# ShigemichiMatsuzaki/MSPL

Hardware: AMD Instinct MI355X
Metric: images/sec pseudo-label gen, ESPDNet-UE s=2.0 480x360(->288x480) bs=16 (higher is better)
Workload: dtype f32; 1 GPU; BASELINE configs[1]: ESPDNet-UE s=2.0 C=13 single-source pseudo-label gen (forward + pred+0.5aux argmax + KL uncertainty + histogram), bs=16/GPU, 16x3x288x480 fp32, hipGraph replay, 3 launches in flight per GPU, 2 consecutive batches of 16 per launch; per_gpu_batch=16, batches_in_flight=3, batches_per_launch=2, classes=13

## Files before the change

include/mspl_hip.h:

```cpp
#ifndef MSPL_HIP_H
#define MSPL_HIP_H

#include <stddef.h>
#include <stdint.h>

#ifdef __cplusplus
extern "C" {
#endif

typedef enum {
    MSPL_OK = 0,
    MSPL_ERR_BAD_SHAPE = -1,
    MSPL_ERR_UNSUPPORTED = -2,
    MSPL_ERR_NULL_POINTER = -3,
    MSPL_ERR_HIP = -4
} mspl_status;

typedef struct {
    const float* scale;
    const float* shift;
    const float* alpha;
    const float* pre_add;
    const float* residual;
    const float* reinf_r;
    const float* reinf_w;
    const float* gate;
    int32_t out_ctot;
    int32_t out_coff;
    float* raw_out;
    uint32_t struct_size;
    uint32_t flags;
} mspl_epilogue_t;

#define MSPL_LAUNCH_THROUGHPUT 1u
#define MSPL_LAUNCH_K2_STREAM_OFF 2u
#define MSPL_LAUNCH_K2_STREAM_FORCE 4u

const char* mspl_version(void);
#define MSPL_ABI_VERSION 5
int mspl_abi_version(void);
size_t mspl_last_error(char* buf, size_t cap);

int mspl_eesp_dw_hff_fwd(const float* x, const float* w, const int32_t dil[4], int32_t stride,
                         int32_t N, int32_t n, int32_t H, int32_t W,
                         const mspl_epilogue_t* ep, float* out, void* stream);

int mspl_conv1x1_fwd(const float* x, const float* w, int32_t N, int32_t Cin, int32_t Cout,
                     int32_t groups, int32_t HW, const mspl_epilogue_t* ep, float* out, void* stream);

int mspl_conv3x3_fwd(const float* x, const float* w, int32_t N, int32_t Cin, int32_t Cout,
                     int32_t groups, int32_t H, int32_t W, int32_t stride, int32_t shuffle_groups,
                     const mspl_epilogue_t* ep, float* out, void* stream);

int mspl_eesp_proj_dw_hff_fits(int32_t N, int32_t Cin, int32_t n, int32_t groups, int32_t H, int32_t W, const int32_t dil[4],
                               uint32_t launch_flags);
int mspl_eesp_proj_dw_hff_fwd(const float* x, const float* wp, const float* pscale, const float* pshift, const float* palpha,
                              const float* w, const int32_t dil[4], int32_t N, int32_t Cin, int32_t n, int32_t groups,
                              int32_t H, int32_t W, const mspl_epilogue_t* ep, float* out, void* stream);

int mspl_eesp_dw_exp_fits(int32_t N, int32_t n, int32_t H, int32_t W, const int32_t dil[4], uint32_t launch_flags);
int64_t mspl_eesp_dw_exp_pack_floats(int32_t n);
int mspl_eesp_dw_exp_pack(const float* w4, const float* bscale, const float* bshift, const float* balpha, const float* wexp,
                          int32_t n, int32_t H, int32_t W, const int32_t dil[4], float* packed, void* stream);
int mspl_eesp_dw_exp_fwd(const float* r, const float* packed, const int32_t dil[4], int32_t N, int32_t n, int32_t H, int32_t W,
                         const mspl_epilogue_t* ep, float* out, void* stream);
int64_t mspl_eesp_dw_exp_next_pack_floats(int32_t n);
int mspl_eesp_dw_exp_next_pack(const float* w1, int32_t n, float* next_packed, void* stream);
int mspl_eesp_dw_exp_next_fwd(const float* r, const float* packed, const int32_t dil[4], int32_t N, int32_t n, int32_t H, int32_t W,
                              const mspl_epilogue_t* ep, float* out, const float* next_packed, const float* nscale,
                              const float* nshift, const float* nalpha, float* rnext, void* stream);

int mspl_avgpool3x3s2_fwd(const float* x, int32_t N, int32_t C, int32_t H, int32_t W,
                          const mspl_epilogue_t* ep, float* out, void* stream);

int mspl_bilinear_fwd(const float* x, int32_t N, int32_t C, int32_t Hi, int32_t Wi, int32_t Ho,
                      int32_t Wo, int32_t align_corners, const mspl_epilogue_t* ep, float* out, void* stream);

int mspl_decoder_merge_fwd(const float* enc, const float* bu, const float* w3, const float* e_scale, const float* e_shift,
                           const float* e_alpha, const float* gate, const float* b_scale, const float* b_shift,
                           const float* b_alpha, const float* wp, const float* p_scale, const float* p_shift,
                           const float* p_alpha, int32_t N, int32_t Cin, int32_t Cout, int32_t P, int32_t H, int32_t W,
                           float* out, void* stream);

int mspl_adaptive_avgpool_fwd(const float* x, int32_t N, int32_t C, int32_t Hi, int32_t Wi,
                              int32_t Ho, int32_t Wo, const mspl_epilogue_t* ep, float* out,
                              void* stream);

int mspl_pointwise_fwd(const float* x, int32_t N, int32_t C, int32_t HW, const mspl_epilogue_t* ep,
                       float* out, void* stream);

int mspl_gap_gate_fwd(const float* x, const float* w, int32_t N, int32_t Cin, int32_t Cout,
                      int32_t HW, float* mean_ws, float* gate, void* stream);

int mspl_fusion_gate_fwd(const float* z, const float* rgb, const float* depth, int64_t count, float* out, void* stream);
int mspl_fusion_gate_bwd(const float* z, const float* rgb, const float* depth, const float* gy, int64_t count,
                         float* gz, float* grgb, float* gdepth, void* stream);

int mspl_avgpool3x3s2_psum_blocks(int32_t H, int32_t W);
int mspl_avgpool3x3s2_psum_fwd(const float* x, int32_t N, int32_t C, int32_t H, int32_t W, const mspl_epilogue_t* ep, float* out,
                               float* psum, void* stream);
int mspl_gate_from_sums_fwd(const float* psum, const float* w, int32_t N, int32_t Cin, int32_t Cout, int32_t nblk, int32_t HW,
                            float* gate, void* stream);

int mspl_down_head_fits(int32_t N, int32_t nin, int32_t n, int32_t groups, int32_t H, int32_t W, uint32_t launch_flags);
int mspl_down_head_psum_blocks(int32_t H, int32_t W);
int mspl_down_head_fwd(const float* x, const float* wp, const float* pscale, const float* pshift, const float* palpha, int32_t N,
                       int32_t nin, int32_t n, int32_t groups, int32_t H, int32_t W, const mspl_epilogue_t* ep, float* r, float* out,
                       float* psum, void* stream);

int64_t mspl_pyr_down_prep_lds_bytes(int32_t N, int32_t P, int32_t h, int32_t w, int32_t nb, const int32_t* hs,
                                     const int32_t* ws);
int mspl_pyr_down_prep_fwd(const float* x, int32_t N, int32_t P, int32_t h, int32_t w, int32_t nb, const int32_t* hs,
                           const int32_t* ws, const float* const* stage_w, float* const* out, void* stream);
int mspl_pyr_down_prep_train_fwd(const float* x, int32_t N, int32_t P, int32_t h, int32_t w, int32_t nb, const int32_t* hs,
                                 const int32_t* ws, const float* const* stage_w, float* const* out, float* const* pooled,
                                 void* stream);
int mspl_pyr_down_mid_bwd(const float* const* g_e, const float* const* pooled, const float* const* stage_w, int32_t N, int32_t P,
                          int32_t h, int32_t w, int32_t nb, const int32_t* hs, const int32_t* ws, float* const* gw,
                          float* const* gx, void* stream);

int mspl_pyrpool_fused_fwd(const float* x, int32_t N, int32_t P, int32_t h, int32_t w, int32_t nb,
                           const int32_t* hs, const int32_t* ws, const float* const* stage_w,
                           const float* const* down_e, const float* br_scale, const float* br_shift,
                           const float* br_alpha, const float* merge_w, const mspl_epilogue_t* ep,
                           float* out, void* stream);

int mspl_pyrpool_fused_train_fwd(const float* x, int32_t N, int32_t P, int32_t h, int32_t w, int32_t nb,
                                 const int32_t* hs, const int32_t* ws, const float* const* stage_w,
                                 const float* const* down_e, const float* br_scale, const float* br_shift,
                                 const float* br_alpha, const float* merge_w, const mspl_epilogue_t* ep,
                                 float* out, float* zcat, void* stream);
int mspl_pyrpool_fused_train_fits(int32_t N, int32_t P, int32_t h, int32_t w, int32_t nb, const int32_t* hs, const int32_t* ws);
int mspl_pyrpool_merge_bwd(const float* gy, const float* mraw, const float* zcat, int32_t N, int32_t P, int32_t h,
                           int32_t w, int32_t nb, const float* br_scale, const float* br_shift, const float* br_alpha,
                           const float* br_mean, const float* br_inv, const float* merge_w, const float* m_scale,
                           const float* m_shift, const float* m_alpha, const float* m_mean, const float* m_inv,
                           float* gt, float* g_br_scale, float* g_br_shift, float* g_br_alpha, float* g_merge_w,
                           float* g_m_scale, float* g_m_shift, float* g_m_alpha, void* stream);
int mspl_pyrpool_branch_bwd_fits(int32_t N, int32_t P, int32_t h, int32_t w, int32_t nb, const int32_t* hs, const int32_t* ws);
int mspl_pyrpool_branch_bwd(const float* x, int32_t N, int32_t P, int32_t h, int32_t w, int32_t nb, const int32_t* hs,
                            const int32_t* ws, const float* const* stage_w, const float* const* gt, float* const* gw,
                            const float* add0, const float* add1, float* gx, void* stream);
typedef enum {
    MSPL_PYR_BRANCH_BWD_UNSUPPORTED = 0,
    MSPL_PYR_BRANCH_BWD_STREAM3 = 1,
    MSPL_PYR_BRANCH_BWD_STREAM = 2,
    MSPL_PYR_BRANCH_BWD_TILE = 3
} mspl_pyr_branch_bwd_form_t;
int mspl_pyrpool_branch_bwd_plan(int32_t N, int32_t P, int32_t h, int32_t w, int32_t nb, const int32_t* hs, const int32_t* ws,
                                 int32_t aligned8, int32_t* form, int32_t* ncb, int32_t* nseg, int32_t* seg, int32_t* taps,
                                 int32_t* tiles_x, int32_t* tiles_y);

int mspl_label_epilogue_fwd(const float* main, const float* aux, int32_t N, int32_t C,
                            int32_t Hm, int32_t Wm, int32_t Ha, int32_t Wa, int32_t H, int32_t W,
                            const uint8_t* lut, uint8_t* labels, float* prob, float* kld,
                            float* main_up, float* aux_up, void* stream);

int64_t mspl_label_epilogue_hist_workspace_bytes(int32_t N, int32_t H, int32_t W);
int mspl_label_epilogue_hist_fits(int32_t N, int32_t C, int32_t Hm, int32_t Wm, int32_t Ha, int32_t Wa, int32_t H, int32_t W);
int mspl_label_epilogue_hist_fwd(const float* main, const float* aux, int32_t N, int32_t C,
                                 int32_t Hm, int32_t Wm, int32_t Ha, int32_t Wa, int32_t H, int32_t W,
                                 const uint8_t* lut, uint8_t* labels, float* kld, unsigned long long* hist,
                                 int32_t num_classes, void* workspace, int64_t workspace_bytes, void* stream);

int mspl_label_epilogue_planes_fits(int32_t N, int32_t P, int32_t C, int32_t Hm, int32_t Wm, int32_t Ha, int32_t Wa,
                                    int32_t H, int32_t W);
int mspl_label_epilogue_planes_fwd(const float* main_planes, const float* main_w, const float* main_b,
                                   const float* aux_planes, const float* aux_w, const float* aux_b, int32_t N, int32_t P,
                                   int32_t C, int32_t Hm, int32_t Wm, int32_t Ha, int32_t Wa, int32_t H, int32_t W,
                                   const uint8_t* lut, uint8_t* labels, float* kld, unsigned long long* hist,
                                   int32_t num_classes, void* workspace, int64_t workspace_bytes, void* stream);

int mspl_merge_labels_fwd(const uint8_t* const* src, int32_t S, int64_t npix, int32_t num_classes,
                          int32_t thresh, int32_t fill, uint8_t* out, unsigned long long* hist,
                          void* stream);


int mspl_conv_bwd_data(const float* gy, const float* w, int32_t N, int32_t Cin, int32_t Cout, int32_t groups,
                       int32_t H, int32_t W, int32_t K, int32_t stride, int32_t dilation, int32_t accumulate,
                       float* gx, void* stream);

int mspl_conv_bwd_weight(const float* gy, const float* x, int32_t N, int32_t Cin, int32_t Cout, int32_t groups,
                         int32_t H, int32_t W, int32_t K, int32_t stride, int32_t dilation, int32_t accumulate,
                         float* gw, void* stream);

typedef enum {
    MSPL_WGRAD_1X1_MFMA = 1,
    MSPL_WGRAD_1X1_LDS = 2,
    MSPL_WGRAD_STEM_S2_STRIP = 3,
    MSPL_WGRAD_STEM_COB4 = 4,
    MSPL_WGRAD_STRIP = 5,
    MSPL_WGRAD_G3X3 = 6,
    MSPL_WGRAD_GENERIC = 7
} mspl_wgrad_form_t;
int mspl_conv_bwd_weight_plan(int32_t N, int32_t Cin, int32_t Cout, int32_t groups, int32_t H, int32_t W, int32_t K, int32_t stride,
                              int32_t dilation, int32_t aligned16, int32_t* form, int32_t* parts, int32_t* ngroups);
int mspl_conv1x1_wgrad_batch(const float* const* gy, const float* const* x, float* const* gw, const float* const* rowscale,
                             const int32_t* N, const int32_t* Cin, const int32_t* Cout, const int32_t* groups, const int32_t* HW, int32_t nprob,
                             void* stream);

int mspl_down_tail_fwd(const float* a, const float* b, const float* reinf, const float* alpha, int32_t N, int32_t nin, int32_t C,
                       int32_t HW, float* y, void* stream);
int mspl_down_tail_bwd(const float* a, const float* b, const float* reinf, const float* gy, const float* alpha, int32_t N, int32_t nin,
                       int32_t C, int32_t HW, float* ga, float* gb, float* greinf, float* galpha, void* stream);

int mspl_affine_prelu_bwd(const float* c, const float* pre_add, const float* residual, const float* gy,
                          const float* scale, const float* shift, const float* alpha, int32_t N, int32_t C,
                          int32_t HW, float* gz, float* gc, float* gscale, float* gshift, float* galpha, void* stream);

int mspl_avgpool3x3s2_bwd(const float* gy, int32_t N, int32_t C, int32_t H, int32_t W, float* gx, void* stream);
int mspl_bilinear_bwd(const float* gy, int32_t N, int32_t C, int32_t Hi, int32_t Wi, int32_t Ho, int32_t Wo,
                      float* gx, void* stream);
int mspl_adaptive_avgpool_bwd(const float* gy, int32_t N, int32_t C, int32_t Hi, int32_t Wi, int32_t Ho, int32_t Wo,
                              float* gx, void* stream);
typedef enum {
    MSPL_BILINEAR_BWD_GENERIC8 = 1,
    MSPL_BILINEAR_BWD_GENERIC12 = 2,
    MSPL_BILINEAR_BWD_TILE8 = 3,
    MSPL_BILINEAR_BWD_TILE12 = 4,
    MSPL_BILINEAR_BWD_WAVE = 5,
    MSPL_BILINEAR_BWD_ROWS = 6
} mspl_bilinear_bwd_form_t;
typedef enum {
    MSPL_AVGPOOL_BWD_VEC = 1,
    MSPL_AVGPOOL_BWD_PLAIN = 2
} mspl_avgpool_bwd_form_t;
int mspl_bilinear_bwd_plan(int32_t N, int32_t C, int32_t Hi, int32_t Wi, int32_t Ho, int32_t Wo, int32_t aligned, int32_t* form,
                           int32_t* tiles_x, int32_t* tiles_y, int32_t* FH, int32_t* FW);
int mspl_avgpool3x3s2_bwd_plan(int32_t N, int32_t C, int32_t H, int32_t W, int32_t aligned16, int32_t* form);

int mspl_plane_dot(const float* a, const float* b, int32_t planes, int32_t HW, float* out, void* stream);
int mspl_plane_broadcast(const float* v, int32_t planes, int32_t HW, float mul, int32_t accumulate, float* gx,
                         void* stream);
int mspl_bn_prelu_bwd(const float* c, const float* pre_add, const float* residual, const float* gy, const float* scale,
                      const float* shift, const float* alpha, const float* bn_mean, const float* bn_inv, int32_t N, int32_t C,
                      int32_t HW, float* gz, float* gc, float* ggamma, float* gbeta, float* galpha, void* stream);
int mspl_gap_gate_bwd(const float* ggate, const float* gate, const float* mean, const float* w, int32_t N,
                      int32_t Cin, int32_t Cout, float* gw, float* gmean, void* stream);
int mspl_gap_gate_bwd_accum(const float* ggate, const float* gate, const float* mean, const float* w, int32_t N,
                      int32_t Cin, int32_t Cout, float* gw, float* gmean, void* stream);
int mspl_hff_suffix_sum(const float* g, int32_t N, int32_t n, int32_t HW, float* out, void* stream);

int mspl_hff_bn_prelu_suffix_bwd(const float* z, const float* gy, const float* scale, const float* shift, const float* alpha,
                                 const float* bn_mean, const float* bn_inv, int32_t N, int32_t n, int32_t HW, float* out,
                                 float* gscale, float* gshift, float* galpha, void* stream);

int mspl_uw_loss_fwd_bwd(const float* pred, const float* aux, const int64_t* target, const float* class_weights,
                         int32_t N, int32_t C, int32_t HW, float ce_scale, float* loss_acc, float* gpred,
                         float* gaux, float* kld_out, void* stream);
int mspl_uw_loss_scaled_fwd_bwd(const float* pred, const float* aux, const int64_t* target, const float* class_weights,
                                int32_t N, int32_t C, int32_t HW, float ce_scale, float out_scale, float* loss_acc,
                                float* gpred, float* gaux, float* kld_out, void* stream);
int mspl_uw_loss_heads_supported(int32_t C);
int mspl_uw_loss_heads_fwd_bwd(const float* main_lo, const float* aux_lo, const int64_t* target, const float* class_weights,
                               int32_t N, int32_t C, int32_t Hm, int32_t Wm, int32_t Ha, int32_t Wa, int32_t H, int32_t W,
                               float ce_scale, float out_scale, float* loss_acc, float* gpred, float* gaux, void* stream);
int mspl_uw_loss_heads_meters_fwd_bwd(const float* main_lo, const float* aux_lo, const int64_t* target, const float* class_weights,
                                      int32_t N, int32_t C, int32_t Hm, int32_t Wm, int32_t Ha, int32_t Wa, int32_t H, int32_t W,
                                      float ce_scale, float out_scale, float* loss_acc, float* gpred, float* gaux,
                                      int32_t miou_classes, float meter_weight, unsigned long long* areas, double* meter, void* stream);

int mspl_dense_conv_fwd(const float* x, const float* w_packed, int32_t N, int32_t Cin, int32_t Cout, int32_t H, int32_t W,
                        int32_t ksize, int32_t dilation, const mspl_epilogue_t* ep, float* out, void* stream);

int mspl_dense_conv_split_fits(int32_t Cin, int32_t Cout, int32_t ksize, int32_t planes);
int mspl_dense_conv_split_fwd(const float* x, const uint16_t* w_split, int32_t N, int32_t Cin, int32_t Cout, int32_t H, int32_t W,
                              int32_t ksize, int32_t dilation, int32_t planes, const mspl_epilogue_t* ep, float* out, void* stream);

int64_t mspl_dense_conv_wgrad_workspace_bytes(int32_t N, int32_t Cin, int32_t Cout, int32_t H, int32_t W, int32_t ksize,
                                              int32_t dilation, int32_t split);
int mspl_dense_conv_wgrad(const float* gy, const float* x, int32_t N, int32_t Cin, int32_t Cout, int32_t H, int32_t W,
                          int32_t ksize, int32_t dilation, int32_t split, void* workspace, int64_t workspace_bytes,
                          float* dw_packed, float* dbias, void* stream);
int mspl_dense_conv_dgrad(const float* const* gy, const float* const* wt_packed, const int32_t* ksize, const int32_t* dilation,
                          int32_t nbranch, int32_t N, int32_t Cg, int32_t Cx, int32_t H, int32_t W, int32_t accumulate,
                          float* gx, void* stream);

int mspl_miou_areas_fwd(const float* logits, const uint8_t* labels, const int64_t* target, int32_t N, int32_t C, int32_t HW,
                        int32_t num_classes, unsigned long long* hist, void* stream);

int mspl_eval_epilogue_fwd(const float* main, const float* aux, const int64_t* target, const float* class_weights,
                           int32_t N, int32_t C, int32_t Hm, int32_t Wm, int32_t Ha, int32_t Wa, int32_t H, int32_t W,
                           float aux_weight, int32_t ignore_index, int32_t miou_classes, double* loss_sums,
                           unsigned long long* areas, uint8_t* labels, void* stream);
int mspl_eval_batch_finalize(double* loss_sums, double* acc, int32_t batch_images, void* stream);

int mspl_ce_meters_fwd(const float* pred, const int64_t* target, const float* class_weights, int32_t ignore_index, int32_t N,
                       int32_t C, int32_t HW, int32_t miou_classes, double* sums, unsigned long long* areas, void* stream);
int mspl_ce_flood_finalize(double* sums, float flood_level, int32_t batch_images, float* out3, double* meter, void* stream);

int mspl_ce_head_supported(int32_t C);
int mspl_ce_head_fits(int32_t N, int32_t C, int32_t Hm, int32_t Wm, int32_t H, int32_t W);
int mspl_ce_head_meters_fwd_bwd(const float* head, const int64_t* target, const float* class_weights, int32_t ignore_index,
                                int32_t N, int32_t C, int32_t Hm, int32_t Wm, int32_t H, int32_t W, int32_t miou_classes,
                                double* sums, unsigned long long* areas, float* ghead_full, void* stream);

int mspl_pixelwise_kld_fwd(const float* d1, const float* d2, int32_t N, int32_t C, int32_t HW, float* kld, void* stream);
int mspl_pixelwise_kld_bwd(const float* d1, const float* d2, const float* gkld, int32_t N, int32_t C, int32_t HW,
                           float* gd1, float* gd2, void* stream);
int mspl_weighted_ce_fwd(const float* pred, const int64_t* target, const float* u_weight, const float* class_weights,
                         int32_t ignore_index, int32_t N, int32_t C, int32_t HW, float* sums, void* stream);
int mspl_weighted_ce_bwd(const float* pred, const int64_t* target, const float* u_weight, const float* class_weights,
                         int32_t ignore_index, int32_t N, int32_t C, int32_t HW, const float* g, const float* den,
                         float* gpred, float* gu, void* stream);

int mspl_resample_ksize(int32_t in_size, int32_t out_size);
int mspl_resample_coeffs(int32_t in_size, int32_t out_size, int32_t* bounds, int32_t* kk);
int mspl_nearest_index(int32_t in_size, int32_t out_size, int32_t* idx);
int mspl_preprocess_u8_fwd(const uint8_t* src, int32_t N, int32_t Hs, int32_t Ws, int32_t C, int32_t H, int32_t W,
                           const int32_t* xb, const int32_t* xk, int32_t kx, const int32_t* yb, const int32_t* yk,
                           int32_t ky, const float* mean, const float* stdv, const uint8_t* flip, uint8_t* tmp,
                           float* out, void* stream);
int mspl_resize_label_fwd(const uint8_t* src, int32_t N, int32_t Hs, int32_t Ws, int32_t H, int32_t W,
                          const int32_t* yi, const int32_t* xi, const uint8_t* flip, int64_t* out, void* stream);

void* mspl_png_writer_create(int32_t workers, int32_t level);
int64_t mspl_png_writer_submit(void* writer, const uint8_t* host, int32_t n, int32_t H, int32_t W, const char* const* paths,
                               void* event);
int mspl_png_writer_poll(void* writer, int64_t ticket, int32_t block);
int mspl_png_writer_destroy(void* writer);

int mspl_bn_batch_stats_fwd(const float* z, int32_t N, int32_t C, int32_t HW, float eps, float momentum,
                            float* running_mean, float* running_var, double* ws, float* mean, float* invstd, void* stream);
int mspl_bn_batch_stats_fold_fwd(const float* z, int32_t N, int32_t C, int32_t HW, float eps, float momentum,
                                 float* running_mean, float* running_var, const float* gamma, const float* beta,
                                 double* ws, float* mean, float* invstd, float* scale, float* shift, void* stream);
int mspl_pyrpool_merge_fwd(const float* zcat, int32_t N, int32_t P, int32_t h, int32_t w, int32_t nb, const float* br_scale,
                           const float* br_shift, const float* br_alpha, const float* merge_w, float* out, void* stream);
int mspl_bn_stats_path_add(float* g, const float* z, const float* p, const float* q, int32_t N, int32_t P, int32_t nb, int32_t HW,
                           void* stream);
int64_t mspl_bn_fused_workspace_bytes(int32_t C);
int mspl_bn_batch_stats_fused_fwd(const float* z, int32_t N, int32_t C, int32_t HW, float eps, float momentum,
                                  float* running_mean, float* running_var, const float* gamma, const float* beta,
                                  void* ws_zeroed, float* mean, float* invstd, float* scale, float* shift,
                                  int64_t* num_batches_tracked, void* stream);
int mspl_bn_train_prelu_bwd(const float* z, const float* residual, const float* gy, const float* scale, const float* shift,
                            const float* alpha, const float* gamma, const float* mean, const float* invstd, int32_t N, int32_t C,
                            int32_t HW, float* gres, float* gc, void* ws_zeroed, int32_t accumulate, float* ggamma, float* gbeta,
                            float* galpha, float* p, float* q, void* stream);
int mspl_bn_train_small_fits(int32_t N, int32_t C, int32_t HW);
int mspl_bn_train_small_fwd(const float* z, const float* residual, const float* gamma, const float* beta, const float* alpha,
                            int32_t N, int32_t C, int32_t HW, float eps, float momentum, float* running_mean, float* running_var,
                            int64_t* num_batches_tracked, float* mean, float* invstd, float* scale, float* shift, float* y, void* stream);
int mspl_bn_train_small_bwd(const float* z, const float* residual, const float* gy, const float* scale, const float* shift,
                            const float* alpha, const float* gamma, const float* mean, const float* invstd, int32_t N, int32_t C,
                            int32_t HW, float eps, int32_t accumulate, float* gz, float* gres, float* ggamma, float* gbeta,
                            float* galpha, void* stream);
int mspl_bn_train_prelu_bwd_apply(const float* z, const float* gy, const float* scale, const float* shift, const float* alpha,
                                  const float* p, const float* q, int32_t N, int32_t C, int32_t HW, float* gz, void* stream);
int mspl_bn_batch_stats_bwd_coeffs(const float* gscale, const float* gshift, const float* gamma, const float* mean,
                                   const float* invstd, const float* scale, int32_t C, double M, int32_t accumulate,
                                   float* ggamma, float* gbeta, float* p, float* q, void* stream);
int mspl_sgd_step(float* p, const float* g, float* buf, int64_t n, float lr, float momentum, float weight_decay,
                  int32_t first_step, void* stream);

int64_t mspl_nid_workspace_floats(int32_t C, int32_t H, int32_t W, int32_t K);
int mspl_nid_hist_fwd(const float* camera, const float* label, int32_t B, int32_t C, int32_t H, int32_t W, int32_t K,
                      float bw_camera, float bw_label, float* ws, float* out, void* stream);
int mspl_nid_hist_bwd(const float* camera, const float* label, int32_t B, int32_t C, int32_t H, int32_t W, int32_t K,
                      float bw_camera, float bw_label, const float* gjoint, const float* gpl, float* glabel, void* stream);

int mspl_eesp_dw_bwd(const float* gs, const float* x, const float* w4, const int32_t* dil, int32_t stride, int32_t N,
                     int32_t n, int32_t H, int32_t W, float* gx, float* const* gw, void* stream);
int mspl_eesp_dw_bwd_weight_chunks(int32_t N, int32_t n, int32_t H, int32_t W, int32_t stride);

int mspl_eesp_bwd_fused_fits(int32_t N, int32_t n, int32_t H, int32_t W, const int32_t* dil);
int mspl_eesp_bwd_fused_bands(int32_t N, int32_t n, int32_t H, int32_t W, const int32_t* dil, int32_t* band_rows);
int mspl_eesp_bwd_fused(const float* z, const float* gy, const float* x, const float* w4, const int32_t* dil,
                        const float* scale, const float* shift, const float* alpha, const float* bn_mean,
                        const float* bn_inv, int32_t N, int32_t n, int32_t H, int32_t W, float* gx, float* const* gw,
                        float* gscale, float* gshift, float* galpha, const float* proj_c, const float* proj_scale,
                        const float* proj_shift, const float* proj_alpha, const float* proj_mean, const float* proj_inv,
                        float* g_proj_scale, float* g_proj_shift, float* g_proj_alpha, void* stream);

int mspl_hff_bn_stat_suffix_bwd(const float* z, const float* gy, const float* scale, const float* shift, const float* alpha,
                                const float* stat_p, const float* stat_q, int32_t N, int32_t n, int32_t HW, float* out, void* stream);
int mspl_eesp_bwd_fused_bnstat(const float* z, const float* gy, const float* x, const float* w4, const int32_t* dil,
                               const float* scale, const float* shift, const float* alpha, const float* stat_p, const float* stat_q,
                               int32_t N, int32_t n, int32_t H, int32_t W, float* gx, float* const* gw, void* stream);

int mspl_sum_n(const float* const* srcs, int32_t n, int64_t count, float* out, void* stream);
int mspl_sum_n_planes(const float* const* srcs, int32_t n, const float* plane_const, float mul, int32_t planes, int32_t HW, float* out,
                      void* stream);

int mspl_transpose_weights(const void* seg_table, const void* block_table, int32_t nblocks, void* stream);

int mspl_adam_step(float* p, const float* g, float* m, float* v, int64_t n, float lr, double beta1, double beta2,
                   float eps, float weight_decay, int32_t step, void* stream);

#define MSPL_FILTER_LANCZOS 1
#define MSPL_FILTER_BILINEAR 2
int mspl_resample_ksize_filter(int32_t in_size, int32_t out_size, int32_t filter);
int mspl_resample_coeffs_filter(int32_t in_size, int32_t out_size, int32_t filter, int32_t* bounds, int32_t* kk);

typedef struct mspl_train_rec {
    const int32_t* scale_x;
    const int32_t* scale_y;
    const int32_t* dscale_x;
    const int32_t* dscale_y;
    const int32_t* out_x;
    const int32_t* out_y;
    const int32_t* near_x;
    const int32_t* near_y;
    const int32_t* near_out_x;
    const int32_t* near_out_y;
    int32_t sh, sw;
    int32_t pad_h, pad_w;
    int32_t crop_i, crop_j;
    int32_t flip;
    int32_t reserved;
} mspl_train_rec_t;
int64_t mspl_train_transform_workspace_bytes(int32_t N, int32_t max_sh, int32_t max_sw, int32_t with_depth);
int mspl_train_transform_fwd(const uint8_t* rgb, const uint8_t* label, const uint8_t* depth, int32_t N, int32_t Hs, int32_t Ws,
                             int32_t H, int32_t W, int32_t crop, int32_t ignore_idx, const mspl_train_rec_t* recs_host,
                             const mspl_train_rec_t* recs_dev, const float* mean, const float* stdv, uint8_t* ws, int32_t max_sh,
                             int32_t max_sw, float* out_rgb, int64_t* out_label, float* out_depth, void* stream);

#ifdef __cplusplus
}
#endif
#endif
```

mspl_amd/csrc/pyrpool.hip:

```cpp
#include <stdlib.h>

#include "common.hpp"

namespace mspl {

constexpr int PYR_MAXB = 5;
constexpr int PYR_HALO = 4;

struct PyrGeom {
    int N, P, h, w, nb;
    int kind[PYR_MAXB];
    int hs[PYR_MAXB], ws[PYR_MAXB];
    float sh[PYR_MAXB], sw[PYR_MAXB];
    const float* stage_w[PYR_MAXB];
    const float* down_e[PYR_MAXB];
    const float* br_scale; const float* br_shift; const float* br_alpha;
    const float* merge_w;
    int TH, TW, tiles_y, tiles_x;
    int XW;
    int UH[PYR_MAXB], UW[PYR_MAXB], uoff[PYR_MAXB];
    int toff[PYR_MAXB];
    int boff, BW;
    int woff;
    unsigned mag_uw[PYR_MAXB], mag_bw;
    int CPB, cblocks;
    int stop_after;
    float* zcat;
};

__device__ __forceinline__ int ada_s(int o, int I, int O) { return (int)(((unsigned)o * (unsigned)I) / (unsigned)O); }
__device__ __forceinline__ int ada_e(int o, int I, int O) { return (int)((((unsigned)(o + 1)) * (unsigned)I + O - 1) / (unsigned)O); }
__device__ __forceinline__ int fdiv(int t, unsigned magic) { return (int)(((unsigned)t * magic) >> 24); }

__global__ __launch_bounds__(256) void pyrpool_fused_kernel(const float* __restrict__ x, PyrGeom g, Epi e,
                                                            float* __restrict__ out) {
    extern __shared__ __attribute__((aligned(16))) float smem[];
    float* xs = smem;
    float* wl = smem + g.woff;
    int bid = blockIdx.x;
    const int txi = bid % g.tiles_x;  bid /= g.tiles_x;
    const int tyi = bid % g.tiles_y;  bid /= g.tiles_y;
    const int cb = bid % g.cblocks;
    const int n = bid / g.cblocks;
    const int y0 = tyi * g.TH, x0 = txi * g.TW;
    const int tid = threadIdx.x;
    const int XH = g.TH + 2 * PYR_HALO;
    const int BH = g.TH + 2, BW2 = g.TW + 2;
    const int py_lo = max(y0 - 1, 0), px_lo = max(x0 - 1, 0);

#pragma unroll
    for (int i = 0; i < PYR_MAXB; ++i) {
        if (i >= g.nb) break;
        float* T = smem + g.toff[i];
        if (g.kind[i] == 0) {
            const int UH = g.UH[i], UW = g.UW[i];
            const int u0 = ada_s(py_lo, g.hs[i], g.h) - 1, v0 = ada_s(px_lo, g.ws[i], g.w) - 1;
            float* UR = T; float* UC = UR + 4 * UH; float* WR = UC + 4 * UW; float* WC = WR + 2 * BH;
            for (int t = tid; t < UH + UW + BH + BW2; t += 256) {
                if (t < UH) {
                    const int u = u0 + t;
                    int ya = 0, yb = 0;  float w0 = 0.f, w1 = 0.f;
                    if (u >= 0 && u < g.hs[i]) bilinear_src(g.sh[i], u, g.h, ya, yb, w0, w1); else { ya = y0; yb = y0; }
                    UR[4 * t] = __int_as_float((ya - y0 + PYR_HALO) * g.XW); UR[4 * t + 1] = __int_as_float((yb - y0 + PYR_HALO) * g.XW);
                    UR[4 * t + 2] = w0; UR[4 * t + 3] = w1;
                } else if (t < UH + UW) {
                    const int q = t - UH, v = v0 + q;
                    int xa = 0, xb = 0;  float w0 = 0.f, w1 = 0.f;
                    if (v >= 0 && v < g.ws[i]) bilinear_src(g.sw[i], v, g.w, xa, xb, w0, w1); else { xa = x0; xb = x0; }
                    UC[4 * q] = __int_as_float(xa - x0 + PYR_HALO); UC[4 * q + 1] = __int_as_float(xb - x0 + PYR_HALO);
                    UC[4 * q + 2] = w0; UC[4 * q + 3] = w1;
                } else if (t < UH + UW + BH) {
                    const int r = t - UH - UW, py = y0 - 1 + r;
                    int first = 0, cnt = 0;
                    if (py >= 0 && py < g.h) { const int us = ada_s(py, g.hs[i], g.h); first = us - 1 - u0; cnt = ada_e(py, g.hs[i], g.h) - us; }
                    WR[2 * r] = __int_as_float(first * UW); WR[2 * r + 1] = __int_as_float(cnt);
                } else {
                    const int q = t - UH - UW - BH, px = x0 - 1 + q;
                    int first = 0, cnt = 0;
                    if (px >= 0 && px < g.w) { const int vs = ada_s(px, g.ws[i], g.w); first = vs - 1 - v0; cnt = ada_e(px, g.ws[i], g.w) - vs; }
                    WC[2 * q] = __int_as_float(first); WC[2 * q + 1] = __int_as_float(cnt);
                }
            }
        } else if (g.kind[i] == 2) {
            float* DR = T; float* DC = DR + 4 * BH;
            for (int t = tid; t < BH + BW2; t += 256) {
                if (t < BH) {
                    const int py = min(max(y0 - 1 + t, 0), g.h - 1);
                    int ya, yb;  float w0, w1;
                    bilinear_src(g.sh[i], py, g.hs[i], ya, yb, w0, w1);
                    DR[4 * t] = __int_as_float(ya * g.ws[i]); DR[4 * t + 1] = __int_as_float(yb * g.ws[i]); DR[4 * t + 2] = w0; DR[4 * t + 3] = w1;
                } else {
                    const int q = t - BH, px = min(max(x0 - 1 + q, 0), g.w - 1);
                    int xa, xb;  float w0, w1;
                    bilinear_src(g.sw[i], px, g.ws[i], xa, xb, w0, w1);
                    DC[4 * q] = __int_as_float(xa); DC[4 * q + 1] = __int_as_float(xb); DC[4 * q + 2] = w0; DC[4 * q + 3] = w1;
                }
            }
        }
    }

    const int xv = g.XW >> 2;
    const bool w4 = (g.w & 3) == 0;
    auto load_x = [&](int c, int i) -> float4 {
        const float* xp = x + ((size_t)n * g.P + c) * (size_t)g.h * g.w;
        const int r = i / xv, v = i - r * xv;
        const int iy = y0 - PYR_HALO + r, ix = x0 - PYR_HALO + 4 * v;
        float4 val = make_float4(0.f, 0.f, 0.f, 0.f);
        if (iy >= 0 && iy < g.h) {
            const float* row = xp + (size_t)iy * g.w;
            if (w4 && ix >= 0 && ix + 3 < g.w) {
                val = *reinterpret_cast<const float4*>(row + ix);
            } else {
                if (ix >= 0 && ix < g.w) val.x = row[ix];
                if (ix + 1 >= 0 && ix + 1 < g.w) val.y = row[ix + 1];
                if (ix + 2 >= 0 && ix + 2 < g.w) val.z = row[ix + 2];
                if (ix + 3 >= 0 && ix + 3 < g.w) val.w = row[ix + 3];
            }
        }
        return val;
    };
    auto load_const = [&](int c, int t) -> float {
        const int n9 = g.nb * 9;
        if (t < n9) { const int i = t / 9, k = t - i * 9; return (g.kind[i] != 2) ? g.stage_w[i][c * 9 + k] : 0.f; }
        if (t < 2 * n9) { const int u = t - n9, i = u / 9, k = u - i * 9; return g.merge_w[((size_t)c * g.nb + i) * 9 + k]; }
        const int u = t - 2 * n9, i = u / 3, k = u - i * 3;
        return (k == 0 ? g.br_scale : (k == 1 ? g.br_shift : g.br_alpha))[i * g.P + c];
    };
    const int nx = XH * xv;
    const int nconst = 2 * g.nb * 9 + 3 * g.nb;
    const int c_first = cb * g.CPB;
    float4 xr0 = make_float4(0.f, 0.f, 0.f, 0.f), xr1 = xr0;
    float cr = 0.f;
    if (tid < nx) xr0 = load_x(c_first, tid);
    if (tid + 256 < nx) xr1 = load_x(c_first, tid + 256);
    if (tid < nconst) cr = load_const(c_first, tid);

    for (int ci = 0; ci < g.CPB; ++ci) {
    const int c = c_first + ci;
    if (tid < nx) *reinterpret_cast<float4*>(xs + (tid / xv) * g.XW + 4 * (tid % xv)) = xr0;
    if (tid + 256 < nx) *reinterpret_cast<float4*>(xs + ((tid + 256) / xv) * g.XW + 4 * ((tid + 256) % xv)) = xr1;
    for (int i = tid + 512; i < nx; i += 256) *reinterpret_cast<float4*>(xs + (i / xv) * g.XW + 4 * (i % xv)) = load_x(c, i);
    if (tid < nconst) wl[tid] = cr;
    if (ci + 1 < g.CPB) {
        if (tid < nx) xr0 = load_x(c + 1, tid);
        if (tid + 256 < nx) xr1 = load_x(c + 1, tid + 256);
        if (tid < nconst) cr = load_const(c + 1, tid);
    }
    __syncthreads();
    if (g.stop_after == 1) return;

#pragma unroll
    for (int i = 0; i < PYR_MAXB; ++i) {
        if (i < g.nb && g.kind[i] == 0) {
            float* U = smem + g.uoff[i];
            const int UH = g.UH[i], UW = g.UW[i];
            const float* UR = smem + g.toff[i];
            const float* UC = UR + 4 * UH;
            const unsigned mag = g.mag_uw[i];
            const int nU = UH * UW;
            for (int t = tid; t < nU; t += 256) {
                const int r = fdiv(t, mag), q = t - r * UW;
                const float4 rr = *reinterpret_cast<const float4*>(UR + 4 * r);
                const float4 cc = *reinterpret_cast<const float4*>(UC + 4 * q);
                const float* ra = xs + __float_as_int(rr.x);
                const float* rb = xs + __float_as_int(rr.y);
                const int xa = __float_as_int(cc.x), xb = __float_as_int(cc.y);
                const float top = cc.z * ra[xa] + cc.w * ra[xb];
                const float bot = cc.z * rb[xa] + cc.w * rb[xb];
                U[t] = rr.z * top + rr.w * bot;
            }
        }
    }
    __syncthreads();
    if (g.stop_after == 2) return;

    float* B = smem + g.boff;
    const int npos = BH * BW2;
    const int XWl = g.XW, BWl = g.BW, hl = g.h, wl_ = g.w;
    const unsigned magb = g.mag_bw;
    auto keep_raw = [&](int i, int r, int q, int py, int px, float b) {
        if (g.zcat && r >= 1 && r <= g.TH && q >= 1 && q <= g.TW)
            g.zcat[(((size_t)n * g.nb + i) * g.P + c) * (size_t)hl * wl_ + (size_t)py * wl_ + px] = b;
    };
#pragma unroll
    for (int i = 0; i < PYR_MAXB; ++i) {
        if (i >= g.nb) break;
        const float* ws9 = wl + i * 9;
        const float* kbr = wl + 2 * g.nb * 9 + i * 3;
        const float bsc = kbr[0], bsh = kbr[1], bal = kbr[2];
        float* Bi = B + i * BH * BWl;
        const float* T = smem + g.toff[i];
        if (g.kind[i] == 1) {
            const float w00 = ws9[0], w01 = ws9[1], w02 = ws9[2], w10 = ws9[3], w11 = ws9[4], w12 = ws9[5],
                        w20 = ws9[6], w21 = ws9[7], w22 = ws9[8];
            for (int t = tid; t < npos; t += 256) {
                const int r = fdiv(t, magb), q = t - r * BW2;
                const int py = y0 - 1 + r, px = x0 - 1 + q;
                float b = 0.f;
                if (py >= 0 && py < hl && px >= 0 && px < wl_) {
                    const float* p = xs + (r + PYR_HALO - 2) * XWl + (q + PYR_HALO - 2);
                    b = w00 * p[0];
                    b = fmaf(w01, p[1], b); b = fmaf(w02, p[2], b);
                    b = fmaf(w10, p[XWl], b); b = fmaf(w11, p[XWl + 1], b); b = fmaf(w12, p[XWl + 2], b);
                    b = fmaf(w20, p[2 * XWl], b); b = fmaf(w21, p[2 * XWl + 1], b); b = fmaf(w22, p[2 * XWl + 2], b);
                    keep_raw(i, r, q, py, px, b);
                    b = fmaf(b, bsc, bsh);
                    b = b > 0.f ? b : bal * b;
                }
                Bi[r * BWl + q] = b;
            }
        } else if (g.kind[i] == 0) {
            const float* U = smem + g.uoff[i];
            const int UW = g.UW[i];
            const float* WR = T + 4 * g.UH[i] + 4 * UW;
            const float* WC = WR + 2 * BH;
            const float w00 = ws9[0], w01 = ws9[1], w02 = ws9[2], w10 = ws9[3], w11 = ws9[4], w12 = ws9[5],
                        w20 = ws9[6], w21 = ws9[7], w22 = ws9[8];
            for (int t = tid; t < npos; t += 256) {
                const int r = fdiv(t, magb), q = t - r * BW2;
                const int py = y0 - 1 + r, px = x0 - 1 + q;
                float b = 0.f;
                if (py >= 0 && py < hl && px >= 0 && px < wl_) {
                    const float2 wr = *reinterpret_cast<const float2*>(WR + 2 * r);
                    const float2 wc = *reinterpret_cast<const float2*>(WC + 2 * q);
                    const int rcnt = __float_as_int(wr.y), ccnt = __float_as_int(wc.y);
                    const float* p0 = U + __float_as_int(wr.x) + __float_as_int(wc.x);
                    float s = 0.f;
                    if (rcnt == 2 && ccnt == 2) {
                        float u[4][4];
#pragma unroll
                        for (int a2 = 0; a2 < 4; ++a2)
#pragma unroll
                            for (int b2 = 0; b2 < 4; ++b2) u[a2][b2] = p0[a2 * UW + b2];
#pragma unroll
                        for (int du = 0; du < 2; ++du)
#pragma unroll
                            for (int dv = 0; dv < 2; ++dv) {
                                float cv = w00 * u[du][dv];
                                cv = fmaf(w01, u[du][dv + 1], cv); cv = fmaf(w02, u[du][dv + 2], cv);
                                cv = fmaf(w10, u[du + 1][dv], cv); cv = fmaf(w11, u[du + 1][dv + 1], cv); cv = fmaf(w12, u[du + 1][dv + 2], cv);
                                cv = fmaf(w20, u[du + 2][dv], cv); cv = fmaf(w21, u[du + 2][dv + 1], cv); cv = fmaf(w22, u[du + 2][dv + 2], cv);
                                s += cv;
                            }
                        b = s * 0.25f;
                    } else {
                        for (int du = 0; du < rcnt; ++du)
                            for (int dv = 0; dv < ccnt; ++dv) {
                                const float* p = p0 + du * UW + dv;
                                float cv = w00 * p[0];
                                cv = fmaf(w01, p[1], cv); cv = fmaf(w02, p[2], cv);
                                cv = fmaf(w10, p[UW], cv); cv = fmaf(w11, p[UW + 1], cv); cv = fmaf(w12, p[UW + 2], cv);
                                cv = fmaf(w20, p[2 * UW], cv); cv = fmaf(w21, p[2 * UW + 1], cv); cv = fmaf(w22, p[2 * UW + 2], cv);
                                s += cv;
                            }
                        b = s / (float)(rcnt * ccnt);
                    }
                    keep_raw(i, r, q, py, px, b);
                    b = fmaf(b, bsc, bsh);
                    b = b > 0.f ? b : bal * b;
                }
                Bi[r * BWl + q] = b;
            }
        } else {
            const float* E = g.down_e[i] + ((size_t)n * g.P + c) * (size_t)g.hs[i] * g.ws[i];
            for (int t = tid; t < npos; t += 256) {
                const int r = fdiv(t, magb), q = t - r * BW2;
                const int py = y0 - 1 + r, px = x0 - 1 + q;
                float b = 0.f;
                if (py >= 0 && py < hl && px >= 0 && px < wl_) {
                    const float4 rr = *reinterpret_cast<const float4*>(T + 4 * r);
                    const float4 cc = *reinterpret_cast<const float4*>(T + 4 * BH + 4 * q);
                    const float* ra = E + __float_as_int(rr.x);
                    const float* rb = E + __float_as_int(rr.y);
                    const int xa = __float_as_int(cc.x), xb = __float_as_int(cc.y);
                    const float top = cc.z * ra[xa] + cc.w * ra[xb];
                    const float bot = cc.z * rb[xa] + cc.w * rb[xb];
                    b = rr.z * top + rr.w * bot;
                    keep_raw(i, r, q, py, px, b);
                    b = fmaf(b, bsc, bsh);
                    b = b > 0.f ? b : bal * b;
                }
                Bi[r * BWl + q] = b;
            }
        }
    }
    __syncthreads();
    if (g.stop_after == 3) return;

    const int cabs = e.coff + c;
    const EpiCh ec = epi_channel(e, cabs);
    const int XS = g.TW >> 2;
    const int nstrip = g.TH * XS, nbl = g.nb;
    for (int t = tid; t < nstrip; t += 256) {
        const int ty = t / XS, xsi = t - ty * XS;
        const int y = y0 + ty, xb = x0 + xsi * 4;
        if (y >= hl || xb >= wl_) continue;
        float acc[4] = {0.f, 0.f, 0.f, 0.f};
#pragma unroll
        for (int i = 0; i < PYR_MAXB; ++i) {
            if (i >= nbl) break;
            const float* wm = wl + nbl * 9 + i * 9;
#pragma unroll
            for (int ky = 0; ky < 3; ++ky) {
                const float* row = B + (i * BH + ty + ky) * BWl + xsi * 4;
                const float4 a = *reinterpret_cast<const float4*>(row);
                const float2 b2 = *reinterpret_cast<const float2*>(row + 4);
                const float rv[6] = {a.x, a.y, a.z, a.w, b2.x, b2.y};
#pragma unroll
                for (int j = 0; j < 4; ++j) {
                    acc[j] = fmaf(wm[ky * 3 + 0], rv[j], acc[j]);
                    acc[j] = fmaf(wm[ky * 3 + 1], rv[j + 1], acc[j]);
                    acc[j] = fmaf(wm[ky * 3 + 2], rv[j + 2], acc[j]);
                }
            }
        }
        const int pix = y * wl_ + xb;
        float* dst = out + epi_offset(e, n, cabs, pix);
        if (e.raw) {
            float* rdst = e.raw + ((size_t)n * g.P + c) * (size_t)hl * wl_ + pix;
#pragma unroll
            for (int j = 0; j < 4; ++j)
                if (xb + j < wl_) rdst[j] = acc[j];
        }
        if ((wl_ & 3) == 0) {
            store_out4(dst, epi_apply4(e, ec, acc, n, cabs, pix));
        } else {
#pragma unroll
            for (int j = 0; j < 4; ++j)
                if (xb + j < wl_) dst[j] = epi_apply(e, ec, acc[j], n, cabs, pix + j);
        }
    }
    __syncthreads();
    }
}

int pyrpool_sep_try(const float* x, int N, int P, int h, int w, int nb, const int32_t* hs, const int32_t* ws,
                    const float* const* stage_w, const float* const* down_e, const float* br_scale,
                    const float* br_shift, const float* br_alpha, const float* merge_w, const Epi& e, float* out,
                    hipStream_t stream, unsigned launch_flags);
int pyrpool_stream_try(const float* x, int N, int P, int h, int w, int nb, const int32_t* hs, const int32_t* ws,
                       const float* const* stage_w, const float* const* down_e, const float* br_scale,
                       const float* br_shift, const float* br_alpha, const float* merge_w, const Epi& e, float* out,
                       hipStream_t stream, float* zcat = nullptr);

}

using namespace mspl;

static int pyrpool_fused_launch(const float* x, int32_t N, int32_t P, int32_t h, int32_t w, int32_t nb,
                               const int32_t* hs, const int32_t* ws, const float* const* stage_w,
                               const float* const* down_e, const float* br_scale, const float* br_shift,
                               const float* br_alpha, const float* merge_w, const mspl_epilogue_t* ep,
                               float* out, float* zcat, void* stream, bool dry = false) {
    MSPL_REQUIRE(dry || (x && hs && ws && stage_w && down_e && br_scale && br_shift && br_alpha && merge_w && out),
                 MSPL_ERR_NULL_POINTER, "pyrpool_fused: null pointer");
    MSPL_REQUIRE(hs && ws, MSPL_ERR_NULL_POINTER, "pyrpool_fused: null pointer");
    MSPL_REQUIRE(N > 0 && P > 0 && h > 0 && w > 0, MSPL_ERR_BAD_SHAPE, "pyrpool_fused: bad shape N=%d P=%d %dx%d", N, P, h, w);
    MSPL_REQUIRE(nb >= 1 && nb <= PYR_MAXB, MSPL_ERR_UNSUPPORTED, "pyrpool_fused: %d branches (1..%d)", nb, PYR_MAXB);
    if (int rc = check_epi(ep, P, "pyrpool_fused", zcat != nullptr)) return rc;
    if (!dry) {
        static const int force_tables = MSPL_TUNE_INT("MSPL_PYR_TABLES", 0);
        if (!force_tables) {
            const int rc3 = pyrpool_stream_try(x, N, P, h, w, nb, hs, ws, stage_w, down_e, br_scale, br_shift, br_alpha, merge_w,
                                               make_epi(ep, P, h * w), out, (hipStream_t)stream, zcat);
            if (rc3 <= 0) return rc3;
            if (!zcat) {
                const int rc = pyrpool_sep_try(x, N, P, h, w, nb, hs, ws, stage_w, down_e, br_scale, br_shift, br_alpha, merge_w,
                                               make_epi(ep, P, h * w), out, (hipStream_t)stream, epi_flags(ep));
                if (rc <= 0) return rc;
            }
        }
    }
    PyrGeom g;
    memset(&g, 0, sizeof(g));
    g.N = N; g.P = P; g.h = h; g.w = w; g.nb = nb;
    g.br_scale = br_scale; g.br_shift = br_shift; g.br_alpha = br_alpha; g.merge_w = merge_w;
    g.zcat = zcat;
    g.TW = w >= 32 ? 32 : ((w + 3) & ~3);
    g.TH = h >= 16 ? 16 : h;
    g.tiles_x = ceil_div(w, g.TW);
    g.tiles_y = ceil_div(h, g.TH);
    g.XW = g.TW + 2 * PYR_HALO;
    int off = (g.TH + 2 * PYR_HALO) * g.XW;
    off = (off + 3) & ~3;
    for (int i = 0; i < nb; ++i) {
        MSPL_REQUIRE(hs[i] > 0 && ws[i] > 0, MSPL_ERR_BAD_SHAPE, "pyrpool_fused: branch %d size %dx%d", i, hs[i], ws[i]);
        g.hs[i] = hs[i]; g.ws[i] = ws[i];
        g.stage_w[i] = dry ? nullptr : stage_w[i]; g.down_e[i] = dry ? nullptr : down_e[i];
        if (hs[i] == h && ws[i] == w) {
            g.kind[i] = 1;
            MSPL_REQUIRE(dry || stage_w[i], MSPL_ERR_NULL_POINTER, "pyrpool_fused: branch %d needs stage weights", i);
        } else if (hs[i] >= h && ws[i] >= w) {
            g.kind[i] = 0;
            MSPL_REQUIRE(dry || stage_w[i], MSPL_ERR_NULL_POINTER, "pyrpool_fused: branch %d needs stage weights", i);
            MSPL_REQUIRE(hs[i] <= 4 * h && ws[i] <= 4 * w, MSPL_ERR_UNSUPPORTED, "pyrpool_fused: up-scale beyond 4x");
            g.sh[i] = bilinear_scale(h, hs[i]); g.sw[i] = bilinear_scale(w, ws[i]);
            g.UH[i] = (int)(((int64_t)(g.TH + 2) * hs[i] + h - 1) / h) + 4;
            g.UW[i] = (int)(((int64_t)(g.TW + 2) * ws[i] + w - 1) / w) + 4;
            g.uoff[i] = off;
            off += g.UH[i] * g.UW[i];
            off = (off + 3) & ~3;
        } else if (hs[i] <= h && ws[i] <= w) {
            g.kind[i] = 2;
            MSPL_REQUIRE(dry || down_e[i], MSPL_ERR_NULL_POINTER, "pyrpool_fused: branch %d needs its low-resolution map", i);
            g.sh[i] = bilinear_scale(hs[i], h); g.sw[i] = bilinear_scale(ws[i], w);
        } else {
            set_error("pyrpool_fused: branch %d mixes up- and down-sampling (%dx%d vs %dx%d)", i, hs[i], ws[i], h, w);
            return MSPL_ERR_UNSUPPORTED;
        }
    }
    auto magic = [](int d) { return (unsigned)(((1u << 24) + (unsigned)d - 1) / (unsigned)d); };
    for (int i = 0; i < nb; ++i) {
        g.toff[i] = off;
        if (g.kind[i] == 0) { off += 4 * g.UH[i] + 4 * g.UW[i] + 2 * (g.TH + 2) + 2 * (g.TW + 2); g.mag_uw[i] = magic(g.UW[i]); }
        else if (g.kind[i] == 2) off += 4 * (g.TH + 2) + 4 * (g.TW + 2);
        off = (off + 3) & ~3;
    }
    g.mag_bw = magic(g.TW + 2);
    static const int dbg_stop = MSPL_TUNE_INT("MSPL_PYR_STOP", 0);
    g.stop_after = dbg_stop;
    g.BW = (g.TW + 2 + 3 + 4) & ~3;
    g.boff = off;
    off += nb * (g.TH + 2) * g.BW;
    off = (off + 3) & ~3;
    g.woff = off;
    off += nb * 9 * 2 + nb * 3;
    const size_t lds = (size_t)off * sizeof(float);
    MSPL_REQUIRE(lds <= 64 * 1024, MSPL_ERR_UNSUPPORTED, "pyrpool_fused: tile needs %zu B of LDS", lds);
    if (dry) return MSPL_OK;
    const Epi e = make_epi(ep, P, h * w);
    int cpb = 1;
    while (cpb * 2 <= P && P % (cpb * 2) == 0 && (int64_t)N * (P / (cpb * 2)) * g.tiles_y * g.tiles_x >= 2048) cpb *= 2;
    static const int dbg_cpb = MSPL_TUNE_INT("MSPL_PYR_CPB", 0);
    if (dbg_cpb > 0 && P % dbg_cpb == 0) cpb = dbg_cpb;
    g.CPB = cpb; g.cblocks = P / cpb;
    const int64_t blocks = (int64_t)N * g.cblocks * g.tiles_y * g.tiles_x;
    MSPL_REQUIRE(blocks < (1ll << 31), MSPL_ERR_BAD_SHAPE, "pyrpool_fused: grid too large");
    hipLaunchKernelGGL(pyrpool_fused_kernel, dim3((unsigned)blocks), dim3(256), lds, (hipStream_t)stream, x, g, e, out);
    MSPL_CHECK_LAUNCH("pyrpool_fused");
    return MSPL_OK;
}

extern "C" int mspl_pyrpool_fused_fwd(const float* x, int32_t N, int32_t P, int32_t h, int32_t w, int32_t nb,
                                      const int32_t* hs, const int32_t* ws, const float* const* stage_w,
                                      const float* const* down_e, const float* br_scale, const float* br_shift,
                                      const float* br_alpha, const float* merge_w, const mspl_epilogue_t* ep,
                                      float* out, void* stream) {
    return pyrpool_fused_launch(x, N, P, h, w, nb, hs, ws, stage_w, down_e, br_scale, br_shift, br_alpha, merge_w, ep, out, nullptr,
                                stream);
}

extern "C" int mspl_pyrpool_fused_train_fwd(const float* x, int32_t N, int32_t P, int32_t h, int32_t w, int32_t nb,
                                            const int32_t* hs, const int32_t* ws, const float* const* stage_w,
                                            const float* const* down_e, const float* br_scale, const float* br_shift,
                                            const float* br_alpha, const float* merge_w, const mspl_epilogue_t* ep,
                                            float* out, float* zcat, void* stream) {
    MSPL_REQUIRE(zcat, MSPL_ERR_NULL_POINTER, "pyrpool_fused_train: zcat is required");
    return pyrpool_fused_launch(x, N, P, h, w, nb, hs, ws, stage_w, down_e, br_scale, br_shift, br_alpha, merge_w, ep, out, zcat,
                                stream);
}

extern "C" int mspl_pyrpool_fused_train_fits(int32_t N, int32_t P, int32_t h, int32_t w, int32_t nb, const int32_t* hs,
                                             const int32_t* ws) {
    float dummy = 0.f;
    return pyrpool_fused_launch(nullptr, N, P, h, w, nb, hs, ws, nullptr, nullptr, nullptr, nullptr, nullptr, nullptr, nullptr, nullptr,
                                &dummy, nullptr, true) == MSPL_OK;
}
```

mspl_amd/csrc/pyrpool_stream.hip:

```cpp
#include <stdlib.h>

#include <algorithm>

#include "common.hpp"
#include "pyr_stencil.hpp"

namespace mspl {

constexpr int P3_MAXB = 5;
#ifndef P3_STEPS
#define P3_STEPS 2
#endif
constexpr int P3_SEGMAX = 19;

struct Pyr3Geom {
    int N, P, h, w;
    int hs[P3_MAXB], ws[P3_MAXB];
    float sh[P3_MAXB], sw[P3_MAXB];
    int SEG, nseg, ncb, CBW;
    unsigned total;
};

template <int T, int PXL>
__device__ __forceinline__ void p3_up_branch(const float (&xw)[5][PXL + 4], const float* __restrict__ Arow,
                                             const float (&C)[3][PXL][5], float (&b)[PXL]) {
    constexpr int R0 = (5 - T) / 2;
    constexpr int NCOL = PXL + T - 1;
#pragma unroll
    for (int ky = 0; ky < 3; ++ky) {
        float a[5];
        {
            const float4 t4 = *reinterpret_cast<const float4*>(Arow + ky * 8);
            a[0] = t4.x; a[1] = t4.y; a[2] = t4.z; a[3] = t4.w;
            a[4] = T > 4 ? Arow[ky * 8 + 4] : 0.f;
        }
        float cs[NCOL];
#pragma unroll
        for (int s = 0; s < NCOL; ++s) {
            float v = a[0] * xw[R0][R0 + s];
#pragma unroll
            for (int rr = 1; rr < T; ++rr) v = fmaf(a[rr], xw[R0 + rr][R0 + s], v);
            cs[s] = v;
        }
#pragma unroll
        for (int j = 0; j < PXL; ++j) {
            float v = b[j];
#pragma unroll
            for (int s = 0; s < T; ++s) v = fmaf(C[ky][j][s], cs[j + s], v);
            b[j] = v;
        }
    }
}

template <int PXL> struct P3Vec;
template <> struct P3Vec<1> { typedef float T; };
template <> struct P3Vec<2> { typedef float2 T; };

template <int T0, int T1, int PXL, bool TRAIN>
__global__ __launch_bounds__(256, 2) void pyrpool_stream_kernel(const float* __restrict__ x, const float* __restrict__ sw0,
                                                                const float* __restrict__ sw1, const float* __restrict__ sw2,
                                                                const float* __restrict__ de3, const float* __restrict__ de4,
                                                                const float* __restrict__ br_scale, const float* __restrict__ br_shift,
                                                                const float* __restrict__ br_alpha, const float* __restrict__ merge_w,
                                                                const float* __restrict__ ep_scale,
                                                                const float* __restrict__ ep_shift,
                                                                const float* __restrict__ ep_alpha, int ep_ctot, int ep_coff,
                                                                Pyr3Geom g, float* __restrict__ out, float* __restrict__ zcat,
                                                                float* __restrict__ mraw) {
    __shared__ __attribute__((aligned(16))) float At[2][(P3_SEGMAX + 2) * 24];
    __shared__ float Gt[2][3][PXL][5][64];
    __shared__ __attribute__((aligned(16))) float Wm[4][5][12];
    const int lane = threadIdx.x & 63, wave = __builtin_amdgcn_readfirstlane(threadIdx.x >> 6);
    unsigned bid = blockIdx.x;
    const int sgi = bid % g.nseg;  bid /= g.nseg;
    const int cb = bid % g.ncb;  bid /= g.ncb;
    const int plane = (int)bid * 4 + wave;
    const int n = plane / g.P, c = plane - n * g.P;
    const int h = g.h, w = g.w;
    const int ys = sgi * g.SEG, ye = min(ys + g.SEG, h);
    const int px0 = cb * g.CBW + (lane - 1) * PXL;
    const bool writer = lane >= 1 && lane <= 62 && px0 < w;

    if (wave < 2) {
        const int ri = lane / 3, ky = lane - 3 * ri;
        if (ri < g.SEG + 2) {
            float acc[5];
            if (wave == 0) p3_coeffs<T0>(ys - 1 + ri, ky, h, g.hs[0], g.sh[0], acc);
            else p3_coeffs<T1>(ys - 1 + ri, ky, h, g.hs[1], g.sh[1], acc);
            float* d = &At[wave][ri * 24 + ky * 8];
            d[0] = acc[0]; d[1] = acc[1]; d[2] = acc[2]; d[3] = acc[3]; d[4] = acc[4];
        }
    }
#pragma unroll
    for (int t = 0; t < 6 * PXL; ++t) {
        if ((t & 3) == wave) {
            const int ub = t / (3 * PXL), r = t - ub * 3 * PXL, kx = r / PXL, j = r - kx * PXL;
            float acc[5];
            if (ub == 0) p3_coeffs<T0>(px0 + j, kx, w, g.ws[0], g.sw[0], acc);
            else p3_coeffs<T1>(px0 + j, kx, w, g.ws[1], g.sw[1], acc);
#pragma unroll
            for (int q = 0; q < 5; ++q) Gt[ub][kx][j][q][lane] = acc[q];
        }
    }
    __syncthreads();
    float C0[3][PXL][5], C1[3][PXL][5];
    {
        const float* w0p = sw0 + (size_t)c * 9;
        const float* w1p = sw1 + (size_t)c * 9;
#pragma unroll
        for (int j = 0; j < PXL; ++j)
#pragma unroll
            for (int s2 = 0; s2 < 5; ++s2) {
                const float a0 = Gt[0][0][j][s2][lane], a1 = Gt[0][1][j][s2][lane], a2 = Gt[0][2][j][s2][lane];
                const float b0 = Gt[1][0][j][s2][lane], b1 = Gt[1][1][j][s2][lane], b2 = Gt[1][2][j][s2][lane];
#pragma unroll
                for (int ky = 0; ky < 3; ++ky) {
                    C0[ky][j][s2] = fmaf(w0p[ky * 3 + 2], a2, fmaf(w0p[ky * 3 + 1], a1, w0p[ky * 3] * a0));
                    C1[ky][j][s2] = fmaf(w1p[ky * 3 + 2], b2, fmaf(w1p[ky * 3 + 1], b1, w1p[ky * 3] * b0));
                }
            }
    }
    unsigned dxa[2][PXL], dxb[2][PXL];  float dw0[2][PXL], dw1[2][PXL];
#pragma unroll
    for (int i = 0; i < 2; ++i)
#pragma unroll
        for (int j = 0; j < PXL; ++j) {
            const int px = min(max(px0 + j, 0), w - 1);
            int xa, xb;
            bilinear_src(g.sw[3 + i], px, g.ws[3 + i], xa, xb, dw0[i][j], dw1[i][j]);
            dxa[i][j] = (unsigned)xa * 4u;  dxb[i][j] = (unsigned)xb * 4u;
        }
    const float* wsame = sw2 + (size_t)c * 9;
    if (lane < 45) Wm[wave][lane / 9][lane % 9] = merge_w[(size_t)c * 45 + lane];
    const float4* wmq = reinterpret_cast<const float4*>(&Wm[wave][0][0]);
    float bsc[5], bsh[5], bal[5];
#pragma unroll
    for (int i = 0; i < 5; ++i) { bsc[i] = br_scale[i * g.P + c]; bsh[i] = br_shift[i * g.P + c]; bal[i] = br_alpha[i * g.P + c]; }
    const int cabs = ep_coff + c;
    const float esc = ep_scale ? ep_scale[cabs] : 1.f, esh = ep_shift ? ep_shift[cabs] : 0.f, eal = ep_alpha ? ep_alpha[cabs] : 1.f;
    const unsigned plane_id = __builtin_amdgcn_readfirstlane((unsigned)(n * g.P + c));
    const float* xpl = x + (size_t)plane_id * (size_t)(h * w);
    const float* e3 = de3 + (size_t)plane_id * (size_t)(g.hs[3] * g.ws[3]);
    const float* e4 = de4 + (size_t)plane_id * (size_t)(g.hs[4] * g.ws[4]);
    float* opl = out + ((size_t)__builtin_amdgcn_readfirstlane((unsigned)(n * ep_ctot + cabs))) * (size_t)(h * w);
    bool colin[PXL];
#pragma unroll
    for (int j = 0; j < PXL; ++j) colin[j] = px0 + j >= 0 && px0 + j < w;

    constexpr unsigned P3_OOB = 0x7ffffff0u;
    unsigned xoff[PXL + 4];
#pragma unroll
    for (int j = 0; j < PXL + 4; ++j) {
        const int cx = px0 - 2 + j;
        xoff[j] = (cx >= 0 && cx < w) ? (unsigned)cx * 4u : P3_OOB;
    }
    auto load_row = [&](int r, float (&v)[PXL + 4]) {
        const bool rin = r >= 0 && r < h;
        const float* row = xpl + (size_t)(rin ? r : 0) * w;
        const __amdgpu_buffer_rsrc_t rs = __builtin_amdgcn_make_buffer_rsrc(const_cast<float*>(row), 0, rin ? w * 4 : 0, 0x00020000);
        if (PXL == 2) {
#pragma unroll
            for (int j = 0; j < PXL + 4; j += 2) {
                typedef unsigned u32x2 __attribute__((ext_vector_type(2)));
                const u32x2 t = __builtin_amdgcn_raw_buffer_load_b64(rs, xoff[j], 0, 0);
                v[j] = __uint_as_float(t.x);  v[j + 1] = __uint_as_float(t.y);
            }
        } else {
#pragma unroll
            for (int j = 0; j < PXL + 4; ++j) v[j] = __uint_as_float(__builtin_amdgcn_raw_buffer_load_b32(rs, xoff[j], 0, 0));
        }
    };

    float xw[5][PXL + 4];
#pragma unroll
    for (int rr = 0; rr < 5; ++rr) load_row(ys - 3 + rr, xw[rr]);
    float en[2][PXL][4];
    float enwy0[2], enwy1[2];
    auto load_e = [&](int r) {
#pragma unroll
        for (int i = 0; i < 2; ++i) {
            int ya, yb;
            bilinear_src(g.sh[3 + i], min(max(r, 0), h - 1), g.hs[3 + i], ya, yb, enwy0[i], enwy1[i]);
            const int rowb = g.ws[3 + i] * 4;
            const __amdgpu_buffer_rsrc_t ra = __builtin_amdgcn_make_buffer_rsrc(const_cast<float*>((i == 0 ? e3 : e4) + ya * g.ws[3 + i]), 0, rowb, 0x00020000);
            const __amdgpu_buffer_rsrc_t rb = __builtin_amdgcn_make_buffer_rsrc(const_cast<float*>((i == 0 ? e3 : e4) + yb * g.ws[3 + i]), 0, rowb, 0x00020000);
#pragma unroll
            for (int j = 0; j < PXL; ++j) {
                en[i][j][0] = __uint_as_float(__builtin_amdgcn_raw_buffer_load_b32(ra, dxa[i][j], 0, 0));
                en[i][j][1] = __uint_as_float(__builtin_amdgcn_raw_buffer_load_b32(ra, dxb[i][j], 0, 0));
                en[i][j][2] = __uint_as_float(__builtin_amdgcn_raw_buffer_load_b32(rb, dxa[i][j], 0, 0));
                en[i][j][3] = __uint_as_float(__builtin_amdgcn_raw_buffer_load_b32(rb, dxb[i][j], 0, 0));
            }
        }
    };
    load_e(ys - 1);
    float acc[3][PXL];
#pragma unroll
    for (int r = 0; r < 3; ++r)
#pragma unroll
        for (int j = 0; j < PXL; ++j) acc[r][j] = 0.f;

    auto row_step = [&](const int br) __attribute__((always_inline)) {
        float bv[5][PXL];
        const bool rowin = br >= 0 && br < h;
        float ecur[2][PXL][4], wy0c[2], wy1c[2];
#pragma unroll
        for (int i = 0; i < 2; ++i) {
            wy0c[i] = enwy0[i]; wy1c[i] = enwy1[i];
#pragma unroll
            for (int j = 0; j < PXL; ++j)
#pragma unroll
                for (int q = 0; q < 4; ++q) ecur[i][j][q] = en[i][j][q];
        }
        if (br < ye) load_e(br + 1);
        float xn[PXL + 4];
        load_row(br + 3, xn);
        __builtin_amdgcn_sched_barrier(0);
        if (rowin) {
            const float* A0 = &At[0][(br - (ys - 1)) * 24];
            const float* A1 = &At[1][(br - (ys - 1)) * 24];
#pragma unroll
            for (int j = 0; j < PXL; ++j) { bv[0][j] = 0.f; bv[1][j] = 0.f; bv[2][j] = 0.f; }
            p3_up_branch<T0, PXL>(xw, A0, C0, bv[0]);
            p3_up_branch<T1, PXL>(xw, A1, C1, bv[1]);
#pragma unroll
            for (int ky = 0; ky < 3; ++ky) {
                const float w0 = wsame[ky * 3], w1 = wsame[ky * 3 + 1], w2 = wsame[ky * 3 + 2];
#pragma unroll
                for (int j = 0; j < PXL; ++j) {
                    bv[2][j] = fmaf(w0, xw[1 + ky][j + 1], bv[2][j]);
                    bv[2][j] = fmaf(w1, xw[1 + ky][j + 2], bv[2][j]);
                    bv[2][j] = fmaf(w2, xw[1 + ky][j + 3], bv[2][j]);
                }
            }
#pragma unroll
            for (int i = 0; i < 2; ++i)
#pragma unroll
                for (int j = 0; j < PXL; ++j) {
                    const float top = dw0[i][j] * ecur[i][j][0] + dw1[i][j] * ecur[i][j][1];
                    const float bot = dw0[i][j] * ecur[i][j][2] + dw1[i][j] * ecur[i][j][3];
                    bv[3 + i][j] = wy0c[i] * top + wy1c[i] * bot;
                }
            if (TRAIN && writer && br >= ys && br < ye) {
#pragma unroll
                for (int i = 0; i < 5; ++i) {
                    float* zp = zcat + (((size_t)n * 5 + i) * g.P + c) * (size_t)h * w + (size_t)br * w + px0;
                    if (PXL == 2) *reinterpret_cast<float2*>(zp) = make_float2(bv[i][0], bv[i][PXL - 1]);
                    else zp[0] = bv[i][0];
                }
            }
#pragma unroll
            for (int i = 0; i < 5; ++i)
#pragma unroll
                for (int j = 0; j < PXL; ++j) {
                    float v = fmaf(bv[i][j], bsc[i], bsh[i]);
                    v = v > 0.f ? v : bal[i] * v;
                    bv[i][j] = colin[j] ? v : 0.f;
                }
        } else {
#pragma unroll
            for (int i = 0; i < 5; ++i)
#pragma unroll
                for (int j = 0; j < PXL; ++j) bv[i][j] = 0.f;
        }
#pragma unroll
        for (int i = 0; i < 5; ++i) {
            float bx[PXL + 2];
            bx[0] = p3_from_left(bv[i][PXL - 1]);
#pragma unroll
            for (int j = 0; j < PXL; ++j) bx[1 + j] = bv[i][j];
            bx[PXL + 1] = p3_from_right(bv[i][0]);
            const float4 q0 = wmq[i * 3], q1 = wmq[i * 3 + 1], q2 = wmq[i * 3 + 2];
            const float wv[12] = {q0.x, q0.y, q0.z, q0.w, q1.x, q1.y, q1.z, q1.w, q2.x, q2.y, q2.z, q2.w};
#pragma unroll
            for (int r = 0; r < 3; ++r) {
                const int ky = 2 - r;
                const float w0 = wv[ky * 3], w1 = wv[ky * 3 + 1], w2 = wv[ky * 3 + 2];
#pragma unroll
                for (int j = 0; j < PXL; ++j) {
                    acc[r][j] = fmaf(w0, bx[j], acc[r][j]);
                    acc[r][j] = fmaf(w1, bx[j + 1], acc[r][j]);
                    acc[r][j] = fmaf(w2, bx[j + 2], acc[r][j]);
                }
            }
        }
#pragma unroll
        for (int rr = 0; rr < 4; ++rr)
#pragma unroll
            for (int j = 0; j < PXL + 4; ++j) xw[rr][j] = xw[rr + 1][j];
#pragma unroll
        for (int j = 0; j < PXL + 4; ++j) xw[4][j] = xn[j];
        const int y = br - 1;
        if (y >= ys) {
            float v[PXL];
#pragma unroll
            for (int j = 0; j < PXL; ++j) {
                v[j] = fmaf(acc[0][j], esc, esh);
                v[j] = (ep_alpha && v[j] <= 0.f) ? eal * v[j] : v[j];
            }
            if (writer) {
                float* dst = opl + (size_t)y * w + px0;
                if (PXL == 2) store_out2(dst, make_float2(v[0], v[PXL - 1]));
                else dst[0] = v[0];
                if (TRAIN) {
                    float* rp = mraw + ((size_t)n * g.P + c) * (size_t)h * w + (size_t)y * w + px0;
                    if (PXL == 2) *reinterpret_cast<float2*>(rp) = make_float2(acc[0][0], acc[0][PXL - 1]);
                    else rp[0] = acc[0][0];
                }
            }
        }
#pragma unroll
        for (int j = 0; j < PXL; ++j) { acc[0][j] = acc[1][j]; acc[1][j] = acc[2][j]; acc[2][j] = 0.f; }
    };
    constexpr int STEPS = TRAIN ? 2 : P3_STEPS;
#pragma unroll 1
    for (int br = ys - 1; br <= ye; br += STEPS) {
        row_step(br);
#pragma unroll
        for (int u = 1; u < STEPS; ++u)
            if (br + u <= ye) row_step(br + u);
    }
}

int pyrpool_stream_try(const float* x, int N, int P, int h, int w, int nb, const int32_t* hs, const int32_t* ws,
                       const float* const* stage_w, const float* const* down_e, const float* br_scale,
                       const float* br_shift, const float* br_alpha, const float* merge_w, const Epi& e, float* out,
                       hipStream_t stream, float* zcat) {
    static const int off = (MSPL_TUNE_INT("MSPL_PYR_STREAM", 1) == 0);
    static const int min_w = MSPL_TUNE_INT("MSPL_PYR_STREAM_MINW", 40);
    if (off || nb != 5 || w < min_w || ((int64_t)N * P) % 4 != 0) return 1;
    if (e.pre_add || e.residual || e.reinf_r || e.gate) return 1;
    for (int i = 0; i < 5; ++i) if (hs[i] <= 0 || ws[i] <= 0) return 1;
    if (!(hs[0] > h && ws[0] > w && hs[1] > h && ws[1] > w)) return 1;
    if (!(hs[2] == h && ws[2] == w)) return 1;
    if (!(hs[3] <= h && ws[3] <= w && hs[4] <= h && ws[4] <= w && (hs[3] < h || ws[3] < w) && (hs[4] < h || ws[4] < w))) return 1;
    if (!stage_w[0] || !stage_w[1] || !stage_w[2] || !down_e[3] || !down_e[4]) return 1;
    int taps[2];
    for (int i = 0; i < 2; ++i) {
        const int R = std::max(p3_stencil_radius(h, hs[i]), p3_stencil_radius(w, ws[i]));
        if (R > 2) return 1;
        taps[i] = R <= 1 ? 3 : 5;
    }
    const int PXL = w <= 62 ? 1 : 2;
    if (PXL == 2 && ((w & 1) || (((uintptr_t)out) & 7) || (((uintptr_t)x) & 7))) return 1;
    if (zcat && (!e.raw || e.ctot != P || e.coff != 0)) return 1;
    if (zcat && PXL == 2 && ((((uintptr_t)zcat) | ((uintptr_t)e.raw)) & 7)) return 1;
    Pyr3Geom g;
    memset(&g, 0, sizeof(g));
    g.N = N; g.P = P; g.h = h; g.w = w;
    for (int i = 0; i < 5; ++i) {
        g.hs[i] = hs[i]; g.ws[i] = ws[i];
        if (i < 2) { g.sh[i] = bilinear_scale(h, hs[i]); g.sw[i] = bilinear_scale(w, ws[i]); }
        if (i > 2) { g.sh[i] = bilinear_scale(hs[i], h); g.sw[i] = bilinear_scale(ws[i], w); }
    }
    g.CBW = 62 * PXL;
    g.ncb = ceil_div(w, g.CBW);
    static const int dbg_seg = MSPL_TUNE_INT("MSPL_PYR_SEG", 0);
    int seg = std::min(h, P3_SEGMAX);
    while (seg > 6 && (int64_t)N * P * g.ncb * ceil_div(h, seg) < 2048) --seg;
    seg = ceil_div(h, ceil_div(h, seg));
    if (dbg_seg > 0 && dbg_seg <= P3_SEGMAX) seg = std::min(dbg_seg, h);
    g.SEG = seg;
    g.nseg = ceil_div(h, seg);
    const int64_t waves = (int64_t)N * P * g.ncb * g.nseg;
    if (waves >= (1ll << 31)) return 1;
    g.total = (unsigned)waves;
    const dim3 grid((unsigned)(waves / 4)), blk(256);
#define MSPL_P3_LAUNCH(A, B, L) do { \
        if (zcat) hipLaunchKernelGGL((pyrpool_stream_kernel<A, B, L, true>), grid, blk, 0, stream, x, stage_w[0], stage_w[1], stage_w[2], down_e[3], down_e[4], br_scale, br_shift, br_alpha, merge_w, e.scale, e.shift, e.alpha, e.ctot, e.coff, g, out, zcat, e.raw); \
        else hipLaunchKernelGGL((pyrpool_stream_kernel<A, B, L, false>), grid, blk, 0, stream, x, stage_w[0], stage_w[1], stage_w[2], down_e[3], down_e[4], br_scale, br_shift, br_alpha, merge_w, e.scale, e.shift, e.alpha, e.ctot, e.coff, g, out, (float*)nullptr, (float*)nullptr); } while (0)
    if (PXL == 1) {
        if (taps[0] == 3 && taps[1] == 3) MSPL_P3_LAUNCH(3, 3, 1);
        else if (taps[0] == 3) MSPL_P3_LAUNCH(3, 5, 1);
        else if (taps[1] == 3) MSPL_P3_LAUNCH(5, 3, 1);
        else MSPL_P3_LAUNCH(5, 5, 1);
    } else {
        if (taps[0] == 3 && taps[1] == 3) MSPL_P3_LAUNCH(3, 3, 2);
        else if (taps[0] == 3) MSPL_P3_LAUNCH(3, 5, 2);
        else if (taps[1] == 3) MSPL_P3_LAUNCH(5, 3, 2);
        else MSPL_P3_LAUNCH(5, 5, 2);
    }
#undef MSPL_P3_LAUNCH
    MSPL_CHECK_LAUNCH("pyrpool_fused(streaming form)");
    return MSPL_OK;
}

}
```

mspl_amd/layers.py:

```python
import contextlib
import gc
import math
import os
import weakref

import torch
from torch import nn

from . import autograd as ag
from . import ops
from .ops import Epi

config_inp_reinf = 3
PYR_SCALES = (2.0, 1.5, 1.0, 0.5, 0.1)


_PARAM_EPOCH = [0]


def bump_param_epoch():
    _PARAM_EPOCH[0] += 1


def _key(tensors):
    return (_PARAM_EPOCH[0],) + tuple((t.data_ptr(), t._version) for t in tensors)


def cached(module, name, deps, builder):
    store = module.__dict__.setdefault('_mspl_cache', {})
    k = _key(deps)
    hit = store.get(name)
    if hit is None or hit[0] != k:
        with torch.no_grad():
            val = builder()
        store[name] = hit = (k, val)
    return hit[1]


def _require_eval(bn):
    if bn.training:
        raise RuntimeError('mspl_amd: BatchNorm in training mode under torch.no_grad(): the fused inference kernels fold the '
                           'running statistics; call model.eval() (the uest label pass runs frozen BN, '
                           'uest_seg_multi_os.py:605-608), or enable gradients for the batch-statistics training path')


def bn_fold(bn):
    _require_eval(bn)

    def build():
        scale = bn.weight * torch.rsqrt(bn.running_var + bn.eps)
        return scale.contiguous(), (bn.bias - bn.running_mean * scale).contiguous()
    return cached(bn, 'fold', [bn.weight, bn.bias, bn.running_mean, bn.running_var], build)


_SIDE_ENABLED = os.environ.get('MSPL_SIDE_STREAMS', '1') != '0'
_SIDE_STREAMS = {}


class side_streams(object):

    def __init__(self, enabled):
        self.enabled = enabled

    def __enter__(self):
        global _SIDE_ENABLED
        self.prev = _SIDE_ENABLED
        _SIDE_ENABLED = self.enabled and os.environ.get('MSPL_SIDE_STREAMS', '1') != '0'

    def __exit__(self, *exc):
        global _SIDE_ENABLED
        _SIDE_ENABLED = self.prev


def _side_stream(idx, device, parent):
    dev = device.index if device.index is not None else torch.cuda.current_device()
    key = (dev, idx, parent.cuda_stream)
    st = _SIDE_STREAMS.get(key)
    if st is None:
        st = _SIDE_STREAMS[key] = torch.cuda.Stream(device=dev)
    return st


class fork(object):

    def __init__(self, idx, inputs=()):
        self.idx, self.inputs, self.ctx = idx, inputs, None

    def __enter__(self):
        if not _SIDE_ENABLED or _training_path() or not self.inputs:
            return self
        cur = torch.cuda.current_stream(self.inputs[0].device)
        side = _side_stream(self.idx, self.inputs[0].device, cur)
        side.wait_stream(cur)
        for t in self.inputs:
            t.record_stream(side)
        self.ctx = torch.cuda.stream(side)
        self.ctx.__enter__()
        return self

    def __exit__(self, *exc):
        if self.ctx is not None:
            self.ctx.__exit__(*exc)
        return False

    def mark(self):
        if self.ctx is None:
            return None
        ev = torch.cuda.Event()
        ev.record(torch.cuda.current_stream())
        return ev


def wait_mark(ev, outputs=()):
    if ev is None:
        return
    cur = torch.cuda.current_stream()
    cur.wait_event(ev)
    for t in outputs:
        if t is not None:
            t.record_stream(cur)


def join(idx, outputs=()):
    outs = [t for t in outputs if t is not None]
    if not _SIDE_ENABLED or _training_path() or not outs:
        return
    cur = torch.cuda.current_stream(outs[0].device)
    cur.wait_stream(_side_stream(idx, outs[0].device, cur))
    for t in outs:
        t.record_stream(cur)


@contextlib.contextmanager
def graph_capture(graph, **kw):
    gc.collect()
    was_enabled = gc.isenabled()
    gc.disable()
    try:
        with torch.cuda.graph(graph, **kw):
            yield
    finally:
        if was_enabled:
            gc.enable()


def _training_path():
    return torch.is_grad_enabled()


def _conv_train(x, conv):
    if conv.kernel_size[0] == 3 and conv.dilation[0] != 1:
        raise RuntimeError('mspl_amd: dilated 3x3 convolutions only occur inside EESP (fused branch op)')
    return ag.conv(x, conv.weight, conv.stride[0], conv.groups)


def _bn_act(z, bn, alpha=None, pre_add=None, residual=None):
    if bn.training:
        if pre_add is not None:
            z, pre_add = z + pre_add, None
        if _FUSED_BN_TRAIN:
            return ag.bn_train_prelu(z, bn, alpha, residual)
        scale, shift = ag.bn_batch_stats(z, bn)
    else:
        scale, shift = train_fold(bn)
        return ag.bn_prelu(z, bn, scale, shift, alpha, pre_add=pre_add, residual=residual)
    return ag.affine_prelu(z, scale, shift, alpha, pre_add=pre_add, residual=residual)


_FUSED_TRAIN_FWD = os.environ.get('MSPL_TRAIN_FUSED_FWD', '1') != '0'
_EESP_DW_BN = os.environ.get('MSPL_EESP_DW_BN', '1') != '0'
_CONV_SKIP = os.environ.get('MSPL_CONV_SKIP', '1') != '0'
_FUSED_BN_TRAIN = os.environ.get('MSPL_FUSED_BN_TRAIN', '1') != '0'
_FUSED_DW_EXP = os.environ.get('MSPL_EESP_EXP', '1') != '0'
_FUSED_DOWN_HEAD = os.environ.get('MSPL_DOWN_HEAD', '1') != '0'
_FUSED_HEAD_CLASSIFIER = os.environ.get('MSPL_HEAD_CLASSIFIER', '1') != '0'
_FUSED_DEC_MERGE = True
_FUSED_NEXT_PROJ = os.environ.get('MSPL_EESP_NEXT', '1') != '0'
_FUSED_EESP_TRAIN = os.environ.get('MSPL_FUSED_EESP_TRAIN', '1') != '0'
_FUSED_PYR_TRAIN = os.environ.get('MSPL_FUSED_PYR_TRAIN', '1') != '0'


def _conv_bn_act(x, conv, bn, alpha=None, pre_add=None, residual=None):
    if bn.training or not _FUSED_TRAIN_FWD:
        return _bn_act(_conv_train(x, conv), bn, alpha, pre_add, residual)
    if conv.kernel_size[0] == 3 and conv.dilation[0] != 1:
        raise RuntimeError('mspl_amd: dilated 3x3 convolutions only occur inside EESP (fused branch op)')
    scale, shift = train_fold(bn)
    return ag.conv_bn_prelu(x, conv.weight, conv.stride[0], conv.groups, bn, scale, shift, alpha, pre_add, residual)


def train_fold(bn):
    def build():
        scale = bn.weight * ag.frozen_bn_inv(bn)
        return scale, torch.addcmul(bn.bias, bn.running_mean, scale, value=-1.0)
    return cached(bn, 'tfold', [bn.weight, bn.bias, bn.running_mean, bn.running_var], build)


def prefold_frozen_bn(model):
    bns = [m for m in model.modules() if isinstance(m, nn.BatchNorm2d) and not m.training]
    if not bns:
        return
    with torch.no_grad():
        invs = [ag.frozen_bn_inv(m) for m in bns]
        scales = torch._foreach_mul([m.weight for m in bns], invs)
        shifts = torch._foreach_addcmul([m.bias for m in bns], [m.running_mean for m in bns], scales, value=-1.0)
    for m, sc, sh in zip(bns, scales, shifts):
        store = m.__dict__.setdefault('_mspl_cache', {})
        store['tfold'] = (_key([m.weight, m.bias, m.running_mean, m.running_var]), (sc, sh))


def _conv_fwd(x, conv, ep, out=None, shuffle_groups=0):
    k = conv.kernel_size[0]
    if k == 1:
        return ops.conv1x1(x, conv.weight, conv.groups, ep, out)
    if k == 3 and conv.dilation[0] == 1:
        return ops.conv3x3(x, conv.weight, conv.groups, conv.stride[0], shuffle_groups, ep, out)
    raise RuntimeError('mspl_amd: no kernel for conv k=%d dilation=%d outside an EESP block' % (k, conv.dilation[0]))


class CBR(nn.Module):
    def __init__(self, nIn, nOut, kSize, stride=1, groups=1):
        super().__init__()
        padding = int((kSize - 1) / 2)
        self.conv = nn.Conv2d(nIn, nOut, kSize, stride=stride, padding=padding, bias=False, groups=groups)
        self.bn = nn.BatchNorm2d(nOut)
        self.act = nn.PReLU(nOut)

    def forward(self, input):
        if _training_path():
            return _conv_bn_act(input, self.conv, self.bn, self.act.weight)
        scale, shift = bn_fold(self.bn)
        return _conv_fwd(input, self.conv, Epi(scale, shift, self.act.weight))


class BR(nn.Module):
    def __init__(self, nOut):
        super().__init__()
        self.bn = nn.BatchNorm2d(nOut)
        self.act = nn.PReLU(nOut)

    def forward(self, input):
        if _training_path():
            return _bn_act(input, self.bn, self.act.weight)
        scale, shift = bn_fold(self.bn)
        return ops.pointwise(input, Epi(scale, shift, self.act.weight))


class CB(nn.Module):
    def __init__(self, nIn, nOut, kSize, stride=1, groups=1):
        super().__init__()
        padding = int((kSize - 1) / 2)
        self.conv = nn.Conv2d(nIn, nOut, kSize, stride=stride, padding=padding, bias=False, groups=groups)
        self.bn = nn.BatchNorm2d(nOut)

    def forward(self, input):
        if _training_path():
            return _conv_bn_act(input, self.conv, self.bn)
        scale, shift = bn_fold(self.bn)
        return _conv_fwd(input, self.conv, Epi(scale, shift))


class C(nn.Module):
    def __init__(self, nIn, nOut, kSize, stride=1, groups=1):
        super().__init__()
        padding = int((kSize - 1) / 2)
        self.conv = nn.Conv2d(nIn, nOut, kSize, stride=stride, padding=padding, bias=False, groups=groups)

    def forward(self, input):
        if _training_path():
            return _conv_train(input, self.conv)
        return _conv_fwd(input, self.conv, None)


class CDilated(nn.Module):

    def __init__(self, nIn, nOut, kSize, stride=1, d=1, groups=1):
        super().__init__()
        padding = int((kSize - 1) / 2) * d
        self.conv = nn.Conv2d(nIn, nOut, kSize, stride=stride, padding=padding, bias=False, dilation=d,
                              groups=groups)

    def forward(self, input):
        if _training_path():
            return _conv_train(input, self.conv)
        return _conv_fwd(input, self.conv, None)


class DecCBR(nn.Module):
    def __init__(self, nIn, nOut, kSize, stride=1, dilation=1, groups=1, act_name='prelu'):
        super().__init__()
        if act_name != 'prelu':
            raise NotImplementedError('mspl_amd: only PReLU activations are on the path')
        padding = int((kSize - 1) / 2) * dilation
        self.cbr = nn.Sequential(
            nn.Conv2d(nIn, nOut, kSize, stride=stride, padding=padding, bias=False, groups=groups, dilation=dilation),
            nn.BatchNorm2d(nOut),
            nn.PReLU(nOut))

    def epi(self, **kw):
        scale, shift = bn_fold(self.cbr[1])
        return Epi(scale, shift, self.cbr[2].weight, **kw)

    def forward(self, x):
        if _training_path():
            return _conv_bn_act(x, self.cbr[0], self.cbr[1], self.cbr[2].weight)
        return _conv_fwd(x, self.cbr[0], self.epi())


class DecBR(nn.Module):
    def __init__(self, nOut, act_name='prelu'):
        super().__init__()
        if act_name != 'prelu':
            raise NotImplementedError('mspl_amd: only PReLU activations are on the path')
        self.br = nn.Sequential(nn.BatchNorm2d(nOut), nn.PReLU(nOut))

    def forward(self, x):
        if _training_path():
            return _bn_act(x, self.br[0], self.br[1].weight)
        scale, shift = bn_fold(self.br[0])
        return ops.pointwise(x, Epi(scale, shift, self.br[1].weight))


class Shuffle(nn.Module):

    def __init__(self, groups):
        super().__init__()
        self.groups = groups

    def forward(self, x):
        n, c, h, w = x.shape
        return x.view(n, self.groups, c // self.groups, h, w).transpose(1, 2).contiguous().view(n, c, h, w)


def eesp_dilations(r_lim, k=4):
    ks = sorted((3 + 2 * i) if (3 + 2 * i) <= r_lim else 3 for i in range(k))
    return [(s - 1) // 2 for s in ks]


class EESP(nn.Module):
    def __init__(self, nIn, nOut, stride=1, k=4, r_lim=7, down_method='esp'):
        super().__init__()
        self.stride = stride
        n = int(nOut / k)
        n1 = nOut - (k - 1) * n
        assert down_method in ['avg', 'esp'], 'One of these is suppported (avg or esp)'
        assert n == n1, "n(={}) and n1(={}) should be equal for Depth-wise Convolution ".format(n, n1)
        if k != 4:
            raise NotImplementedError('mspl_amd: the fused EESP kernel is built for k=4 branches')
        self.proj_1x1 = CBR(nIn, n, 1, stride=1, groups=k)
        self.dilations = eesp_dilations(r_lim, k)
        self.spp_dw = nn.ModuleList(CDilated(n, n, kSize=3, stride=stride, groups=n, d=d) for d in self.dilations)
        self.conv_1x1_exp = CB(nOut, nOut, 1, 1, groups=k)
        self.br_after_cat = BR(nOut)
        self.module_act = nn.PReLU(nOut)
        self.downAvg = True if down_method == 'avg' else False
        self.k = k

    def _dw_weights(self):
        ws = [m.conv.weight for m in self.spp_dw]
        return cached(self, 'w4', ws, lambda: torch.stack([w.reshape(-1, 3, 3) for w in ws]).contiguous())

    def _dw_exp_packed(self, H, W):
        br, exp = self.br_after_cat, self.conv_1x1_exp
        deps = [m.conv.weight for m in self.spp_dw] + [br.bn.weight, br.bn.bias, br.bn.running_mean, br.bn.running_var,
                                                      br.act.weight, exp.conv.weight]

        def build():
            bs, bb = bn_fold(br.bn)
            return ops.eesp_dw_exp_pack(self._dw_weights(), bs, bb, br.act.weight, exp.conv.weight, H, W, self.dilations)
        return cached(self, 'dwexp%dx%d' % (H, W), deps, build)

    def reduce_transform(self, input):
        scale, shift = bn_fold(self.br_after_cat.bn)
        pj = self.proj_1x1
        if ops.eesp_proj_dw_hff_fits(input.shape, pj.conv.out_channels, pj.conv.groups, self.dilations, self.stride):
            ps, pb = bn_fold(pj.bn)
            return ops.eesp_proj_dw_hff(input, pj.conv.weight, ps, pb, pj.act.weight, self._dw_weights(), self.dilations,
                                        pj.conv.groups, Epi(scale, shift, self.br_after_cat.act.weight))
        return self.transform(pj(input))

    def transform(self, o1):
        scale, shift = bn_fold(self.br_after_cat.bn)
        return ops.eesp_dw_hff(o1, self._dw_weights(), self.dilations, self.stride,
                               Epi(scale, shift, self.br_after_cat.act.weight))

    def _forward_train(self, input):
        pj, br, exp = self.proj_1x1, self.br_after_cat, self.conv_1x1_exp
        if _FUSED_EESP_TRAIN and not (pj.bn.training or br.bn.training or exp.bn.training):
            strided_avg = self.stride == 2 and self.downAvg
            residual = (not strided_avg) and self.stride == 1 and exp.conv.out_channels == input.shape[1]
            cfg = {'stride': self.stride, 'dil': tuple(self.dilations), 'groups': pj.conv.groups, 'residual': residual}
            ws = [m.conv.weight for m in self.spp_dw]
            folds = [ag.frozen_bn_fold(bn, *train_fold(bn)) for bn in (pj.bn, br.bn, exp.bn)]
            return ag.EESPFn.apply(input, cfg, *folds, pj.conv.weight, pj.bn.weight, pj.bn.bias,
                                   pj.act.weight, ws[0], ws[1], ws[2], ws[3], br.bn.weight, br.bn.bias, br.act.weight,
                                   exp.conv.weight, exp.bn.weight, exp.bn.bias, None if strided_avg else self.module_act.weight)
        has_res = self.stride == 1 and exp.conv.out_channels == input.shape[1] and not (self.stride == 2 and self.downAvg)
        skip = input
        if has_res and pj.bn.training and _CONV_SKIP and input.requires_grad:
            z1, skip = ag.conv_skip(input, pj.conv.weight, pj.conv.groups)
            o1 = _bn_act(z1, pj.bn, pj.act.weight)
        else:
            o1 = self.proj_1x1(input)
        if br.bn.training and _EESP_DW_BN and o1.requires_grad:
            cat = ag.eesp_dw_bn(o1, [m.conv.weight for m in self.spp_dw], self.dilations, br.bn, br.act.weight, self.stride)
        else:
            cat = ag.eesp_dw(o1, [m.conv.weight for m in self.spp_dw], self.dilations, self.stride)
            cat = self.br_after_cat(cat)
        if self.stride == 2 and self.downAvg:
            return _conv_bn_act(cat, exp.conv, exp.bn)
        return _conv_bn_act(cat, exp.conv, exp.bn, self.module_act.weight, residual=skip if has_res else None)

    def _fused_dw_exp(self, shape):
        exp = self.conv_1x1_exp
        return (self.stride == 1 and exp.conv.out_channels == shape[1] and _FUSED_DW_EXP
                and ops.eesp_dw_exp_fits((shape[0], self.proj_1x1.conv.out_channels) + tuple(shape[2:]), self.dilations))

    def _next_proj(self):
        pj = self.proj_1x1
        ps, pb = bn_fold(pj.bn)
        return cached(self, 'nextproj', [pj.conv.weight], lambda: ops.eesp_dw_exp_next_pack(pj.conv.weight)), ps, pb, pj.act.weight

    def forward(self, input, _reduced=None, _next=None):
        if _training_path():
            return self._forward_train(input)
        exp = self.conv_1x1_exp
        if self._fused_dw_exp(input.shape):
            o1 = self.proj_1x1(input) if _reduced is None else _reduced
            scale, shift = bn_fold(exp.bn)
            ep = Epi(scale, shift, self.module_act.weight, residual=input)
            packed = self._dw_exp_packed(input.shape[2], input.shape[3])
            nxt = _next is not None and _FUSED_NEXT_PROJ and _next._fused_dw_exp(input.shape) \
                and _next.proj_1x1.conv.out_channels == self.proj_1x1.conv.out_channels and _next.proj_1x1.conv.groups == 4
            if nxt:
                return ops.eesp_dw_exp(o1, packed, self.dilations, ep, next_proj=_next._next_proj())
            y = ops.eesp_dw_exp(o1, packed, self.dilations, ep)
            return (y, None) if _next is not None else y
        if _next is not None:
            return self.forward(input), None
        cat = self.reduce_transform(input)
        scale, shift = bn_fold(self.conv_1x1_exp.bn)
        if self.stride == 2 and self.downAvg:
            return ops.conv1x1(cat, self.conv_1x1_exp.conv.weight, self.k, Epi(scale, shift))
        residual = input if (self.stride == 1 and self.conv_1x1_exp.conv.out_channels == input.shape[1]) else None
        return ops.conv1x1(cat, self.conv_1x1_exp.conv.weight, self.k,
                           Epi(scale, shift, self.module_act.weight, residual=residual))


def run_eesp_chain(blocks, x):
    blocks = list(blocks)
    if _training_path():
        for m in blocks:
            x = m(x)
        return x
    reduced = None
    for i, m in enumerate(blocks):
        nxt = blocks[i + 1] if i + 1 < len(blocks) else None
        if nxt is None:
            x = m(x, _reduced=reduced)
        else:
            x, reduced = m(x, _reduced=reduced, _next=nxt)
    return x


class ImagePyramid:

    def __init__(self, image):
        self.levels = [image]

    def at_height(self, h):
        i = 1
        while True:
            if i == len(self.levels):
                prev = self.levels[-1]
                if prev.shape[2] == 1 and prev.shape[3] == 1:
                    raise RuntimeError('mspl_amd: image pyramid never reaches height %d' % h)
                self.levels.append(ops.avgpool3x3s2(prev))
            if self.levels[i].shape[2] == h:
                return self.levels[i]
            i += 1


class DownSampler(nn.Module):
    def __init__(self, nin, nout, k=4, r_lim=9, reinf=True):
        super().__init__()
        nout_new = nout - nin
        self.eesp = EESP(nin, nout_new, stride=2, k=k, r_lim=r_lim, down_method='avg')
        self.avg = nn.AvgPool2d(kernel_size=3, padding=1, stride=2)
        if reinf:
            self.inp_reinf = nn.Sequential(
                CBR(config_inp_reinf, config_inp_reinf, 3, 1),
                CB(config_inp_reinf, nout, 1, 1))
        self.act = nn.PReLU(nout)
        self.nin, self.nout = nin, nout

    def _epilogue_vectors(self, with_reinf):
        bn = self.eesp.conv_1x1_exp.bn
        deps = [bn.weight, bn.bias, bn.running_mean, bn.running_var]
        if with_reinf:
            cb = self.inp_reinf[1]
            deps += [cb.conv.weight, cb.bn.weight, cb.bn.bias, cb.bn.running_mean, cb.bn.running_var]

        def build():
            es, eb = bn_fold(bn)
            scale = torch.cat([torch.ones(self.nin, device=es.device), es])
            shift = torch.cat([torch.zeros(self.nin, device=es.device), eb])
            rw = None
            if with_reinf:
                rs, rb = bn_fold(cb.bn)
                rw = (cb.conv.weight.reshape(self.nout, config_inp_reinf) * rs[:, None]).contiguous()
                shift = shift + rb
            return scale.contiguous(), shift.contiguous(), rw
        return cached(self, 'epi%d' % int(with_reinf), deps, build)

    def _forward_train(self, input, input2, alias=None):
        avg_out = ag.avgpool(input)
        eesp_out = self.eesp(input if alias is None else alias)
        reinf = None
        if input2 is not None:
            with torch.no_grad():
                pyr = input2 if isinstance(input2, ImagePyramid) else ImagePyramid(input2)
                img = pyr.at_height(avg_out.shape[2])
            if img.shape[3] != avg_out.shape[3]:
                raise RuntimeError('The size of tensor a (%d) must match the size of tensor b (%d) at non-singleton '
                                   'dimension 3' % (avg_out.shape[3], img.shape[3]))
            reinf = self.inp_reinf(img)
        return ag.down_tail(avg_out, eesp_out, self.act.weight, reinf)

    def forward(self, input, input2=None, _alias=None):
        if _training_path():
            return self._forward_train(input, input2, _alias)
        N, _, H, W = input.shape
        Ho, Wo = (H - 1) // 2 + 1, (W - 1) // 2 + 1
        out = torch.empty((N, self.nout, Ho, Wo), device=input.device, dtype=torch.float32)
        r = None
        if input2 is not None:
            pyr = input2 if isinstance(input2, ImagePyramid) else ImagePyramid(input2)
            with fork(0, (pyr.levels[0],)):
                r = self.inp_reinf[0](pyr.at_height(Ho))
            if r.shape[3] != Wo:
                raise RuntimeError('The size of tensor a (%d) must match the size of tensor b (%d) at non-singleton '
                                   'dimension 3' % (Wo, r.shape[3]))
        pj = self.eesp.proj_1x1
        if _FUSED_DOWN_HEAD and ops.down_head_fits(input.shape, pj.conv.out_channels, pj.conv.groups):
            join(0, (r,))
            scale, shift, rw = self._epilogue_vectors(r is not None)
            ep = Epi(scale, shift, self.act.weight, reinf_r=r, reinf_w=rw)
            ps, pb = bn_fold(pj.bn)
            o1, sums = ops.down_head(input, pj.conv.weight, ps, pb, pj.act.weight, pj.conv.groups, ep, out)
            _remember_plane_sums(input, sums)
            cat = self.eesp.transform(o1)
            ops.conv1x1(cat, self.eesp.conv_1x1_exp.conv.weight, self.eesp.k, ep, out=(out, self.nin))
            return out
        cat = self.eesp.reduce_transform(input)
        join(0, (r,))
        scale, shift, rw = self._epilogue_vectors(r is not None)
        ep = Epi(scale, shift, self.act.weight, reinf_r=r, reinf_w=rw)
        _, sums = ops.avgpool3x3s2(input, ep, out=(out, 0), plane_sums=True)
        _remember_plane_sums(input, sums)
        ops.conv1x1(cat, self.eesp.conv_1x1_exp.conv.weight, self.eesp.k, ep, out=(out, self.nin))
        return out


_PLANE_SUMS = weakref.WeakKeyDictionary()


class _TensorKey(object):
    __slots__ = ('__weakref__',)


def _remember_plane_sums(t, sums):
    key = getattr(t, '_mspl_key', None)
    if key is None:
        key = _TensorKey()
        t._mspl_key = key
    _PLANE_SUMS[key] = (t.data_ptr(), t._version, sums)


def _recall_plane_sums(t):
    key = getattr(t, '_mspl_key', None)
    hit = _PLANE_SUMS.get(key) if key is not None else None
    if hit is None or hit[0] != t.data_ptr() or hit[1] != t._version:
        return None
    return hit[2]


class EfficientPyrPool(nn.Module):
    def __init__(self, in_planes, proj_planes, out_planes, scales=[2.0, 1.5, 1.0, 0.5, 0.1], last_layer_br=True):
        super().__init__()
        scales = sorted(scales, reverse=True)
        self.stages = nn.ModuleList()
        self.projection_layer = DecCBR(in_planes, proj_planes, 1, 1)
        for _ in scales:
            self.stages.append(nn.Conv2d(proj_planes, proj_planes, kernel_size=3, stride=1, padding=1, bias=False,
                                         groups=proj_planes))
        self.merge_layer = nn.Sequential(
            DecBR(proj_planes * len(scales)),
            Shuffle(groups=len(scales)),
            DecCBR(proj_planes * len(scales), proj_planes, 3, 1, groups=proj_planes),
            nn.Conv2d(proj_planes, out_planes, kernel_size=1, stride=1, bias=not last_layer_br))
        if last_layer_br:
            self.br = DecBR(out_planes)
        self.last_layer_br = last_layer_br
        self.scales = scales
        self.proj_planes = proj_planes

    def _final_epilogue(self):
        conv = self.merge_layer[3]
        if not self.last_layer_br:
            return Epi(shift=conv.bias)
        bn, act = self.br.br[0], self.br.br[1]
        scale, shift = bn_fold(bn)
        return Epi(scale, shift, act.weight)

    def branch_sizes(self, height, width):
        return [(max(int(math.ceil(height * s)), 5), max(int(math.ceil(width * s)), 5)) for s in self.scales]

    def _fusable(self, sizes, height, width):
        for hs, ws in sizes:
            up, down = (hs >= height and ws >= width), (hs <= height and ws <= width)
            if not (up or down) or hs > 4 * height or ws > 4 * width:
                return False
        return len(sizes) <= 5

    def forward_unfused(self, x):
        N, P, height, width = x.shape
        S = len(self.scales)
        cat = torch.empty((N, P * S, height, width), device=x.device, dtype=torch.float32)
        br = self.merge_layer[0].br
        bscale, bshift = bn_fold(br[0])
        ep = Epi(bscale, bshift, br[1].weight)
        for i, (stage, (h_s, w_s)) in enumerate(zip(self.stages, self.branch_sizes(height, width))):
            dst = (cat, i * P)
            if self.scales[i] < 1.0:
                h = ops.adaptive_avgpool(x, (h_s, w_s))
                h = ops.conv3x3(h, stage.weight, P)
                ops.bilinear(h, (height, width), ep, out=dst)
            elif self.scales[i] > 1.0:
                h = ops.bilinear(x, (h_s, w_s))
                h = ops.conv3x3(h, stage.weight, P)
                ops.adaptive_avgpool(h, (height, width), ep, out=dst)
            else:
                ops.conv3x3(x, stage.weight, P, ep=ep, out=dst)
        mcbr = self.merge_layer[2]
        return ops.conv3x3(cat, mcbr.cbr[0].weight, P, 1, shuffle_groups=S, ep=mcbr.epi())

    def forward_fused(self, x, sizes):
        N, P, height, width = x.shape
        stage_ws, down_es = [], []
        down = [i for i, (h_s, w_s) in enumerate(sizes) if self.scales[i] < 1.0 and (h_s, w_s) != (height, width)]
        prepped = {}
        if down and ops.pyr_down_prep_fits(x.shape, [sizes[i] for i in down]):
            maps = ops.pyr_down_prep(x, [sizes[i] for i in down], [self.stages[i].weight for i in down])
            prepped = dict(zip(down, maps))
        for i, (stage, (h_s, w_s)) in enumerate(zip(self.stages, sizes)):
            if i in down:
                stage_ws.append(None)
                down_es.append(prepped[i] if i in prepped else
                               ops.conv3x3(ops.adaptive_avgpool(x, (h_s, w_s)), stage.weight, P))
            else:
                stage_ws.append(stage.weight)
                down_es.append(None)
        br = self.merge_layer[0].br
        bscale, bshift = bn_fold(br[0])
        mcbr = self.merge_layer[2]
        return ops.pyrpool_fused(x, sizes, stage_ws, down_es, bscale, bshift, br[1].weight, mcbr.cbr[0].weight,
                                 mcbr.epi())

    def _body_train_fused(self, x, sizes):
        bn0, act0 = self.merge_layer[0].br[0], self.merge_layer[0].br[1]
        mcbr = self.merge_layer[2].cbr
        conv2, bn2, act2 = mcbr[0], mcbr[1], mcbr[2]
        folds = [ag.frozen_bn_fold(bn, *train_fold(bn)) for bn in (bn0, bn2)]
        return ag.PyrBodyFn.apply(x, sizes, *folds, bn0.weight, bn0.bias, act0.weight, conv2.weight, bn2.weight,
                                  bn2.bias, act2.weight, *[st.weight for st in self.stages])

    def _body_train_bn(self, x, sizes):
        bn0, act0 = self.merge_layer[0].br[0], self.merge_layer[0].br[1]
        mcbr = self.merge_layer[2].cbr
        conv2, bn2, act2 = mcbr[0], mcbr[1], mcbr[2]
        return ag.PyrBodyBNFn.apply(x, sizes, ag.bn_train_params(bn0, x.device), ag.bn_train_params(bn2, x.device), bn0.weight, bn0.bias,
                                    act0.weight, conv2.weight, bn2.weight, bn2.bias, act2.weight, *[st.weight for st in self.stages])

    def _forward_train(self, x):
        x = self.projection_layer(x)
        height, width = x.shape[2:]
        P = self.proj_planes
        sizes = self.branch_sizes(height, width)
        bn0, bn2 = self.merge_layer[0].br[0], self.merge_layer[2].cbr[1]
        frozen = not (bn0.training or bn2.training)
        both_train = bn0.training and bn2.training
        if _FUSED_PYR_TRAIN and (frozen or both_train) and ag.pyr_body_fits(x.shape, sizes) and (frozen or (height * width) % 4 == 0):
            out = self._body_train_fused(x, sizes) if frozen else self._body_train_bn(x, sizes)
            conv = self.merge_layer[3]
            if self.last_layer_br:
                return _conv_bn_act(out, conv, self.br.br[0], self.br.br[1].weight)
            return ag.conv_affine_prelu(out, conv.weight, 1, 1, None, conv.bias, None)
        hs = []
        xs = ag.fan_out(x, len(self.stages))
        for xb, stage, sc, (h_s, w_s) in zip(xs, self.stages, self.scales, self.branch_sizes(height, width)):
            if sc < 1.0:
                h = ag.adaptive_avgpool(xb, (h_s, w_s))
                h = ag.conv(h, stage.weight, 1, P)
                h = ag.bilinear(h, (height, width))
            elif sc > 1.0:
                h = ag.bilinear(xb, (h_s, w_s))
                h = ag.conv(h, stage.weight, 1, P)
                h = ag.adaptive_avgpool(h, (height, width))
            else:
                h = ag.conv(xb, stage.weight, 1, P)
            hs.append(h)
        out = self.merge_layer[0](torch.cat(hs, 1))
        out = self.merge_layer[1](out)
        out = self.merge_layer[2](out)
        conv = self.merge_layer[3]
        if self.last_layer_br:
            return _conv_bn_act(out, conv, self.br.br[0], self.br.br[1].weight)
        if _FUSED_TRAIN_FWD:
            return ag.conv_affine_prelu(out, conv.weight, 1, 1, None, conv.bias, None)
        return ag.affine_prelu(ag.conv(out, conv.weight, 1, 1), None, conv.bias, None)

    def forward(self, x, fused=True, projected=False, planes=False):
        if _training_path():
            return self._forward_train(x)
        if not projected:
            x = self.projection_layer(x)
        height, width = x.shape[2:]
        sizes = self.branch_sizes(height, width)
        ok = fused and self._fusable(sizes, height, width) and all(
            (s >= 1.0) or (hs <= height and ws <= width) for s, (hs, ws) in zip(self.scales, sizes))
        m = self.forward_fused(x, sizes) if ok else self.forward_unfused(x)
        if planes and _FUSED_HEAD_CLASSIFIER and not self.last_layer_br:
            return m, self.merge_layer[3].weight, self.merge_layer[3].bias
        return ops.conv1x1(m, self.merge_layer[3].weight, 1, self._final_epilogue())


class EfficientPWConv(nn.Module):
    def __init__(self, nin, nout):
        super().__init__()
        self.wt_layer = nn.Sequential(
            nn.AdaptiveAvgPool2d(output_size=1),
            nn.Conv2d(nin, nout, kernel_size=1, stride=1, padding=0, groups=1, bias=False),
            nn.Sigmoid())
        self.groups = math.gcd(nin, nout)
        self.expansion_layer = DecCBR(nin, nout, kSize=3, stride=1, groups=self.groups)
        self.out_size = nout
        self.in_size = nin

    def forward(self, x, _alias=None):
        if _training_path():
            gate = ag.gap_gate(x, self.wt_layer[1].weight)
            return ag.channel_scale(self.expansion_layer(x if _alias is None else _alias), gate)
        return self.expand(x, self.gate(x))

    def gate(self, x):
        sums = _recall_plane_sums(x)
        if sums is not None:
            return ops.gate_from_sums(sums, self.wt_layer[1].weight, x.shape[2] * x.shape[3])
        return ops.gap_gate(x, self.wt_layer[1].weight)

    def expand(self, x, gate):
        return ops.conv3x3(x, self.expansion_layer.cbr[0].weight, self.groups, ep=self.expansion_layer.epi(gate=gate))

    def __repr__(self):
        return '%s(in_channels=%d, out_channels=%d)' % (self.__class__.__name__, self.in_size, self.out_size)


def decoder_stage_fusable(merge, enc, pyr):
    return (_FUSED_DEC_MERGE and not _training_path() and
            ops.decoder_merge_shape_ok(merge.in_size, merge.out_size, pyr.proj_planes, enc.shape[2], enc.shape[3]))


def decoder_stage_fused(merge, enc, gate, bu_lowres, br_seq, pyr):
    if tuple(enc.shape[2:]) != (bu_lowres.shape[2] * 2, bu_lowres.shape[3] * 2):
        raise RuntimeError('The size of tensor a (%d) must match the size of tensor b (%d) at non-singleton dimension 2'
                           % (enc.shape[2], bu_lowres.shape[2] * 2))
    exp, proj = merge.expansion_layer.cbr, pyr.projection_layer.cbr
    return ops.decoder_merge(enc, bu_lowres, exp[0].weight, tuple(bn_fold(exp[1])) + (exp[2].weight,), gate,
                             tuple(bn_fold(br_seq[0])) + (br_seq[1].weight,), proj[0].weight, tuple(bn_fold(proj[1])) + (proj[2].weight,))


def decoder_merge(pw_out, bu_lowres, br_seq):
    size = (bu_lowres.shape[2] * 2, bu_lowres.shape[3] * 2)
    if tuple(pw_out.shape[2:]) != size:
        raise RuntimeError('The size of tensor a (%d) must match the size of tensor b (%d) at non-singleton dimension 2'
                           % (pw_out.shape[2], size[0]))
    if _training_path():
        return _bn_act(ag.bilinear(bu_lowres, size), br_seq[0], br_seq[1].weight, pre_add=pw_out)
    scale, shift = bn_fold(br_seq[0])
    return ops.bilinear(bu_lowres, size, Epi(scale, shift, br_seq[1].weight, pre_add=pw_out))
```

mspl_amd/ops.py:

```python
import ctypes
import math

import torch

from . import _native as nat
from ._native import Epilogue, check, lib


def _stream():
    return ctypes.c_void_p(torch.cuda.current_stream().cuda_stream)


def _f32(t, name):
    if not isinstance(t, torch.Tensor) or not t.is_cuda:
        raise RuntimeError('mspl_amd: %s must be a CUDA (ROCm) tensor; there is no CPU path' % name)
    if t.dtype != torch.float32:
        raise RuntimeError('mspl_amd: %s must be float32, got %s' % (name, t.dtype))
    if not t.is_contiguous():
        t = t.contiguous()
    return t


def _p(t):
    return None if t is None else ctypes.c_void_p(t.data_ptr())


def _vec(t, n, name):
    if t is None:
        return None
    t = _f32(t, name)
    if t.numel() != n:
        raise RuntimeError('mspl_amd: %s has %d elements, expected %d' % (name, t.numel(), n))
    return t


class Epi:
    __slots__ = ('scale', 'shift', 'alpha', 'pre_add', 'residual', 'reinf_r', 'reinf_w', 'gate', 'raw_out')

    def __init__(self, scale=None, shift=None, alpha=None, pre_add=None, residual=None, reinf_r=None,
                 reinf_w=None, gate=None, raw_out=None):
        self.scale, self.shift, self.alpha = scale, shift, alpha
        self.pre_add, self.residual = pre_add, residual
        self.reinf_r, self.reinf_w, self.gate = reinf_r, reinf_w, gate
        self.raw_out = raw_out


import threading
_LAUNCH = threading.local()


class launch_flags(object):

    def __init__(self, throughput=False, k2_stream=None):
        self.value = nat.LAUNCH_THROUGHPUT if throughput else 0
        if k2_stream is not None:
            self.value |= nat.LAUNCH_K2_STREAM_FORCE if k2_stream else nat.LAUNCH_K2_STREAM_OFF

    def __enter__(self):
        self.prev = getattr(_LAUNCH, 'flags', 0)
        _LAUNCH.flags = self.value
        return self

    def __exit__(self, *exc):
        _LAUNCH.flags = self.prev


def current_launch_flags():
    return getattr(_LAUNCH, 'flags', 0)


def _build(ep, out, coff, N, C, hw):
    ctot = out.shape[1]
    if coff < 0 or coff + C > ctot:
        raise RuntimeError('mspl_amd: channel slice [%d,%d) outside destination with %d channels' % (coff, coff + C, ctot))
    s = Epilogue()
    s.struct_size = ctypes.sizeof(Epilogue)
    s.flags = current_launch_flags()
    s.out_ctot, s.out_coff = ctot, coff
    keep = []
    if ep is not None:
        for f in ('scale', 'shift', 'alpha'):
            v = _vec(getattr(ep, f), ctot, f)
            keep.append(v)
            setattr(s, f, None if v is None else v.data_ptr())
        for f in ('pre_add', 'residual'):
            v = getattr(ep, f)
            if v is not None:
                v = _f32(v, f)
                if v.numel() != N * ctot * hw:
                    raise RuntimeError('mspl_amd: %s shape %s does not match destination %s' % (f, tuple(v.shape), tuple(out.shape)))
                keep.append(v)
                setattr(s, f, v.data_ptr())
        if ep.reinf_r is not None:
            r = _vec(ep.reinf_r, N * 3 * hw, 'reinf_r')
            w = _vec(ep.reinf_w, ctot * 3, 'reinf_w')
            keep += [r, w]
            s.reinf_r, s.reinf_w = r.data_ptr(), w.data_ptr()
        if ep.gate is not None:
            g = _vec(ep.gate, N * ctot, 'gate')
            keep.append(g)
            s.gate = g.data_ptr()
        if ep.raw_out is not None:
            r = ep.raw_out
            if not r.is_cuda or r.dtype != torch.float32 or not r.is_contiguous() or r.numel() != N * C * hw or coff != 0 or ctot != C:
                raise RuntimeError('mspl_amd: raw_out must be a contiguous float32 CUDA tensor of the (un-sliced) destination shape')
            keep.append(r)
            s.raw_out = r.data_ptr()
    return s, keep


def _dest(out, shape, like):
    if out is None:
        return torch.empty(shape, device=like.device, dtype=torch.float32), 0
    dst, coff = out
    if (dst.shape[0],) + tuple(dst.shape[2:]) != (shape[0],) + tuple(shape[2:]) or not dst.is_contiguous() \
            or dst.dtype != torch.float32 or not dst.is_cuda:
        raise RuntimeError('mspl_amd: destination %s incompatible with result %s' % (tuple(dst.shape), tuple(shape)))
    return dst, coff


def eesp_dw_hff(x, w4, dil, stride, ep=None, out=None):
    x, w4 = _f32(x, 'x'), _f32(w4, 'w4')
    N, n, H, W = x.shape
    if tuple(w4.shape) != (4, n, 3, 3):
        raise RuntimeError('mspl_amd: eesp_dw_hff weight %s, expected (4,%d,3,3)' % (tuple(w4.shape), n))
    Ho, Wo = (H - 1) // stride + 1, (W - 1) // stride + 1
    dst, coff = _dest(out, (N, 4 * n, Ho, Wo), x)
    s, keep = _build(ep, dst, coff, N, 4 * n, Ho * Wo)
    d = (ctypes.c_int32 * 4)(*[int(v) for v in dil])
    check(lib.mspl_eesp_dw_hff_fwd(_p(x), _p(w4), d, stride, N, n, H, W, ctypes.byref(s), _p(dst), _stream()))
    return dst


def eesp_proj_dw_hff_fits(shape, n, groups, dilations, stride):
    if stride != 1:
        return False
    N, Cin, H, W = [int(v) for v in shape]
    d = (ctypes.c_int32 * 4)(*[int(v) for v in dilations])
    return bool(lib.mspl_eesp_proj_dw_hff_fits(N, Cin, int(n), int(groups), H, W, d, current_launch_flags()))


def eesp_proj_dw_hff(x, wproj, pscale, pshift, palpha, w4, dilations, groups, ep=None, out=None):
    x = _f32(x, 'x')
    N, Cin, H, W = x.shape
    wproj = _f32(wproj, 'projection weight')
    n = wproj.shape[0]
    w4 = _vec(w4, 4 * n * 9, 'w')
    ps, pb, pa = _vec(pscale, n, 'pscale'), _vec(pshift, n, 'pshift'), _vec(palpha, n, 'palpha')
    dst, coff = _dest(out, (N, 4 * n, H, W), x)
    s, keep = _build(ep, dst, coff, N, 4 * n, H * W)
    d = (ctypes.c_int32 * 4)(*[int(v) for v in dilations])
    check(lib.mspl_eesp_proj_dw_hff_fwd(_p(x), _p(wproj), _p(ps), _p(pb), _p(pa), _p(w4), d, N, Cin, n, int(groups), H, W,
                                        ctypes.byref(s), _p(dst), _stream()))
    return dst


def eesp_dw_exp_fits(shape, dilations):
    N, n, H, W = [int(v) for v in shape]
    d = (ctypes.c_int32 * 4)(*[int(v) for v in dilations])
    return bool(lib.mspl_eesp_dw_exp_fits(N, n, H, W, d, current_launch_flags()))


def eesp_dw_exp_pack(w4, bscale, bshift, balpha, wexp, H, W, dilations):
    w4 = _f32(w4, 'w4')
    n = w4.shape[1]
    if tuple(w4.shape) != (4, n, 3, 3):
        raise RuntimeError('mspl_amd: eesp_dw_exp weight %s, expected (4,%d,3,3)' % (tuple(w4.shape), n))
    bs, bb, ba = _vec(bscale, 4 * n, 'bscale'), _vec(bshift, 4 * n, 'bshift'), _vec(balpha, 4 * n, 'balpha')
    wexp = _vec(wexp, 4 * n * n, 'expansion weight')
    packed = torch.empty(int(lib.mspl_eesp_dw_exp_pack_floats(n)), device=w4.device, dtype=torch.float32)
    d = (ctypes.c_int32 * 4)(*[int(v) for v in dilations])
    check(lib.mspl_eesp_dw_exp_pack(_p(w4), _p(bs), _p(bb), _p(ba), _p(wexp), n, int(H), int(W), d, _p(packed), _stream()))
    return packed


def eesp_dw_exp_next_pack(w1):
    w1 = _f32(w1, 'next projection weight')
    n = w1.shape[0]
    if w1.numel() != n * n:
        raise RuntimeError('mspl_amd: next projection weight %s, expected (%d,%d)' % (tuple(w1.shape), n, n))
    packed = torch.empty(int(lib.mspl_eesp_dw_exp_next_pack_floats(n)), device=w1.device, dtype=torch.float32)
    check(lib.mspl_eesp_dw_exp_next_pack(_p(w1), n, _p(packed), _stream()))
    return packed


def eesp_dw_exp(r, packed, dilations, ep, next_proj=None):
    r = _f32(r, 'r')
    N, n, H, W = r.shape
    packed = _vec(packed, int(lib.mspl_eesp_dw_exp_pack_floats(n)), 'packed')
    dst = torch.empty((N, 4 * n, H, W), device=r.device, dtype=torch.float32)
    s, keep = _build(ep, dst, 0, N, 4 * n, H * W)
    d = (ctypes.c_int32 * 4)(*[int(v) for v in dilations])
    if next_proj is None:
        check(lib.mspl_eesp_dw_exp_fwd(_p(r), _p(packed), d, N, n, H, W, ctypes.byref(s), _p(dst), _stream()))
        return dst
    npk = _vec(next_proj[0], int(lib.mspl_eesp_dw_exp_next_pack_floats(n)), 'next_packed')
    ns, nb, na = _vec(next_proj[1], n, 'nscale'), _vec(next_proj[2], n, 'nshift'), _vec(next_proj[3], n, 'nalpha')
    rn = torch.empty((N, n, H, W), device=r.device, dtype=torch.float32)
    check(lib.mspl_eesp_dw_exp_next_fwd(_p(r), _p(packed), d, N, n, H, W, ctypes.byref(s), _p(dst), _p(npk), _p(ns), _p(nb), _p(na), _p(rn),
                                        _stream()))
    return dst, rn


def conv1x1(x, w, groups=1, ep=None, out=None):
    x, w = _f32(x, 'x'), _f32(w, 'w')
    N, Cin, H, W = x.shape
    Cout = w.shape[0]
    if w.numel() != Cout * (Cin // groups) or Cin % groups or Cout % groups:
        raise RuntimeError('mspl_amd: conv1x1 weight %s does not match Cin=%d groups=%d' % (tuple(w.shape), Cin, groups))
    dst, coff = _dest(out, (N, Cout, H, W), x)
    s, keep = _build(ep, dst, coff, N, Cout, H * W)
    check(lib.mspl_conv1x1_fwd(_p(x), _p(w), N, Cin, Cout, groups, H * W, ctypes.byref(s), _p(dst), _stream()))
    return dst


def conv3x3(x, w, groups=1, stride=1, shuffle_groups=0, ep=None, out=None):
    x, w = _f32(x, 'x'), _f32(w, 'w')
    N, Cin, H, W = x.shape
    Cout = w.shape[0]
    if tuple(w.shape[2:]) != (3, 3) or Cin % groups or Cout % groups or w.shape[1] != Cin // groups:
        raise RuntimeError('mspl_amd: conv3x3 weight %s does not match Cin=%d groups=%d' % (tuple(w.shape), Cin, groups))
    Ho, Wo = (H - 1) // stride + 1, (W - 1) // stride + 1
    dst, coff = _dest(out, (N, Cout, Ho, Wo), x)
    s, keep = _build(ep, dst, coff, N, Cout, Ho * Wo)
    check(lib.mspl_conv3x3_fwd(_p(x), _p(w), N, Cin, Cout, groups, H, W, stride, shuffle_groups, ctypes.byref(s),
                               _p(dst), _stream()))
    return dst


def pack_dense_weight(w):
    w = _f32(w, 'w')
    Cout, Cin, kh, kw = w.shape
    return w.permute(2, 3, 0, 1).reshape(kh * kw, Cout, Cin).contiguous()


def dense_conv(x, w_packed, ksize, dilation=1, ep=None, out=None):
    x, w_packed = _f32(x, 'x'), _f32(w_packed, 'w_packed')
    N, Cin, H, W = x.shape
    taps = ksize * ksize
    if w_packed.dim() != 3 or w_packed.shape[0] != taps or w_packed.shape[2] != Cin:
        raise RuntimeError('mspl_amd: dense_conv packed weight %s does not match k=%d Cin=%d' % (tuple(w_packed.shape), ksize, Cin))
    Cout = w_packed.shape[1]
    dst, coff = _dest(out, (N, Cout, H, W), x)
    s, keep = _build(ep, dst, coff, N, Cout, H * W)
    check(lib.mspl_dense_conv_fwd(_p(x), _p(w_packed), N, Cin, Cout, H, W, ksize, int(dilation), ctypes.byref(s), _p(dst),
                                  _stream()))
    return dst


def pack_dense_weight_split(w, planes):
    if not isinstance(w, torch.Tensor) or w.dim() != 4 or w.shape[2] != w.shape[3] or w.dtype != torch.float32:
        raise RuntimeError('mspl_amd: pack_dense_weight_split takes a float32 (Cout, Cin, k, k) weight')
    if planes not in (2, 3):
        raise RuntimeError('mspl_amd: pack_dense_weight_split: %r planes (2 or 3)' % (planes,))
    Cout, Cin, k, _ = w.shape
    r = w.detach().permute(2, 3, 0, 1).reshape(k * k, Cout, Cin)
    out = torch.empty((planes, k * k, Cout, Cin), device=w.device, dtype=torch.bfloat16)
    for p in range(planes):
        out[p] = r.to(torch.bfloat16)
        r = r - out[p].to(torch.float32)
    return out


def dense_conv_split_fits(Cin, Cout, ksize, planes):
    return bool(lib.mspl_dense_conv_split_fits(int(Cin), int(Cout), int(ksize), int(planes)))


def dense_conv_split(x, w_split, ksize, dilation=1, ep=None, out=None):
    x = _f32(x, 'x')
    if not isinstance(w_split, torch.Tensor) or not w_split.is_cuda or w_split.dtype != torch.bfloat16 or not w_split.is_contiguous():
        raise RuntimeError('mspl_amd: dense_conv_split weights must be a contiguous CUDA (ROCm) bfloat16 tensor from pack_dense_weight_split')
    N, Cin, H, W = x.shape
    taps = ksize * ksize
    if w_split.dim() != 4 or w_split.shape[1] != taps or w_split.shape[3] != Cin:
        raise RuntimeError('mspl_amd: dense_conv_split weight %s does not match k=%d Cin=%d' % (tuple(w_split.shape), ksize, Cin))
    planes, Cout = w_split.shape[0], w_split.shape[2]
    dst, coff = _dest(out, (N, Cout, H, W), x)
    s, keep = _build(ep, dst, coff, N, Cout, H * W)
    check(lib.mspl_dense_conv_split_fwd(_p(x), _p(w_split), N, Cin, Cout, H, W, ksize, int(dilation), planes, ctypes.byref(s), _p(dst),
                                        _stream()))
    return dst


def pack_dense_weight_dgrad(w):
    if w.dim() != 4 or w.shape[2] != w.shape[3] or w.dtype != torch.float32:
        raise RuntimeError('mspl_amd: pack_dense_weight_dgrad takes a float32 (Cout, Cin, k, k) weight, got %s %s' % (tuple(w.shape), w.dtype))
    Cout, Cin, k, _ = w.shape
    return w.flip(2, 3).permute(2, 3, 1, 0).reshape(k * k, Cin, Cout).contiguous()


def unpack_dense_weight(wp, ksize):
    taps, Cout, Cin = wp.shape
    return wp.view(ksize, ksize, Cout, Cin).permute(2, 3, 0, 1)


def dense_conv_wgrad(gy, x, ksize, dilation=1, want_bias=True, split=0, out_bias=None):
    gy, x = _f32(gy, 'gy'), _f32(x, 'x')
    N, Cin, H, W = x.shape
    Cout = gy.shape[1]
    if (gy.shape[0],) + tuple(gy.shape[2:]) != (N, H, W):
        raise RuntimeError('mspl_amd: dense_conv_wgrad gy %s does not match x %s' % (tuple(gy.shape), tuple(x.shape)))
    args = (N, Cin, Cout, H, W, int(ksize), int(dilation), int(split))
    nbytes = int(lib.mspl_dense_conv_wgrad_workspace_bytes(*args))
    if nbytes < 0:
        check(nbytes)
    ws = torch.empty((nbytes + 3) // 4, device=x.device, dtype=torch.float32) if nbytes else None
    dw = torch.empty((ksize * ksize, Cout, Cin), device=x.device, dtype=torch.float32)
    db = None
    if want_bias:
        db = out_bias if out_bias is not None else torch.empty(Cout, device=x.device, dtype=torch.float32)
    check(lib.mspl_dense_conv_wgrad(_p(gy), _p(x), *args, _p(ws), nbytes, _p(dw), _p(db), _stream()))
    return dw, db


def dense_conv_dgrad(gys, wts, ksizes, dilations, out=None):
    gys = [_f32(g, 'gy') for g in gys]
    wts = [_f32(w, 'wt_packed') for w in wts]
    n = len(gys)
    N, Cg, H, W = gys[0].shape
    Cx = wts[0].shape[1]
    for g, w, k in zip(gys, wts, ksizes):
        if tuple(g.shape) != (N, Cg, H, W) or tuple(w.shape) != (k * k, Cx, Cg):
            raise RuntimeError('mspl_amd: dense_conv_dgrad gy %s / weights %s do not match (N,%d,%d,%d) / (k*k,%d,%d)'
                               % (tuple(g.shape), tuple(w.shape), Cg, H, W, Cx, Cg))
    if out is None:
        gx = torch.empty((N, Cx, H, W), device=gys[0].device, dtype=torch.float32)
    else:
        gx, _ = _dest((out, 0), (N, Cx, H, W), gys[0])
        if gx.shape[1] != Cx:
            raise RuntimeError('mspl_amd: dense_conv_dgrad destination %s, expected %d channels' % (tuple(gx.shape), Cx))
    arr = lambda ts: (ctypes.c_void_p * n)(*[t.data_ptr() for t in ts])
    ints = lambda vs: (ctypes.c_int32 * n)(*[int(v) for v in vs])
    check(lib.mspl_dense_conv_dgrad(arr(gys), arr(wts), ints(ksizes), ints(dilations), n, N, Cg, Cx, H, W, int(out is not None), _p(gx),
                                    _stream()))
    return gx


def avgpool3x3s2(x, ep=None, out=None, plane_sums=False):
    x = _f32(x, 'x')
    N, C, H, W = x.shape
    Ho, Wo = (H - 1) // 2 + 1, (W - 1) // 2 + 1
    dst, coff = _dest(out, (N, C, Ho, Wo), x)
    s, keep = _build(ep, dst, coff, N, C, Ho * Wo)
    if not plane_sums:
        check(lib.mspl_avgpool3x3s2_fwd(_p(x), N, C, H, W, ctypes.byref(s), _p(dst), _stream()))
        return dst
    nblk = lib.mspl_avgpool3x3s2_psum_blocks(H, W)
    if nblk <= 0:
        check(nblk)
    sums = torch.empty((N * C, nblk), device=x.device, dtype=torch.float32)
    check(lib.mspl_avgpool3x3s2_psum_fwd(_p(x), N, C, H, W, ctypes.byref(s), _p(dst), _p(sums), _stream()))
    return dst, sums


def down_head_fits(shape, n, groups):
    N, nin, H, W = [int(v) for v in shape]
    return bool(lib.mspl_down_head_fits(N, nin, int(n), int(groups), H, W, current_launch_flags()))


def down_head(x, wproj, pscale, pshift, palpha, groups, ep, out):
    x, wproj = _f32(x, 'x'), _f32(wproj, 'projection weight')
    N, nin, H, W = x.shape
    n = wproj.shape[0]
    if wproj.numel() != n * (nin // groups) or nin % groups or n % groups:
        raise RuntimeError('mspl_amd: down_head weight %s does not match nin=%d groups=%d' % (tuple(wproj.shape), nin, groups))
    ps, pb, pa = _vec(pscale, n, 'pscale'), _vec(pshift, n, 'pshift'), _vec(palpha, n, 'palpha')
    dst, coff = _dest((out, 0), (N, nin, H // 2, W // 2), x)
    s, keep = _build(ep, dst, coff, N, nin, (H // 2) * (W // 2))
    nblk = lib.mspl_down_head_psum_blocks(H, W)
    if nblk <= 0:
        check(nblk)
    r = torch.empty((N, n, H, W), device=x.device, dtype=torch.float32)
    sums = torch.empty((N * nin, nblk), device=x.device, dtype=torch.float32)
    check(lib.mspl_down_head_fwd(_p(x), _p(wproj), _p(ps), _p(pb), _p(pa), N, nin, n, int(groups), H, W, ctypes.byref(s), _p(r),
                                 _p(dst), _p(sums), _stream()))
    return r, sums


def gate_from_sums(plane_sums, w, hw):
    w = _f32(w, 'w')
    Cout = w.shape[0]
    Cin = w.numel() // Cout
    planes, nblk = plane_sums.shape
    N = planes // Cin
    if planes != N * Cin or plane_sums.dtype != torch.float32 or not plane_sums.is_contiguous():
        raise RuntimeError('mspl_amd: gate_from_sums: sums %s do not match Cin=%d' % (tuple(plane_sums.shape), Cin))
    gate = torch.empty((N, Cout), device=w.device, dtype=torch.float32)
    check(lib.mspl_gate_from_sums_fwd(_p(plane_sums), _p(w), N, Cin, Cout, nblk, int(hw), _p(gate), _stream()))
    return gate


def decoder_merge_shape_ok(Cin, Cout, P, H, W):
    groups = math.gcd(Cin, Cout)
    cg, cob = Cin // groups, Cout // groups
    if H % 2 or W % 2 or H < 2 or W < 2 or P not in (2, 6, 10, 16) or Cout > 1024:
        return False
    return (cg, cob) in ((1, 1), (8, 3)) or ((cg, cob) == (4, 1) and groups >= 16 and W % 4 == 0 and 16 <= W <= 256 and H >= 4)


def decoder_merge(enc, bu, w3, e_epi, gate, b_epi, wp, p_epi):
    enc, bu, w3, wp = _f32(enc, 'enc'), _f32(bu, 'bu'), _f32(w3, 'w3'), _f32(wp, 'wp')
    N, Cin, H, W = enc.shape
    Cout, P = w3.shape[0], wp.shape[0]
    if tuple(bu.shape) != (N, Cout, H // 2, W // 2) or H % 2 or W % 2:
        return None
    groups = math.gcd(Cin, Cout)
    if tuple(w3.shape) != (Cout, Cin // groups, 3, 3) or wp.numel() != P * Cout:
        raise RuntimeError('mspl_amd: decoder_merge weights %s / %s do not match Cin=%d Cout=%d'
                           % (tuple(w3.shape), tuple(wp.shape), Cin, Cout))
    gate = _vec(gate, N * Cout, 'gate')
    es, eb, ea = [_vec(t, Cout, 'expansion epilogue') for t in e_epi]
    bs, bb, ba = [_vec(t, Cout, 'bu_br epilogue') for t in b_epi]
    ps, pb, pa = [_vec(t, P, 'projection epilogue') for t in p_epi]
    if any(t is None for t in (es, eb, ea, bs, bb, ba, ps, pb, pa)):
        return None
    dst = torch.empty((N, P, H, W), device=enc.device, dtype=torch.float32)
    rc = lib.mspl_decoder_merge_fwd(_p(enc), _p(bu), _p(w3), _p(es), _p(eb), _p(ea), _p(gate), _p(bs), _p(bb), _p(ba), _p(wp),
                                    _p(ps), _p(pb), _p(pa), N, Cin, Cout, P, H, W, _p(dst), _stream())
    if rc == nat.ERR_UNSUPPORTED:
        return None
    check(rc)
    return dst


def bilinear(x, size, ep=None, out=None, align_corners=True):
    x = _f32(x, 'x')
    N, C, H, W = x.shape
    Ho, Wo = int(size[0]), int(size[1])
    dst, coff = _dest(out, (N, C, Ho, Wo), x)
    s, keep = _build(ep, dst, coff, N, C, Ho * Wo)
    check(lib.mspl_bilinear_fwd(_p(x), N, C, H, W, Ho, Wo, 1 if align_corners else 0, ctypes.byref(s), _p(dst), _stream()))
    return dst


def adaptive_avgpool(x, size, ep=None, out=None):
    x = _f32(x, 'x')
    N, C, H, W = x.shape
    Ho, Wo = int(size[0]), int(size[1])
    dst, coff = _dest(out, (N, C, Ho, Wo), x)
    s, keep = _build(ep, dst, coff, N, C, Ho * Wo)
    check(lib.mspl_adaptive_avgpool_fwd(_p(x), N, C, H, W, Ho, Wo, ctypes.byref(s), _p(dst), _stream()))
    return dst


def pointwise(x, ep, out=None):
    x = _f32(x, 'x')
    N, C = x.shape[:2]
    hw = x[0, 0].numel()
    dst = torch.empty_like(x) if out is None else out
    s, keep = _build(ep, dst, 0, N, C, hw)
    check(lib.mspl_pointwise_fwd(_p(x), N, C, hw, ctypes.byref(s), _p(dst), _stream()))
    return dst


def pyrpool_merge(zcat, scale, shift, alpha, merge_w, out=None):
    zcat, merge_w = _f32(zcat, 'zcat'), _f32(merge_w, 'merge_w')
    N, C, h, w = zcat.shape
    P, nb = merge_w.shape[:2]
    if C != P * nb or tuple(merge_w.shape[2:]) != (3, 3) or any(t.numel() != C for t in (scale, shift, alpha)):
        raise RuntimeError('mspl_amd: pyrpool_merge operands do not match: zcat %s merge_w %s' % (tuple(zcat.shape), tuple(merge_w.shape)))
    dst = torch.empty((N, P, h, w), device=zcat.device, dtype=torch.float32) if out is None else out
    check(lib.mspl_pyrpool_merge_fwd(_p(zcat), N, P, h, w, nb, _p(_f32(scale, 'scale')), _p(_f32(shift, 'shift')), _p(_f32(alpha, 'alpha')),
                                     _p(merge_w), _p(dst), _stream()))
    return dst


def gap_gate(x, w):
    x, w = _f32(x, 'x'), _f32(w, 'w')
    N, Cin, H, W = x.shape
    Cout = w.shape[0]
    if w.numel() != Cout * Cin:
        raise RuntimeError('mspl_amd: gap_gate weight %s does not match Cin=%d' % (tuple(w.shape), Cin))
    ws = torch.empty((N, Cin), device=x.device, dtype=torch.float32)
    gate = torch.empty((N, Cout), device=x.device, dtype=torch.float32)
    check(lib.mspl_gap_gate_fwd(_p(x), _p(w), N, Cin, Cout, H * W, _p(ws), _p(gate), _stream()))
    return gate


def fusion_gate(z, rgb, depth):
    rgb, depth = _f32(rgb, 'rgb'), _f32(depth, 'depth')
    if rgb.shape != depth.shape or (z is not None and z.shape != rgb.shape):
        raise RuntimeError('mspl_amd: fusion_gate operands differ in shape: %s %s %s'
                           % (tuple(rgb.shape), tuple(depth.shape), None if z is None else tuple(z.shape)))
    out = torch.empty_like(rgb)
    check(lib.mspl_fusion_gate_fwd(None if z is None else _p(_f32(z, 'z')), _p(rgb), _p(depth), rgb.numel(), _p(out),
                                   _stream()))
    return out


def pyr_down_prep_fits(shape, sizes):
    nb = len(sizes)
    N, P, h, w = [int(v) for v in shape]
    if nb < 1 or nb > 4 or any(int(s[0]) > h or int(s[1]) > w for s in sizes):
        return False
    hs = (ctypes.c_int32 * nb)(*[int(s[0]) for s in sizes])
    ws = (ctypes.c_int32 * nb)(*[int(s[1]) for s in sizes])
    return lib.mspl_pyr_down_prep_lds_bytes(N, P, h, w, nb, hs, ws) > 0


def pyr_down_prep(x, sizes, stage_ws, keep_pooled=False):
    x = _f32(x, 'x')
    N, P, h, w = x.shape
    nb = len(sizes)
    hs = (ctypes.c_int32 * nb)(*[int(s[0]) for s in sizes])
    ws = (ctypes.c_int32 * nb)(*[int(s[1]) for s in sizes])
    sw, op, pp = (ctypes.c_void_p * nb)(), (ctypes.c_void_p * nb)(), (ctypes.c_void_p * nb)()
    outs, pools, keep = [], [], []
    for i in range(nb):
        t = _f32(stage_ws[i], 'stage weight')
        if t.numel() != P * 9:
            raise RuntimeError('mspl_amd: pyramid stage weight %s, expected (%d,1,3,3)' % (tuple(t.shape), P))
        keep.append(t)
        sw[i] = t.data_ptr()
        o = torch.empty((N, P, int(sizes[i][0]), int(sizes[i][1])), device=x.device, dtype=torch.float32)
        outs.append(o)
        op[i] = o.data_ptr()
        if keep_pooled:
            pools.append(torch.empty_like(o))
            pp[i] = pools[-1].data_ptr()
    if keep_pooled:
        check(lib.mspl_pyr_down_prep_train_fwd(_p(x), N, P, h, w, nb, hs, ws, sw, op, pp, _stream()))
        return outs, pools
    check(lib.mspl_pyr_down_prep_fwd(_p(x), N, P, h, w, nb, hs, ws, sw, op, _stream()))
    return outs


def pyrpool_fused(x, sizes, stage_ws, down_es, br_scale, br_shift, br_alpha, merge_w, ep=None, out=None):
    x = _f32(x, 'x')
    N, P, h, w = x.shape
    nb = len(sizes)
    merge_w = _f32(merge_w, 'merge_w')
    if tuple(merge_w.shape) != (P, nb, 3, 3):
        raise RuntimeError('mspl_amd: pyrpool merge weight %s, expected (%d,%d,3,3)' % (tuple(merge_w.shape), P, nb))
    hs = (ctypes.c_int32 * nb)(*[int(s[0]) for s in sizes])
    ws = (ctypes.c_int32 * nb)(*[int(s[1]) for s in sizes])
    keep = []
    sw, de = (ctypes.c_void_p * nb)(), (ctypes.c_void_p * nb)()
    for i in range(nb):
        if stage_ws[i] is not None:
            t = _f32(stage_ws[i], 'stage weight')
            if t.numel() != P * 9:
                raise RuntimeError('mspl_amd: pyrpool stage weight %s, expected (%d,1,3,3)' % (tuple(t.shape), P))
            keep.append(t)
            sw[i] = t.data_ptr()
        if down_es[i] is not None:
            t = _f32(down_es[i], 'down map')
            if tuple(t.shape) != (N, P, int(sizes[i][0]), int(sizes[i][1])):
                raise RuntimeError('mspl_amd: pyrpool low-res map %s does not match branch size %s' % (tuple(t.shape), sizes[i]))
            keep.append(t)
            de[i] = t.data_ptr()
    bs, bh, ba = _vec(br_scale, nb * P, 'br_scale'), _vec(br_shift, nb * P, 'br_shift'), _vec(br_alpha, nb * P, 'br_alpha')
    dst, coff = _dest(out, (N, P, h, w), x)
    s, k2 = _build(ep, dst, coff, N, P, h * w)
    check(lib.mspl_pyrpool_fused_fwd(_p(x), N, P, h, w, nb, hs, ws, sw, de, _p(bs), _p(bh), _p(ba), _p(merge_w),
                                     ctypes.byref(s), _p(dst), _stream()))
    return dst


def label_epilogue(main, aux, size, lut=None, want_labels=True, want_prob=False, want_kld=False,
                   want_logits=False):
    main = _f32(main, 'main')
    N, C, Hm, Wm = main.shape
    Ha = Wa = 0
    if aux is not None:
        aux = _f32(aux, 'aux')
        if aux.shape[0] != N or aux.shape[1] != C:
            raise RuntimeError('mspl_amd: aux logits %s do not match main %s' % (tuple(aux.shape), tuple(main.shape)))
        Ha, Wa = aux.shape[2:]
    H, W = int(size[0]), int(size[1])
    dev = main.device
    res = {}
    if lut is not None:
        if lut.dtype != torch.uint8 or not lut.is_cuda or lut.numel() < C:
            raise RuntimeError('mspl_amd: lut must be a CUDA uint8 tensor with >= %d entries' % C)
    if want_labels:
        res['labels'] = torch.empty((N, H, W), device=dev, dtype=torch.uint8)
    if want_prob:
        res['prob'] = torch.empty((N, C, H, W), device=dev, dtype=torch.float32)
    if want_kld:
        res['kld'] = torch.empty((N, H, W), device=dev, dtype=torch.float32)
    if want_logits:
        res['main_up'] = torch.empty((N, C, H, W), device=dev, dtype=torch.float32)
        if aux is not None:
            res['aux_up'] = torch.empty((N, C, H, W), device=dev, dtype=torch.float32)
    check(lib.mspl_label_epilogue_fwd(_p(main), _p(aux), N, C, Hm, Wm, Ha, Wa, H, W, _p(lut), _p(res.get('labels')),
                                      _p(res.get('prob')), _p(res.get('kld')), _p(res.get('main_up')),
                                      _p(res.get('aux_up')), _stream()))
    return res


def label_epilogue_hist_fits(main, aux, size):
    N, C, Hm, Wm = [int(v) for v in main.shape]
    Ha, Wa = ([int(v) for v in aux.shape[2:]] if aux is not None else (0, 0))
    return bool(lib.mspl_label_epilogue_hist_fits(N, C, Hm, Wm, Ha, Wa, int(size[0]), int(size[1])))


def label_epilogue_hist(main, aux, size, hist, num_classes, lut=None, want_kld=False):
    main = _f32(main, 'main')
    N, C, Hm, Wm = main.shape
    Ha = Wa = 0
    if aux is not None:
        aux = _f32(aux, 'aux')
        if aux.shape[0] != N or aux.shape[1] != C:
            raise RuntimeError('mspl_amd: aux logits %s do not match main %s' % (tuple(aux.shape), tuple(main.shape)))
        Ha, Wa = aux.shape[2:]
    H, W = int(size[0]), int(size[1])
    if hist.dtype != torch.int64 or not hist.is_cuda or hist.numel() < num_classes:
        raise RuntimeError('mspl_amd: hist must be a CUDA int64 tensor with >= num_classes entries')
    if lut is not None and (lut.dtype != torch.uint8 or not lut.is_cuda or lut.numel() < C):
        raise RuntimeError('mspl_amd: lut must be a CUDA uint8 tensor with >= %d entries' % C)
    res = {'labels': torch.empty((N, H, W), device=main.device, dtype=torch.uint8)}
    if want_kld:
        res['kld'] = torch.empty((N, H, W), device=main.device, dtype=torch.float32)
    nbytes = int(lib.mspl_label_epilogue_hist_workspace_bytes(N, H, W))
    ws = torch.empty(max(nbytes, 4), device=main.device, dtype=torch.uint8)
    check(lib.mspl_label_epilogue_hist_fwd(_p(main), _p(aux), N, C, Hm, Wm, Ha, Wa, H, W, _p(lut), _p(res['labels']),
                                           _p(res.get('kld')), _p(hist), int(num_classes), _p(ws), nbytes, _stream()))
    return res


def _head_planes(head, what):
    planes, weight, bias = head
    planes, weight, bias = _f32(planes, what + ' planes'), _f32(weight, what + ' weight'), _f32(bias, what + ' bias')
    N, P, h, w = [int(v) for v in planes.shape]
    C = int(weight.shape[0])
    if weight.numel() != C * P or bias.numel() != C:
        raise RuntimeError('mspl_amd: %s classifier %s / bias %s does not match %d planes' %
                           (what, tuple(weight.shape), tuple(bias.shape), P))
    return planes, weight, bias, (N, P, C, h, w)


def label_epilogue_planes_fits(main, aux, size):
    N, P, Hm, Wm = [int(v) for v in main[0].shape]
    C = int(main[1].shape[0])
    Ha, Wa = ([int(v) for v in aux[0].shape[2:]] if aux is not None else (0, 0))
    if aux is not None and (int(aux[0].shape[1]) != P or int(aux[1].shape[0]) != C):
        return False
    return bool(lib.mspl_label_epilogue_planes_fits(N, P, C, Hm, Wm, Ha, Wa, int(size[0]), int(size[1])))


def label_epilogue_planes(main, aux, size, hist=None, num_classes=0, lut=None, want_kld=False):
    mp, mw, mbias, (N, P, C, Hm, Wm) = _head_planes(main, 'main')
    ap = aw = abias = None
    Ha = Wa = 0
    if aux is not None:
        ap, aw, abias, (Na, Pa, Ca, Ha, Wa) = _head_planes(aux, 'aux')
        if (Na, Pa, Ca) != (N, P, C):
            raise RuntimeError('mspl_amd: aux head (N=%d, P=%d, C=%d) does not match main (N=%d, P=%d, C=%d)' % (Na, Pa, Ca, N, P, C))
    H, W = int(size[0]), int(size[1])
    if hist is not None and (hist.dtype != torch.int64 or not hist.is_cuda or hist.numel() < num_classes):
        raise RuntimeError('mspl_amd: hist must be a CUDA int64 tensor with >= num_classes entries')
    if lut is not None and (lut.dtype != torch.uint8 or not lut.is_cuda or lut.numel() < C):
        raise RuntimeError('mspl_amd: lut must be a CUDA uint8 tensor with >= %d entries' % C)
    res = {'labels': torch.empty((N, H, W), device=mp.device, dtype=torch.uint8)}
    if want_kld:
        res['kld'] = torch.empty((N, H, W), device=mp.device, dtype=torch.float32)
    ws, nbytes = None, 0
    if hist is not None:
        nbytes = int(lib.mspl_label_epilogue_hist_workspace_bytes(N, H, W))
        ws = torch.empty(max(nbytes, 4), device=mp.device, dtype=torch.uint8)
    check(lib.mspl_label_epilogue_planes_fwd(_p(mp), _p(mw), _p(mbias), _p(ap), _p(aw), _p(abias), N, P, C, Hm, Wm, Ha, Wa, H, W,
                                             _p(lut), _p(res['labels']), _p(res.get('kld')), _p(hist), int(num_classes), _p(ws),
                                             nbytes, _stream()))
    return res


def merge_labels(sources, num_classes, thresh, fill=4, hist=None):
    S = len(sources)
    if S < 1:
        raise RuntimeError('mspl_amd: merge_labels needs at least one source')
    src = []
    for t in sources:
        if t.dtype != torch.uint8 or not t.is_cuda:
            raise RuntimeError('mspl_amd: merge_labels sources must be CUDA uint8 tensors')
        if t.shape != sources[0].shape:
            raise RuntimeError('mspl_amd: merge_labels sources differ in shape')
        src.append(t.contiguous())
    out = torch.empty_like(src[0])
    if hist is not None and (hist.dtype != torch.int64 or not hist.is_cuda or hist.numel() < num_classes):
        raise RuntimeError('mspl_amd: hist must be a CUDA int64 tensor with >= num_classes entries')
    arr = (ctypes.c_void_p * S)(*[t.data_ptr() for t in src])
    check(lib.mspl_merge_labels_fwd(arr, S, out.numel(), num_classes, int(thresh), int(fill), _p(out), _p(hist),
                                    _stream()))
    return out
```

Before: 21820 images/s.

## Precompute pyramid-pool interpolation coefficient tables once and stream them from memory

The streaming pyramid-pool kernel used to recompute the bilinear/stencil coefficient tables (At row coefficients, Gt column coefficients) in every block before doing any work, with a barrier in between. A one-time table-build kernel now stores these geometry-only coefficients in a device buffer, cached per module and shape. A TAB variant of the kernel loads them into registers and LDS and allows longer row segments (SEGMAX 72). This removes per-block setup ALU and LDS traffic and lets each block cover more rows, at the cost of extra global reads, register pressure and a table registry lookup on the host.

```diff
diff --git a/include/mspl_hip.h b/include/mspl_hip.h
--- a/include/mspl_hip.h
+++ b/include/mspl_hip.h
@@ -124,6 +124,30 @@
                            const float* const* down_e, const float* br_scale, const float* br_shift,
                            const float* br_alpha, const float* merge_w, const mspl_epilogue_t* ep,
                            float* out, void* stream);
+int64_t mspl_pyr_stream_tables_bytes(int32_t h, int32_t w, int32_t nb, const int32_t* hs, const int32_t* ws);
+int mspl_pyr_stream_tables_build(int32_t h, int32_t w, int32_t nb, const int32_t* hs, const int32_t* ws, float* tables,
+                                 int64_t bytes, void* stream);
+int mspl_pyrpool_fused_tab_fwd(const float* x, int32_t N, int32_t P, int32_t h, int32_t w, int32_t nb,
+                               const int32_t* hs, const int32_t* ws, const float* const* stage_w,
+                               const float* const* down_e, const float* br_scale, const float* br_shift,
+                               const float* br_alpha, const float* merge_w, const float* ep_scale, const float* ep_shift,
+                               const float* ep_alpha, int32_t out_ctot, int32_t out_coff, uint32_t launch_flags, float* out,
+                               const float* tables, void* stream);
+#define MSPL_PYR_STREAM_PLAN_TAKEN 0
+#define MSPL_PYR_STREAM_PLAN_T0 1
+#define MSPL_PYR_STREAM_PLAN_T1 2
+#define MSPL_PYR_STREAM_PLAN_PXL 3
+#define MSPL_PYR_STREAM_PLAN_NCB 4
+#define MSPL_PYR_STREAM_PLAN_CBW 5
+#define MSPL_PYR_STREAM_PLAN_SEG 6
+#define MSPL_PYR_STREAM_PLAN_NSEG 7
+#define MSPL_PYR_STREAM_PLAN_WAVES 8
+#define MSPL_PYR_STREAM_PLAN_SEG_INKERNEL 9
+#define MSPL_PYR_STREAM_PLAN_NSEG_INKERNEL 10
+#define MSPL_PYR_STREAM_PLAN_WAVES_INKERNEL 11
+#define MSPL_PYR_STREAM_PLAN_LEN 12
+int mspl_pyrpool_stream_plan(int32_t N, int32_t P, int32_t h, int32_t w, int32_t nb, const int32_t* hs, const int32_t* ws,
+                             int32_t* out);
 
 int mspl_pyrpool_fused_train_fwd(const float* x, int32_t N, int32_t P, int32_t h, int32_t w, int32_t nb,
                                  const int32_t* hs, const int32_t* ws, const float* const* stage_w,
diff --git a/mspl_amd/csrc/pyrpool.hip b/mspl_amd/csrc/pyrpool.hip
--- a/mspl_amd/csrc/pyrpool.hip
+++ b/mspl_amd/csrc/pyrpool.hip
@@ -341,7 +341,11 @@
 int pyrpool_stream_try(const float* x, int N, int P, int h, int w, int nb, const int32_t* hs, const int32_t* ws,
                        const float* const* stage_w, const float* const* down_e, const float* br_scale,
                        const float* br_shift, const float* br_alpha, const float* merge_w, const Epi& e, float* out,
-                       hipStream_t stream, float* zcat = nullptr);
+                       hipStream_t stream, float* zcat = nullptr, const float* tab = nullptr);
+int pyrpool_stream_tables_build(int h, int w, int nb, const int32_t* hs, const int32_t* ws, float* tab, int64_t bytes,
+                                hipStream_t stream);
+int64_t pyrpool_stream_tables_bytes(int h, int w, int nb, const int32_t* hs, const int32_t* ws);
+void pyrpool_stream_plan(int N, int P, int h, int w, int nb, const int32_t* hs, const int32_t* ws, int32_t* out);
 
 }
 
@@ -351,7 +355,7 @@
                                const int32_t* hs, const int32_t* ws, const float* const* stage_w,
                                const float* const* down_e, const float* br_scale, const float* br_shift,
                                const float* br_alpha, const float* merge_w, const mspl_epilogue_t* ep,
-                               float* out, float* zcat, void* stream, bool dry = false) {
+                               float* out, float* zcat, void* stream, bool dry = false, const float* tab = nullptr) {
     MSPL_REQUIRE(dry || (x && hs && ws && stage_w && down_e && br_scale && br_shift && br_alpha && merge_w && out),
                  MSPL_ERR_NULL_POINTER, "pyrpool_fused: null pointer");
     MSPL_REQUIRE(hs && ws, MSPL_ERR_NULL_POINTER, "pyrpool_fused: null pointer");
@@ -362,7 +366,7 @@
         static const int force_tables = MSPL_TUNE_INT("MSPL_PYR_TABLES", 0);
         if (!force_tables) {
             const int rc3 = pyrpool_stream_try(x, N, P, h, w, nb, hs, ws, stage_w, down_e, br_scale, br_shift, br_alpha, merge_w,
-                                               make_epi(ep, P, h * w), out, (hipStream_t)stream, zcat);
+                                               make_epi(ep, P, h * w), out, (hipStream_t)stream, zcat, tab);
             if (rc3 <= 0) return rc3;
             if (!zcat) {
                 const int rc = pyrpool_sep_try(x, N, P, h, w, nb, hs, ws, stage_w, down_e, br_scale, br_shift, br_alpha, merge_w,
@@ -450,6 +454,41 @@
                                 stream);
 }
 
+extern "C" int mspl_pyrpool_fused_tab_fwd(const float* x, int32_t N, int32_t P, int32_t h, int32_t w, int32_t nb,
+                                          const int32_t* hs, const int32_t* ws, const float* const* stage_w,
+                                          const float* const* down_e, const float* br_scale, const float* br_shift,
+                                          const float* br_alpha, const float* merge_w, const float* ep_scale,
+                                          const float* ep_shift, const float* ep_alpha, int32_t out_ctot, int32_t out_coff,
+                                          uint32_t launch_flags, float* out, const float* tables, void* stream) {
+    mspl_epilogue_t ep;
+    memset(&ep, 0, sizeof(ep));
+    ep.scale = ep_scale; ep.shift = ep_shift; ep.alpha = ep_alpha;
+    ep.out_ctot = out_ctot; ep.out_coff = out_coff;
+    ep.struct_size = (uint32_t)sizeof(ep); ep.flags = launch_flags;
+    return pyrpool_fused_launch(x, N, P, h, w, nb, hs, ws, stage_w, down_e, br_scale, br_shift, br_alpha, merge_w, &ep, out, nullptr,
+                                stream, false, tables);
+}
+
+extern "C" int64_t mspl_pyr_stream_tables_bytes(int32_t h, int32_t w, int32_t nb, const int32_t* hs, const int32_t* ws) {
+    if (!hs || !ws || h <= 0 || w <= 0) return 0;
+    return pyrpool_stream_tables_bytes(h, w, nb, hs, ws);
+}
+
+extern "C" int mspl_pyr_stream_tables_build(int32_t h, int32_t w, int32_t nb, const int32_t* hs, const int32_t* ws, float* tables,
+                                            int64_t bytes, void* stream) {
+    MSPL_REQUIRE(hs && ws && tables, MSPL_ERR_NULL_POINTER, "pyr_stream_tables: null pointer");
+    MSPL_REQUIRE(h > 0 && w > 0, MSPL_ERR_BAD_SHAPE, "pyr_stream_tables: bad shape %dx%d", h, w);
+    return pyrpool_stream_tables_build(h, w, nb, hs, ws, tables, bytes, (hipStream_t)stream);
+}
+
+extern "C" int mspl_pyrpool_stream_plan(int32_t N, int32_t P, int32_t h, int32_t w, int32_t nb, const int32_t* hs, const int32_t* ws,
+                                        int32_t* out) {
+    MSPL_REQUIRE(hs && ws && out, MSPL_ERR_NULL_POINTER, "pyrpool_stream_plan: null pointer");
+    MSPL_REQUIRE(N > 0 && P > 0 && h > 0 && w > 0, MSPL_ERR_BAD_SHAPE, "pyrpool_stream_plan: bad shape N=%d P=%d %dx%d", N, P, h, w);
+    pyrpool_stream_plan(N, P, h, w, nb, hs, ws, out);
+    return MSPL_OK;
+}
+
 extern "C" int mspl_pyrpool_fused_train_fwd(const float* x, int32_t N, int32_t P, int32_t h, int32_t w, int32_t nb,
                                             const int32_t* hs, const int32_t* ws, const float* const* stage_w,
                                             const float* const* down_e, const float* br_scale, const float* br_shift,
diff --git a/mspl_amd/csrc/pyrpool_stream.hip b/mspl_amd/csrc/pyrpool_stream.hip
--- a/mspl_amd/csrc/pyrpool_stream.hip
+++ b/mspl_amd/csrc/pyrpool_stream.hip
@@ -1,6 +1,8 @@
 #include <stdlib.h>
 
 #include <algorithm>
+#include <mutex>
+#include <unordered_map>
 
 #include "common.hpp"
 #include "pyr_stencil.hpp"
@@ -12,6 +14,8 @@
 #define P3_STEPS 2
 #endif
 constexpr int P3_SEGMAX = 19;
+constexpr int P3_TAB_SEGMAX = 72;
+constexpr int P3_TAB_ACOPY = ((P3_TAB_SEGMAX + 2) * 6 + 127) / 128;
 
 struct Pyr3Geom {
     int N, P, h, w;
@@ -55,8 +59,11 @@
 template <int PXL> struct P3Vec;
 template <> struct P3Vec<1> { typedef float T; };
 template <> struct P3Vec<2> { typedef float2 T; };
-
-template <int T0, int T1, int PXL, bool TRAIN>
+template <int PXL> __device__ __forceinline__ float p3_vec_get(const typename P3Vec<PXL>::T& v, int j);
+template <> __device__ __forceinline__ float p3_vec_get<1>(const float& v, int) { return v; }
+template <> __device__ __forceinline__ float p3_vec_get<2>(const float2& v, int j) { return j == 0 ? v.x : v.y; }
+
+template <int T0, int T1, int PXL, bool TRAIN, bool TAB>
 __global__ __launch_bounds__(256, 2) void pyrpool_stream_kernel(const float* __restrict__ x, const float* __restrict__ sw0,
                                                                 const float* __restrict__ sw1, const float* __restrict__ sw2,
                                                                 const float* __restrict__ de3, const float* __restrict__ de4,
@@ -66,9 +73,8 @@
                                                                 const float* __restrict__ ep_shift,
                                                                 const float* __restrict__ ep_alpha, int ep_ctot, int ep_coff,
                                                                 Pyr3Geom g, float* __restrict__ out, float* __restrict__ zcat,
-                                                                float* __restrict__ mraw) {
-    __shared__ __attribute__((aligned(16))) float At[2][(P3_SEGMAX + 2) * 24];
-    __shared__ float Gt[2][3][PXL][5][64];
+                                                                float* __restrict__ mraw, const float* __restrict__ tab) {
+    __shared__ __attribute__((aligned(16))) float At[2][((TAB ? P3_TAB_SEGMAX : P3_SEGMAX) + 2) * 24];
     __shared__ __attribute__((aligned(16))) float Wm[4][5][12];
     const int lane = threadIdx.x & 63, wave = __builtin_amdgcn_readfirstlane(threadIdx.x >> 6);
     unsigned bid = blockIdx.x;
@@ -81,44 +87,64 @@
     const int px0 = cb * g.CBW + (lane - 1) * PXL;
     const bool writer = lane >= 1 && lane <= 62 && px0 < w;
 
-    if (wave < 2) {
-        const int ri = lane / 3, ky = lane - 3 * ri;
-        if (ri < g.SEG + 2) {
-            float acc[5];
-            if (wave == 0) p3_coeffs<T0>(ys - 1 + ri, ky, h, g.hs[0], g.sh[0], acc);
-            else p3_coeffs<T1>(ys - 1 + ri, ky, h, g.hs[1], g.sh[1], acc);
-            float* d = &At[wave][ri * 24 + ky * 8];
-            d[0] = acc[0]; d[1] = acc[1]; d[2] = acc[2]; d[3] = acc[3]; d[4] = acc[4];
-        }
-    }
-#pragma unroll
-    for (int t = 0; t < 6 * PXL; ++t) {
-        if ((t & 3) == wave) {
-            const int ub = t / (3 * PXL), r = t - ub * 3 * PXL, kx = r / PXL, j = r - kx * PXL;
-            float acc[5];
-            if (ub == 0) p3_coeffs<T0>(px0 + j, kx, w, g.ws[0], g.sw[0], acc);
-            else p3_coeffs<T1>(px0 + j, kx, w, g.ws[1], g.sw[1], acc);
-#pragma unroll
-            for (int q = 0; q < 5; ++q) Gt[ub][kx][j][q][lane] = acc[q];
-        }
-    }
-    __syncthreads();
     float C0[3][PXL][5], C1[3][PXL][5];
-    {
-        const float* w0p = sw0 + (size_t)c * 9;
-        const float* w1p = sw1 + (size_t)c * 9;
-#pragma unroll
-        for (int j = 0; j < PXL; ++j)
-#pragma unroll
-            for (int s2 = 0; s2 < 5; ++s2) {
-                const float a0 = Gt[0][0][j][s2][lane], a1 = Gt[0][1][j][s2][lane], a2 = Gt[0][2][j][s2][lane];
-                const float b0 = Gt[1][0][j][s2][lane], b1 = Gt[1][1][j][s2][lane], b2 = Gt[1][2][j][s2][lane];
-#pragma unroll
-                for (int ky = 0; ky < 3; ++ky) {
-                    C0[ky][j][s2] = fmaf(w0p[ky * 3 + 2], a2, fmaf(w0p[ky * 3 + 1], a1, w0p[ky * 3] * a0));
-                    C1[ky][j][s2] = fmaf(w1p[ky * 3 + 2], b2, fmaf(w1p[ky * 3 + 1], b1, w1p[ky * 3] * b0));
-                }
-            }
+    typedef typename P3Vec<PXL>::T gvec_t;
+    gvec_t Gr[2][3][5];
+    float4 Ar[P3_TAB_ACOPY];
+    if constexpr (!TAB) {
+        __shared__ float Gt[2][3][PXL][5][64];
+        if (wave < 2) {
+            const int ri = lane / 3, ky = lane - 3 * ri;
+            if (ri < g.SEG + 2) {
+                float acc[5];
+                if (wave == 0) p3_coeffs<T0>(ys - 1 + ri, ky, h, g.hs[0], g.sh[0], acc);
+                else p3_coeffs<T1>(ys - 1 + ri, ky, h, g.hs[1], g.sh[1], acc);
+                float* d = &At[wave][ri * 24 + ky * 8];
+                d[0] = acc[0]; d[1] = acc[1]; d[2] = acc[2]; d[3] = acc[3]; d[4] = acc[4];
+            }
+        }
+#pragma unroll
+        for (int t = 0; t < 6 * PXL; ++t) {
+            if ((t & 3) == wave) {
+                const int ub = t / (3 * PXL), r = t - ub * 3 * PXL, kx = r / PXL, j = r - kx * PXL;
+                float acc[5];
+                if (ub == 0) p3_coeffs<T0>(px0 + j, kx, w, g.ws[0], g.sw[0], acc);
+                else p3_coeffs<T1>(px0 + j, kx, w, g.ws[1], g.sw[1], acc);
+#pragma unroll
+                for (int q = 0; q < 5; ++q) Gt[ub][kx][j][q][lane] = acc[q];
+            }
+        }
+        __syncthreads();
+        {
+            const float* w0p = sw0 + (size_t)c * 9;
+            const float* w1p = sw1 + (size_t)c * 9;
+#pragma unroll
+            for (int j = 0; j < PXL; ++j)
+#pragma unroll
+                for (int s2 = 0; s2 < 5; ++s2) {
+                    const float a0 = Gt[0][0][j][s2][lane], a1 = Gt[0][1][j][s2][lane], a2 = Gt[0][2][j][s2][lane];
+                    const float b0 = Gt[1][0][j][s2][lane], b1 = Gt[1][1][j][s2][lane], b2 = Gt[1][2][j][s2][lane];
+#pragma unroll
+                    for (int ky = 0; ky < 3; ++ky) {
+                        C0[ky][j][s2] = fmaf(w0p[ky * 3 + 2], a2, fmaf(w0p[ky * 3 + 1], a1, w0p[ky * 3] * a0));
+                        C1[ky][j][s2] = fmaf(w1p[ky * 3 + 2], b2, fmaf(w1p[ky * 3 + 1], b1, w1p[ky * 3] * b0));
+                    }
+                }
+        }
+    } else {
+        const gvec_t* Gp = reinterpret_cast<const gvec_t*>(tab + 2 * (h + 2) * 24);
+        const int nslots = g.ncb * 62 + 2, slot = cb * 62 + lane;
+#pragma unroll
+        for (int ub = 0; ub < 2; ++ub)
+#pragma unroll
+            for (int kx = 0; kx < 3; ++kx)
+#pragma unroll
+                for (int q = 0; q < 5; ++q)
+                    if (q < (ub == 0 ? T0 : T1)) Gr[ub][kx][q] = Gp[((ub * 3 + kx) * 5 + q) * nslots + slot];
+        const int npc = min(g.SEG + 2, h + 2 - ys) * 6, t7 = threadIdx.x & 127;
+        const float4* Ap = reinterpret_cast<const float4*>(tab) + ((wave >> 1) * (h + 2) + ys) * 6;
+#pragma unroll
+        for (int k = 0; k < P3_TAB_ACOPY; ++k) Ar[k] = Ap[min(t7 + 128 * k, npc - 1)];
     }
     unsigned dxa[2][PXL], dxb[2][PXL];  float dw0[2][PXL], dw1[2][PXL];
 #pragma unroll
@@ -194,6 +220,32 @@
         }
     };
     load_e(ys - 1);
+    if constexpr (TAB) {
+        const int npc = min(g.SEG + 2, h + 2 - ys) * 6, t7 = threadIdx.x & 127;
+        float4* Ad = reinterpret_cast<float4*>(&At[wave >> 1][0]);
+#pragma unroll
+        for (int k = 0; k < P3_TAB_ACOPY; ++k)
+            if (t7 + 128 * k < npc) Ad[t7 + 128 * k] = Ar[k];
+        __syncthreads();
+        const float* w0p = sw0 + (size_t)c * 9;
+        const float* w1p = sw1 + (size_t)c * 9;
+#pragma unroll
+        for (int j = 0; j < PXL; ++j)
+#pragma unroll
+            for (int s2 = 0; s2 < 5; ++s2) {
+                float ga[3], gb[3];
+#pragma unroll
+                for (int kx = 0; kx < 3; ++kx) {
+                    ga[kx] = s2 < T0 ? p3_vec_get<PXL>(Gr[0][kx][s2], j) : 0.f;
+                    gb[kx] = s2 < T1 ? p3_vec_get<PXL>(Gr[1][kx][s2], j) : 0.f;
+                }
+#pragma unroll
+                for (int ky = 0; ky < 3; ++ky) {
+                    C0[ky][j][s2] = fmaf(w0p[ky * 3 + 2], ga[2], fmaf(w0p[ky * 3 + 1], ga[1], w0p[ky * 3] * ga[0]));
+                    C1[ky][j][s2] = fmaf(w1p[ky * 3 + 2], gb[2], fmaf(w1p[ky * 3 + 1], gb[1], w1p[ky * 3] * gb[0]));
+                }
+            }
+    }
     float acc[3][PXL];
 #pragma unroll
     for (int r = 0; r < 3; ++r)
@@ -322,30 +374,94 @@
     }
 }
 
-int pyrpool_stream_try(const float* x, int N, int P, int h, int w, int nb, const int32_t* hs, const int32_t* ws,
-                       const float* const* stage_w, const float* const* down_e, const float* br_scale,
-                       const float* br_shift, const float* br_alpha, const float* merge_w, const Epi& e, float* out,
-                       hipStream_t stream, float* zcat) {
+
+template <int T0, int T1, int PXL>
+__global__ __launch_bounds__(256) void p3_tables_kernel(Pyr3Geom g, float* __restrict__ tab) {
+    const int h = g.h, w = g.w, nslots = g.ncb * 62 + 2;
+    const int na = 2 * (h + 2) * 3, ng = 2 * 3 * nslots * PXL;
+    const int t = blockIdx.x * 256 + threadIdx.x;
+    float acc[5];
+    if (t < na) {
+        const int ub = t / ((h + 2) * 3), r = t - ub * (h + 2) * 3, row = r / 3, ky = r - row * 3;
+        if (ub == 0) p3_coeffs<T0>(row - 1, ky, h, g.hs[0], g.sh[0], acc);
+        else p3_coeffs<T1>(row - 1, ky, h, g.hs[1], g.sh[1], acc);
+        float* d = tab + (ub * (h + 2) + row) * 24 + ky * 8;
+#pragma unroll
+        for (int q = 0; q < 8; ++q) d[q] = q < 5 ? acc[q] : 0.f;
+    } else if (t < na + ng) {
+        const int u = t - na;
+        const int ub = u / (3 * nslots * PXL), r = u - ub * 3 * nslots * PXL, kx = r / (nslots * PXL), r2 = r - kx * nslots * PXL;
+        const int slot = r2 / PXL, j = r2 - slot * PXL;
+        if (ub == 0) p3_coeffs<T0>((slot - 1) * PXL + j, kx, w, g.ws[0], g.sw[0], acc);
+        else p3_coeffs<T1>((slot - 1) * PXL + j, kx, w, g.ws[1], g.sw[1], acc);
+        float* d = tab + 2 * (h + 2) * 24;
+#pragma unroll
+        for (int q = 0; q < 5; ++q) d[(((ub * 3 + kx) * 5 + q) * nslots + slot) * PXL + j] = acc[q];
+    }
+}
+
+struct P3Shape {
+    bool ok;
+    int T0, T1, PXL, ncb, CBW;
+};
+static P3Shape p3_shape(int h, int w, int nb, const int32_t* hs, const int32_t* ws) {
+    P3Shape s;
+    memset(&s, 0, sizeof(s));
     static const int off = (MSPL_TUNE_INT("MSPL_PYR_STREAM", 1) == 0);
     static const int min_w = MSPL_TUNE_INT("MSPL_PYR_STREAM_MINW", 40);
-    if (off || nb != 5 || w < min_w || ((int64_t)N * P) % 4 != 0) return 1;
-    if (e.pre_add || e.residual || e.reinf_r || e.gate) return 1;
-    for (int i = 0; i < 5; ++i) if (hs[i] <= 0 || ws[i] <= 0) return 1;
-    if (!(hs[0] > h && ws[0] > w && hs[1] > h && ws[1] > w)) return 1;
-    if (!(hs[2] == h && ws[2] == w)) return 1;
-    if (!(hs[3] <= h && ws[3] <= w && hs[4] <= h && ws[4] <= w && (hs[3] < h || ws[3] < w) && (hs[4] < h || ws[4] < w))) return 1;
-    if (!stage_w[0] || !stage_w[1] || !stage_w[2] || !down_e[3] || !down_e[4]) return 1;
+    if (off || nb != 5 || w < min_w || h <= 0) return s;
+    for (int i = 0; i < 5; ++i) if (hs[i] <= 0 || ws[i] <= 0) return s;
+    if (!(hs[0] > h && ws[0] > w && hs[1] > h && ws[1] > w)) return s;
+    if (!(hs[2] == h && ws[2] == w)) return s;
+    if (!(hs[3] <= h && ws[3] <= w && hs[4] <= h && ws[4] <= w && (hs[3] < h || ws[3] < w) && (hs[4] < h || ws[4] < w))) return s;
     int taps[2];
     for (int i = 0; i < 2; ++i) {
         const int R = std::max(p3_stencil_radius(h, hs[i]), p3_stencil_radius(w, ws[i]));
-        if (R > 2) return 1;
+        if (R > 2) return s;
         taps[i] = R <= 1 ? 3 : 5;
     }
-    const int PXL = w <= 62 ? 1 : 2;
-    if (PXL == 2 && ((w & 1) || (((uintptr_t)out) & 7) || (((uintptr_t)x) & 7))) return 1;
-    if (zcat && (!e.raw || e.ctot != P || e.coff != 0)) return 1;
-    if (zcat && PXL == 2 && ((((uintptr_t)zcat) | ((uintptr_t)e.raw)) & 7)) return 1;
-    Pyr3Geom g;
+    s.T0 = taps[0]; s.T1 = taps[1];
+    s.PXL = w <= 62 ? 1 : 2;
+    if (s.PXL == 2 && (w & 1)) return s;
+    s.CBW = 62 * s.PXL;
+    s.ncb = ceil_div(w, s.CBW);
+    s.ok = true;
+    return s;
+}
+
+struct P3Plan {
+    bool taken;
+    P3Shape s;
+    int seg_tab, nseg_tab, seg_ik, nseg_ik;
+    int64_t waves_tab, waves_ik;
+};
+static P3Plan p3_plan(int N, int P, int h, int w, int nb, const int32_t* hs, const int32_t* ws) {
+    P3Plan p;
+    memset(&p, 0, sizeof(p));
+    if (N <= 0 || P <= 0 || ((int64_t)N * P) % 4 != 0) return p;
+    p.s = p3_shape(h, w, nb, hs, ws);
+    if (!p.s.ok) return p;
+    const int64_t cols = (int64_t)N * P * p.s.ncb;
+    static const int dbg_seg = MSPL_TUNE_INT("MSPL_PYR_SEG", 0);
+    int seg = std::min(h, P3_SEGMAX);
+    while (seg > 6 && cols * ceil_div(h, seg) < 2048) --seg;
+    seg = ceil_div(h, ceil_div(h, seg));
+    if (dbg_seg > 0 && dbg_seg <= P3_SEGMAX) seg = std::min(dbg_seg, h);
+    p.seg_ik = seg; p.nseg_ik = ceil_div(h, seg); p.waves_ik = cols * p.nseg_ik;
+    static const int min_waves = MSPL_TUNE_INT("MSPL_PYR_TAB_WAVES", 2048);
+    static const int seg_cap = std::min(std::max(MSPL_TUNE_INT("MSPL_PYR_TAB_SEGCAP", P3_TAB_SEGMAX), 1), P3_TAB_SEGMAX);
+    seg = std::min(h, seg_cap);
+    while (seg > 6 && cols * ceil_div(h, seg) < min_waves) --seg;
+    seg = ceil_div(h, ceil_div(h, seg));
+    if (dbg_seg > 0 && dbg_seg <= P3_TAB_SEGMAX) seg = std::min(dbg_seg, h);
+    p.seg_tab = seg; p.nseg_tab = ceil_div(h, seg); p.waves_tab = cols * p.nseg_tab;
+    p.taken = p.waves_ik < (1ll << 31) && p.waves_tab < (1ll << 31);
+    return p;
+}
+
+static size_t p3_table_floats(const P3Shape& s, int h) { return (size_t)2 * (h + 2) * 24 + (size_t)30 * (s.ncb * 62 + 2) * s.PXL; }
+
+static void p3_fill_geom(Pyr3Geom& g, const P3Shape& s, int N, int P, int h, int w, const int32_t* hs, const int32_t* ws) {
     memset(&g, 0, sizeof(g));
     g.N = N; g.P = P; g.h = h; g.w = w;
     for (int i = 0; i < 5; ++i) {
@@ -353,34 +469,124 @@
         if (i < 2) { g.sh[i] = bilinear_scale(h, hs[i]); g.sw[i] = bilinear_scale(w, ws[i]); }
         if (i > 2) { g.sh[i] = bilinear_scale(hs[i], h); g.sw[i] = bilinear_scale(ws[i], w); }
     }
-    g.CBW = 62 * PXL;
-    g.ncb = ceil_div(w, g.CBW);
-    static const int dbg_seg = MSPL_TUNE_INT("MSPL_PYR_SEG", 0);
-    int seg = std::min(h, P3_SEGMAX);
-    while (seg > 6 && (int64_t)N * P * g.ncb * ceil_div(h, seg) < 2048) --seg;
-    seg = ceil_div(h, ceil_div(h, seg));
-    if (dbg_seg > 0 && dbg_seg <= P3_SEGMAX) seg = std::min(dbg_seg, h);
-    g.SEG = seg;
-    g.nseg = ceil_div(h, seg);
-    const int64_t waves = (int64_t)N * P * g.ncb * g.nseg;
-    if (waves >= (1ll << 31)) return 1;
+    g.CBW = s.CBW;
+    g.ncb = s.ncb;
+}
+
+struct P3TabKey {
+    int v[9];
+    bool operator==(const P3TabKey& o) const { return memcmp(v, o.v, sizeof(v)) == 0; }
+};
+static P3TabKey p3_tab_key(const P3Shape& s, int h, int w, const int32_t* hs, const int32_t* ws) {
+    P3TabKey k = {{h, w, hs[0], ws[0], hs[1], ws[1], s.T0, s.T1, s.PXL}};
+    return k;
+}
+static std::mutex p3_tab_mutex;
+static std::unordered_map<const void*, P3TabKey>& p3_tab_registry() {
+    static std::unordered_map<const void*, P3TabKey> m;
+    return m;
+}
+
+int pyrpool_stream_tables_build(int h, int w, int nb, const int32_t* hs, const int32_t* ws, float* tab, int64_t bytes,
+                                hipStream_t stream) {
+    const P3Shape s = p3_shape(h, w, nb, hs, ws);
+    MSPL_REQUIRE(s.ok, MSPL_ERR_UNSUPPORTED, "pyr_stream_tables: the streaming form does not cover a %dx%d map with these branches", h, w);
+    MSPL_REQUIRE(bytes == (int64_t)(p3_table_floats(s, h) * sizeof(float)), MSPL_ERR_BAD_SHAPE,
+                 "pyr_stream_tables: %lld bytes given, the geometry takes %zu", (long long)bytes, p3_table_floats(s, h) * sizeof(float));
+    MSPL_REQUIRE((((uintptr_t)tab) & 15) == 0, MSPL_ERR_BAD_SHAPE, "pyr_stream_tables: the table must be 16-byte aligned");
+    Pyr3Geom g;
+    p3_fill_geom(g, s, 0, 0, h, w, hs, ws);
+    const int entries = 2 * (h + 2) * 3 + 2 * 3 * (s.ncb * 62 + 2) * s.PXL;
+    const dim3 grid((unsigned)ceil_div(entries, 256)), blk(256);
+#define MSPL_P3_TABLES(A, B, L) hipLaunchKernelGGL((p3_tables_kernel<A, B, L>), grid, blk, 0, stream, g, tab)
+    if (s.PXL == 1) {
+        if (s.T0 == 3 && s.T1 == 3) MSPL_P3_TABLES(3, 3, 1);
+        else if (s.T0 == 3) MSPL_P3_TABLES(3, 5, 1);
+        else if (s.T1 == 3) MSPL_P3_TABLES(5, 3, 1);
+        else MSPL_P3_TABLES(5, 5, 1);
+    } else {
+        if (s.T0 == 3 && s.T1 == 3) MSPL_P3_TABLES(3, 3, 2);
+        else if (s.T0 == 3) MSPL_P3_TABLES(3, 5, 2);
+        else if (s.T1 == 3) MSPL_P3_TABLES(5, 3, 2);
+        else MSPL_P3_TABLES(5, 5, 2);
+    }
+#undef MSPL_P3_TABLES
+    MSPL_CHECK_LAUNCH("pyr_stream_tables");
+    std::lock_guard<std::mutex> lock(p3_tab_mutex);
+    p3_tab_registry()[tab] = p3_tab_key(s, h, w, hs, ws);
+    return MSPL_OK;
+}
+
+int64_t pyrpool_stream_tables_bytes(int h, int w, int nb, const int32_t* hs, const int32_t* ws) {
+    const P3Shape s = p3_shape(h, w, nb, hs, ws);
+    return s.ok ? (int64_t)(p3_table_floats(s, h) * sizeof(float)) : 0;
+}
+
+void pyrpool_stream_plan(int N, int P, int h, int w, int nb, const int32_t* hs, const int32_t* ws, int32_t* out) {
+    const P3Plan p = p3_plan(N, P, h, w, nb, hs, ws);
+    for (int i = 0; i < MSPL_PYR_STREAM_PLAN_LEN; ++i) out[i] = 0;
+    if (!p.taken) return;
+    out[MSPL_PYR_STREAM_PLAN_TAKEN] = 1;
+    out[MSPL_PYR_STREAM_PLAN_T0] = p.s.T0; out[MSPL_PYR_STREAM_PLAN_T1] = p.s.T1;
+    out[MSPL_PYR_STREAM_PLAN_PXL] = p.s.PXL; out[MSPL_PYR_STREAM_PLAN_NCB] = p.s.ncb; out[MSPL_PYR_STREAM_PLAN_CBW] = p.s.CBW;
+    out[MSPL_PYR_STREAM_PLAN_SEG] = p.seg_tab; out[MSPL_PYR_STREAM_PLAN_NSEG] = p.nseg_tab;
+    out[MSPL_PYR_STREAM_PLAN_WAVES] = (int32_t)p.waves_tab;
+    out[MSPL_PYR_STREAM_PLAN_SEG_INKERNEL] = p.seg_ik; out[MSPL_PYR_STREAM_PLAN_NSEG_INKERNEL] = p.nseg_ik;
+    out[MSPL_PYR_STREAM_PLAN_WAVES_INKERNEL] = (int32_t)p.waves_ik;
+}
+
+int pyrpool_stream_try(const float* x, int N, int P, int h, int w, int nb, const int32_t* hs, const int32_t* ws,
+                       const float* const* stage_w, const float* const* down_e, const float* br_scale,
+                       const float* br_shift, const float* br_alpha, const float* merge_w, const Epi& e, float* out,
+                       hipStream_t stream, float* zcat, const float* tab) {
+    const P3Plan plan = p3_plan(N, P, h, w, nb, hs, ws);
+    if (!plan.taken) return 1;
+    const P3Shape& s = plan.s;
+    if (tab) {
+        MSPL_REQUIRE(!zcat, MSPL_ERR_UNSUPPORTED, "pyrpool_fused(streaming form): the training forward takes no geometry tables");
+        bool known = false;
+        P3TabKey have;
+        {
+            std::lock_guard<std::mutex> lock(p3_tab_mutex);
+            auto it = p3_tab_registry().find(tab);
+            if (it != p3_tab_registry().end()) { known = true; have = it->second; }
+        }
+        MSPL_REQUIRE(known, MSPL_ERR_BAD_SHAPE, "pyrpool_fused(streaming form): no geometry tables were built at %p", (const void*)tab);
+        MSPL_REQUIRE(have == p3_tab_key(s, h, w, hs, ws), MSPL_ERR_BAD_SHAPE,
+                     "pyrpool_fused(streaming form): the tables were built for a %dx%d map (up branches %dx%d, %dx%d), this is %dx%d "
+                     "(%dx%d, %dx%d)", have.v[0], have.v[1], have.v[2], have.v[3], have.v[4], have.v[5], h, w, hs[0], ws[0], hs[1], ws[1]);
+    }
+    if (e.pre_add || e.residual || e.reinf_r || e.gate) return 1;
+    if (!stage_w[0] || !stage_w[1] || !stage_w[2] || !down_e[3] || !down_e[4]) return 1;
+    const int PXL = s.PXL;
+    if (PXL == 2 && ((((uintptr_t)out) & 7) || (((uintptr_t)x) & 7))) return 1;
+    if (zcat && (!e.raw || e.ctot != P || e.coff != 0)) return 1;
+    if (zcat && PXL == 2 && ((((uintptr_t)zcat) | ((uintptr_t)e.raw)) & 7)) return 1;
+    Pyr3Geom g;
+    p3_fill_geom(g, s, N, P, h, w, hs, ws);
+    g.SEG = tab ? plan.seg_tab : plan.seg_ik;
+    g.nseg = tab ? plan.nseg_tab : plan.nseg_ik;
+    const int64_t waves = tab ? plan.waves_tab : plan.waves_ik;
     g.total = (unsigned)waves;
     const dim3 grid((unsigned)(waves / 4)), blk(256);
+#define MSPL_P3_ARGS x, stage_w[0], stage_w[1], stage_w[2], down_e[3], down_e[4], br_scale, br_shift, br_alpha, merge_w, e.scale, e.shift, e.alpha, e.ctot, e.coff, g, out
 #define MSPL_P3_LAUNCH(A, B, L) do { \
-        if (zcat) hipLaunchKernelGGL((pyrpool_stream_kernel<A, B, L, true>), grid, blk, 0, stream, x, stage_w[0], stage_w[1], stage_w[2], down_e[3], down_e[4], br_scale, br_shift, br_alpha, merge_w, e.scale, e.shift, e.alpha, e.ctot, e.coff, g, out, zcat, e.raw); \
-        else hipLaunchKernelGGL((pyrpool_stream_kernel<A, B, L, false>), grid, blk, 0, stream, x, stage_w[0], stage_w[1], stage_w[2], down_e[3], down_e[4], br_scale, br_shift, br_alpha, merge_w, e.scale, e.shift, e.alpha, e.ctot, e.coff, g, out, (float*)nullptr, (float*)nullptr); } while (0)
+        if (zcat) hipLaunchKernelGGL((pyrpool_stream_kernel<A, B, L, true, false>), grid, blk, 0, stream, MSPL_P3_ARGS, zcat, e.raw, (const float*)nullptr); \
+        else if (tab) hipLaunchKernelGGL((pyrpool_stream_kernel<A, B, L, false, true>), grid, blk, 0, stream, MSPL_P3_ARGS, (float*)nullptr, (float*)nullptr, tab); \
+        else hipLaunchKernelGGL((pyrpool_stream_kernel<A, B, L, false, false>), grid, blk, 0, stream, MSPL_P3_ARGS, (float*)nullptr, (float*)nullptr, (const float*)nullptr); } while (0)
     if (PXL == 1) {
-        if (taps[0] == 3 && taps[1] == 3) MSPL_P3_LAUNCH(3, 3, 1);
-        else if (taps[0] == 3) MSPL_P3_LAUNCH(3, 5, 1);
-        else if (taps[1] == 3) MSPL_P3_LAUNCH(5, 3, 1);
+        if (s.T0 == 3 && s.T1 == 3) MSPL_P3_LAUNCH(3, 3, 1);
+        else if (s.T0 == 3) MSPL_P3_LAUNCH(3, 5, 1);
+        else if (s.T1 == 3) MSPL_P3_LAUNCH(5, 3, 1);
         else MSPL_P3_LAUNCH(5, 5, 1);
     } else {
-        if (taps[0] == 3 && taps[1] == 3) MSPL_P3_LAUNCH(3, 3, 2);
-        else if (taps[0] == 3) MSPL_P3_LAUNCH(3, 5, 2);
-        else if (taps[1] == 3) MSPL_P3_LAUNCH(5, 3, 2);
+        if (s.T0 == 3 && s.T1 == 3) MSPL_P3_LAUNCH(3, 3, 2);
+        else if (s.T0 == 3) MSPL_P3_LAUNCH(3, 5, 2);
+        else if (s.T1 == 3) MSPL_P3_LAUNCH(5, 3, 2);
         else MSPL_P3_LAUNCH(5, 5, 2);
     }
 #undef MSPL_P3_LAUNCH
+#undef MSPL_P3_ARGS
     MSPL_CHECK_LAUNCH("pyrpool_fused(streaming form)");
     return MSPL_OK;
 }
diff --git a/mspl_amd/layers.py b/mspl_amd/layers.py
--- a/mspl_amd/layers.py
+++ b/mspl_amd/layers.py
@@ -174,6 +174,7 @@
 _FUSED_DW_EXP = os.environ.get('MSPL_EESP_EXP', '1') != '0'
 _FUSED_DOWN_HEAD = os.environ.get('MSPL_DOWN_HEAD', '1') != '0'
 _FUSED_HEAD_CLASSIFIER = os.environ.get('MSPL_HEAD_CLASSIFIER', '1') != '0'
+_PYR_STREAM_TABLES = os.environ.get('MSPL_PYR_STREAM_TABLES', '1') != '0'
 _FUSED_DEC_MERGE = True
 _FUSED_NEXT_PROJ = os.environ.get('MSPL_EESP_NEXT', '1') != '0'
 _FUSED_EESP_TRAIN = os.environ.get('MSPL_FUSED_EESP_TRAIN', '1') != '0'
@@ -665,7 +666,20 @@
         bscale, bshift = bn_fold(br[0])
         mcbr = self.merge_layer[2]
         return ops.pyrpool_fused(x, sizes, stage_ws, down_es, bscale, bshift, br[1].weight, mcbr.cbr[0].weight,
-                                 mcbr.epi())
+                                 mcbr.epi(), tables=self._stream_tables(x, sizes) if _PYR_STREAM_TABLES else None)
+
+    def _stream_tables(self, x, sizes):
+        N, P, height, width = x.shape
+        key = (x.device, N * P % 4, height, width) + tuple((int(a), int(b)) for a, b in sizes)
+        store = self.__dict__.setdefault('_mspl_pyr_tables', {})
+        if key not in store:
+            if torch.cuda.is_current_stream_capturing():
+                return None
+            taken = ops.pyrpool_stream_plan(x.shape, sizes)['taken']
+            store[key] = ops.pyr_stream_tables(height, width, sizes, x.device) if taken else None
+            if taken:
+                torch.cuda.current_stream(x.device).synchronize()
+        return store[key]
 
     def _body_train_fused(self, x, sizes):
         bn0, act0 = self.merge_layer[0].br[0], self.merge_layer[0].br[1]
diff --git a/mspl_amd/ops.py b/mspl_amd/ops.py
--- a/mspl_amd/ops.py
+++ b/mspl_amd/ops.py
@@ -525,7 +525,30 @@
     return outs
 
 
-def pyrpool_fused(x, sizes, stage_ws, down_es, br_scale, br_shift, br_alpha, merge_w, ep=None, out=None):
+def pyrpool_stream_plan(shape, sizes):
+    N, P, h, w = [int(v) for v in shape]
+    nb = len(sizes)
+    hs = (ctypes.c_int32 * nb)(*[int(s[0]) for s in sizes])
+    ws = (ctypes.c_int32 * nb)(*[int(s[1]) for s in sizes])
+    out = (ctypes.c_int32 * nat.PYR_STREAM_PLAN_LEN)()
+    check(lib.mspl_pyrpool_stream_plan(N, P, h, w, nb, hs, ws, out))
+    names = ('TAKEN', 'T0', 'T1', 'PXL', 'NCB', 'CBW', 'SEG', 'NSEG', 'WAVES', 'SEG_INKERNEL', 'NSEG_INKERNEL', 'WAVES_INKERNEL')
+    return {n.lower(): int(out[getattr(nat, 'PYR_STREAM_PLAN_' + n)]) for n in names}
+
+
+def pyr_stream_tables(h, w, sizes, device):
+    nb = len(sizes)
+    hs = (ctypes.c_int32 * nb)(*[int(s[0]) for s in sizes])
+    ws = (ctypes.c_int32 * nb)(*[int(s[1]) for s in sizes])
+    nbytes = int(lib.mspl_pyr_stream_tables_bytes(int(h), int(w), nb, hs, ws))
+    if nbytes <= 0:
+        return None
+    tab = torch.empty(nbytes // 4, device=device, dtype=torch.float32)
+    check(lib.mspl_pyr_stream_tables_build(int(h), int(w), nb, hs, ws, _p(tab), nbytes, _stream()))
+    return tab
+
+
+def pyrpool_fused(x, sizes, stage_ws, down_es, br_scale, br_shift, br_alpha, merge_w, ep=None, out=None, tables=None):
     x = _f32(x, 'x')
     N, P, h, w = x.shape
     nb = len(sizes)
@@ -552,6 +575,11 @@
     bs, bh, ba = _vec(br_scale, nb * P, 'br_scale'), _vec(br_shift, nb * P, 'br_shift'), _vec(br_alpha, nb * P, 'br_alpha')
     dst, coff = _dest(out, (N, P, h, w), x)
     s, k2 = _build(ep, dst, coff, N, P, h * w)
+    if tables is not None and not (s.pre_add or s.residual or s.reinf_r or s.gate or s.raw_out):
+        check(lib.mspl_pyrpool_fused_tab_fwd(_p(x), N, P, h, w, nb, hs, ws, sw, de, _p(bs), _p(bh), _p(ba), _p(merge_w),
+                                             s.scale, s.shift, s.alpha, s.out_ctot, s.out_coff, s.flags, _p(dst), _p(tables),
+                                             _stream()))
+        return dst
     check(lib.mspl_pyrpool_fused_fwd(_p(x), N, P, h, w, nb, hs, ws, sw, de, _p(bs), _p(bh), _p(ba), _p(merge_w),
                                      ctypes.byref(s), _p(dst), _stream()))
     return dst
```

Measured after the change: 22120 images/s (median of 6 runs). 1.4% higher.
